# sinamalakouti/CDDMSL

Measured on AMD Instinct MI355X. Metric: images/sec (train step) VOC+Clipart RN50-C4, higher is better.
Workload: dtype bf16

## Files before the change

cddmsl_amd/csrc/bottleneck64.hip:

```cpp
#include "gemm_common.h"

namespace {

struct BottleneckArgs {
  const char* o1;
  const char* w2;
  const char* w3;
  const char* wd;
  const char* w1n;
  const char* x0;
  const char* residual;
  char* out;
  char* o1n;
  const float *s2, *b2, *s3, *b3, *sd, *bd, *s1n, *b1n;
  int H, W, M;
  FastDiv dW, dH;
};

template <bool DOWN, bool NEXT>
__global__ __launch_bounds__(512) void k_bottleneck64(BottleneckArgs p) {
  using T = __bf16;
  constexpr int KS2 = 36, WAVES = 8;
  const int lane = threadIdx.x & 63, r = lane & 31, hh = lane >> 5, wv = threadIdx.x >> 6;
  __shared__ __attribute__((aligned(16))) u32x4 wl2[2 * KS2 * 64];
  __shared__ __attribute__((aligned(16))) u32x4 wl3[8 * 4 * 64];
  __shared__ __attribute__((aligned(16))) u32x4 slots[WAVES * 256];
  __shared__ float sbl[4 * 256];
  for (int f = wv; f < 2 * KS2; f += WAVES) {
    const int nt = f / KS2, ks = f - nt * KS2;
    wl2[f * 64 + lane] = *(const u32x4*)(p.w2 + ((long)(nt * 32 + r) * (2 * KS2) + 2 * ks + hh) * 16);
  }
  for (int f = wv; f < 32; f += WAVES)
    wl3[f * 64 + lane] = *(const u32x4*)(p.w3 + ((long)((f >> 2) * 32 + r) * 8 + 2 * (f & 3) + hh) * 16);
  if (threadIdx.x < 256) {
    sbl[threadIdx.x] = p.s3[threadIdx.x]; sbl[256 + threadIdx.x] = p.b3[threadIdx.x];
    if (DOWN) { sbl[512 + threadIdx.x] = p.sd[threadIdx.x]; sbl[768 + threadIdx.x] = p.bd[threadIdx.x]; }
  }
  __syncthreads();
  float sc2[2], bi2[2], sc1[2], bi1[2];
#pragma unroll
  for (int nt = 0; nt < 2; ++nt) {
    sc2[nt] = p.s2[nt * 32 + r]; bi2[nt] = p.b2[nt * 32 + r];
    sc1[nt] = NEXT ? p.s1n[nt * 32 + r] : 1.f; bi1[nt] = NEXT ? p.b1n[nt * 32 + r] : 0.f;
  }
  const int wave = blockIdx.x * WAVES + wv, nwaves = gridDim.x * WAVES;
  const int ntiles = (p.M + 31) >> 5;
  const __amdgpu_buffer_rsrc_t rx = __builtin_amdgcn_make_buffer_rsrc((void*)(p.o1 - (long)(p.W + 1) * 128), 0, 0x7fffffff, 0x00020000);
  const __amdgpu_buffer_rsrc_t rx0 = __builtin_amdgcn_make_buffer_rsrc((void*)p.x0, 0, DOWN ? p.M * 128 : 0, 0x00020000);
  const __amdgpu_buffer_rsrc_t rres = __builtin_amdgcn_make_buffer_rsrc((void*)p.residual, 0, DOWN ? 0 : p.M * 512, 0x00020000);
  const __amdgpu_buffer_rsrc_t rout = __builtin_amdgcn_make_buffer_rsrc((void*)p.out, 0, p.M * 512, 0x00020000);
  const __amdgpu_buffer_rsrc_t ro1n = __builtin_amdgcn_make_buffer_rsrc((void*)p.o1n, 0, NEXT ? p.M * 128 : 0, 0x00020000);
  const float relu_floor = 0.f;
  char* const sb = (char*)slots + wv * 4096;
  char* wbase[8];
#pragma unroll
  for (int c = 0; c < 8; ++c) wbase[c] = sb + 4 * hh * 128 + ((((r >> 3) ^ (hh << 1)) ^ c) << 4) + (r & 7) * 2;
  const char* fbase = sb + r * 128;
  const int fsw = hh ^ ((r >> 1) & 7);
  const int mrow = lane >> 3;
  char* const mbase0 = sb + mrow * 128 + ((((lane & 7) ^ (lane >> 4))) << 4);
  char* const mbase1 = sb + mrow * 128 + ((((lane & 7) ^ (lane >> 4) ^ 4)) << 4);
  auto maddr = [&](int i) -> char* { return ((i & 1) ? mbase1 : mbase0) + i * 1024; };
  auto put = [&](const f32x16 (&acc)[2], const float (&sc)[2], const float (&bi)[2]) {
#pragma unroll
    for (int nt = 0; nt < 2; ++nt)
#pragma unroll
      for (int g = 0; g < 16; ++g) {
        float v = affine<T>(acc[nt][g], sc[nt], bi[nt]);
        asm("v_max_f32 %0, %1, %2" : "=v"(v) : "v"(v), "s"(relu_floor));
        *(unsigned short*)(wbase[(nt << 2) ^ ((g & 3) >> 1) ^ (((g >> 2) & 1) << 2)] + ((g & 3) + 8 * (g >> 2)) * 128) = f2bf(v);
      }
  };
  auto frags = [&](u32x4 (&fa)[4]) {
#pragma unroll
    for (int ks = 0; ks < 4; ++ks) fa[ks] = *(const u32x4*)(fbase + (((2 * ks) ^ fsw) << 4));
  };
  for (int tile = wave; tile < ntiles; tile += nwaves) {
    const int m = tile * 32 + r;
    const bool vm = m < p.M;
    const unsigned mm = vm ? m : 0;
    const unsigned tq = fdiv(mm, p.dW), ox = mm - tq * p.W;
    const unsigned img = fdiv(tq, p.dH), oy = tq - img * p.H;
    const int iy0 = (int)oy - 1, ix0 = (int)ox - 1;
    const unsigned lbase = (unsigned)((((int)img * p.H + iy0 + 1) * p.W + ix0 + 1) * 128) + hh * 16;
    unsigned bad = vm ? 0u : 0x1ffu;
#pragma unroll
    for (int ky = 0; ky < 3; ++ky)
#pragma unroll
      for (int kx = 0; kx < 3; ++kx)
        if ((unsigned)(iy0 + ky) >= (unsigned)p.H || (unsigned)(ix0 + kx) >= (unsigned)p.W) bad |= 1u << (3 * ky + kx);
    u32x4 a[KS2];
#pragma unroll
    for (int ks = 0; ks < KS2; ++ks) {
      const int t0 = (2 * ks) / 8, c0 = (2 * ks) % 8;
      const unsigned v = lbase | (__builtin_amdgcn_ubfe(bad, (unsigned)t0, 1u) << 31);
      a[ks] = __builtin_amdgcn_raw_buffer_load_b128(rx, v, ((t0 / 3) * p.W + (t0 % 3)) * 128 + c0 * 16, 0);
    }
    const unsigned rowbad[4] = {tile * 32 + mrow < p.M ? 0u : 0x80000000u, tile * 32 + 8 + mrow < p.M ? 0u : 0x80000000u,
                                tile * 32 + 16 + mrow < p.M ? 0u : 0x80000000u, tile * 32 + 24 + mrow < p.M ? 0u : 0x80000000u};
    const unsigned vq = (unsigned)(mrow * 512 + (lane & 7) * 16);
    u32x4 xa[4], rr[4];
    if (DOWN) {
#pragma unroll
      for (int ks = 0; ks < 4; ++ks)
        xa[ks] = __builtin_amdgcn_raw_buffer_load_b128(rx0, (unsigned)(r * 128 + hh * 16) | (vm ? 0u : 0x80000000u), tile * 4096 + ks * 32, 0);
    } else {
#pragma unroll
      for (int i = 0; i < 4; ++i) rr[i] = __builtin_amdgcn_raw_buffer_load_b128(rres, (vq + i * 4096) | rowbad[i], tile * 16384, 0);
    }
    f32x16 acc2[2];
#pragma unroll
    for (int nt = 0; nt < 2; ++nt)
#pragma unroll
      for (int g = 0; g < 16; ++g) acc2[nt][g] = 0.f;
    int wlane = lane;
    asm volatile("" : "+v"(wlane));
    const char* const wdp = p.wd + ((wlane & 31) * 8 + (wlane >> 5)) * 16;
    const char* const w1p = p.w1n + ((wlane & 31) * 32 + (wlane >> 5)) * 16;
#pragma unroll
    for (int ks = 0; ks < KS2; ++ks)
#pragma unroll
      for (int nt = 0; nt < 2; ++nt) Mma<T>::step(acc2[nt], a[ks], wl2[(nt * KS2 + ks) * 64 + wlane]);
    asm volatile("" ::: "memory");
    put(acc2, sc2, bi2);
    asm volatile("" ::: "memory");
    u32x4 fo2[4];
    frags(fo2);
    asm volatile("" ::: "memory");
    f32x16 acc1[2];
#pragma unroll
    for (int nt = 0; nt < 2; ++nt)
#pragma unroll
      for (int g = 0; g < 16; ++g) acc1[nt][g] = 0.f;
#pragma unroll
    for (int q = 0; q < 4; ++q) {
      f32x16 acc3[2], accd[2];
#pragma unroll
      for (int nt = 0; nt < 2; ++nt)
#pragma unroll
        for (int g = 0; g < 16; ++g) { acc3[nt][g] = 0.f; accd[nt][g] = 0.f; }
      u32x4 wdf[DOWN ? 2 : 1][DOWN ? 4 : 1], w1f[NEXT ? 2 : 1][NEXT ? 4 : 1];
      if (DOWN) {
#pragma unroll
        for (int nt = 0; nt < 2; ++nt)
#pragma unroll
          for (int ks = 0; ks < 4; ++ks)
            wdf[DOWN ? nt : 0][DOWN ? ks : 0] = *(const u32x4*)(wdp + ((q * 2 + nt) * 32 * 8 + 2 * ks) * 16);
      }
      if (!DOWN) {
#pragma unroll
        for (int i = 0; i < 4; ++i) *(u32x4*)maddr(i) = rr[i];
        if (q < 3) {
#pragma unroll
          for (int i = 0; i < 4; ++i) rr[i] = __builtin_amdgcn_raw_buffer_load_b128(rres, (vq + i * 4096) | rowbad[i], tile * 16384 + (q + 1) * 128, 0);
        }
      }
#pragma unroll
      for (int ks = 0; ks < 4; ++ks)
#pragma unroll
        for (int nt = 0; nt < 2; ++nt) Mma<T>::step(acc3[nt], fo2[ks], wl3[(((q * 2 + nt) << 2) + ks) * 64 + wlane]);
      if (DOWN) {
#pragma unroll
        for (int ks = 0; ks < 4; ++ks)
#pragma unroll
          for (int nt = 0; nt < 2; ++nt) Mma<T>::step(accd[nt], xa[ks], wdf[DOWN ? nt : 0][DOWN ? ks : 0]);
      }
      if (NEXT) {
#pragma unroll
        for (int nt = 0; nt < 2; ++nt)
#pragma unroll
          for (int ks = 0; ks < 4; ++ks)
            w1f[NEXT ? nt : 0][NEXT ? ks : 0] = *(const u32x4*)(w1p + (nt * 32 * 32 + 2 * (4 * q + ks)) * 16);
      }
      asm volatile("" ::: "memory");
#pragma unroll
      for (int nt = 0; nt < 2; ++nt) {
        const int ch = (q * 2 + nt) * 32 + r;
        const float s3 = sbl[ch], b3 = sbl[256 + ch];
        const float sd = DOWN ? sbl[512 + ch] : 1.f, bd = DOWN ? sbl[768 + ch] : 0.f;
#pragma unroll
        for (int g = 0; g < 16; ++g) {
          unsigned short* e = (unsigned short*)(wbase[(nt << 2) ^ ((g & 3) >> 1) ^ (((g >> 2) & 1) << 2)] + ((g & 3) + 8 * (g >> 2)) * 128);
          float v = affine<T>(acc3[nt][g], s3, b3);
          if (DOWN) v += bf2f(f2bf(affine<T>(accd[nt][g], sd, bd)));
          else v += bf2f(*e);
          asm("v_max_f32 %0, %1, %2" : "=v"(v) : "v"(v), "s"(relu_floor));
          *e = f2bf(v);
        }
      }
      asm volatile("" ::: "memory");
#pragma unroll
      for (int i = 0; i < 4; ++i) {
        const u32x4 o = *(const u32x4*)maddr(i);
        __builtin_amdgcn_raw_buffer_store_b128(o, rout, (vq + i * 4096) | rowbad[i], tile * 16384 + q * 128, CDDMSL_STORE_AUX);
        asm volatile("s_nop 4" ::: "memory");
        asm volatile("" :: "v"(o));
      }
      if (NEXT) {
        u32x4 fo[4];
        frags(fo);
#pragma unroll
        for (int ks = 0; ks < 4; ++ks)
#pragma unroll
          for (int nt = 0; nt < 2; ++nt) Mma<T>::step(acc1[nt], fo[ks], w1f[NEXT ? nt : 0][NEXT ? ks : 0]);
      }
      asm volatile("" ::: "memory");
    }
    if (NEXT) {
      put(acc1, sc1, bi1);
      asm volatile("" ::: "memory");
#pragma unroll
      for (int i = 0; i < 4; ++i) {
        const u32x4 o = *(const u32x4*)maddr(i);
        __builtin_amdgcn_raw_buffer_store_b128(o, ro1n, (unsigned)((i * 64 + lane) * 16) | rowbad[i], tile * 4096, 0);
        asm volatile("s_nop 4" ::: "memory");
        asm volatile("" :: "v"(o));
      }
      asm volatile("" ::: "memory");
    }
  }
}

}

extern "C" int cddmsl_bottleneck64_ok(int Nimg, int H, int W, int dtype) {
  if (dtype != 0 || Nimg <= 0 || H <= 0 || W <= 0) return 0;
  return (long)Nimg * H * W + W + 64 < (1L << 31) / 512 ? 1 : 0;
}

extern "C" int cddmsl_bottleneck64_fwd(const void* o1, const void* w2, const float* s2, const float* b2, const void* w3,
                                       const float* s3, const float* b3, const void* residual, const void* x0, const void* wd,
                                       const float* sd, const float* bd, const void* w1n, const float* s1n, const float* b1n,
                                       void* out, void* o1n, int Nimg, int H, int W, int dtype, void* stream) {
  if (!cddmsl_bottleneck64_ok(Nimg, H, W, dtype)) return CDDMSL_ERR_ARG;
  if (!o1 || !w2 || !s2 || !b2 || !w3 || !s3 || !b3 || !out) return CDDMSL_ERR_ARG;
  const bool down = wd != nullptr, next = w1n != nullptr;
  if (down ? (!x0 || !sd || !bd || residual) : (!residual || x0 || sd || bd)) return CDDMSL_ERR_ARG;
  if (next ? (!s1n || !b1n || !o1n) : (s1n || b1n || o1n)) return CDDMSL_ERR_ARG;
  BottleneckArgs a;
  a.o1 = (const char*)o1; a.w2 = (const char*)w2; a.w3 = (const char*)w3; a.wd = (const char*)wd; a.w1n = (const char*)w1n;
  a.x0 = (const char*)x0; a.residual = (const char*)residual; a.out = (char*)out; a.o1n = (char*)o1n;
  a.s2 = s2; a.b2 = b2; a.s3 = s3; a.b3 = b3; a.sd = sd; a.bd = bd; a.s1n = s1n; a.b1n = b1n;
  a.H = H; a.W = W; a.M = Nimg * H * W;
  a.dW = make_fastdiv((unsigned)W); a.dH = make_fastdiv((unsigned)H);
  if (record_kernel(13)) return CDDMSL_OK;
  const int ncu = persistent_blocks_raw(), ntiles = (a.M + 31) / 32;
  const int want = (ntiles + 7) / 8, cap = ncu > 0 ? ncu : 256;
  const unsigned nb = (unsigned)(want < cap ? want : cap);
  const hipStream_t st = (hipStream_t)stream;
  if (down && next) hipLaunchKernelGGL((k_bottleneck64<true, true>), dim3(nb), dim3(512), 0, st, a);
  else if (down) hipLaunchKernelGGL((k_bottleneck64<true, false>), dim3(nb), dim3(512), 0, st, a);
  else if (next) hipLaunchKernelGGL((k_bottleneck64<false, true>), dim3(nb), dim3(512), 0, st, a);
  else hipLaunchKernelGGL((k_bottleneck64<false, false>), dim3(nb), dim3(512), 0, st, a);
  return launch_status();
}
```

cddmsl_amd/csrc/conv_fwd.hip:

```cpp
#include "gemm_common.h"

namespace {

template <typename T> __device__ __forceinline__ void load8(const char* p, float* f);
template <> __device__ __forceinline__ void load8<__bf16>(const char* p, float* f) {
  const u32x4 v = *(const u32x4*)p;
#pragma unroll
  for (int j = 0; j < 4; ++j) { f[2 * j] = bf2f(v[j] & 0xffff); f[2 * j + 1] = bf2f(v[j] >> 16); }
}
template <> __device__ __forceinline__ void load8<float>(const char* p, float* f) {
  const f32x4 a = ((const f32x4*)p)[0], b = ((const f32x4*)p)[1];
  f[0] = a[0]; f[1] = a[1]; f[2] = a[2]; f[3] = a[3]; f[4] = b[0]; f[5] = b[1]; f[6] = b[2]; f[7] = b[3];
}

__device__ __forceinline__ int swz(int row, int chunk) { return row * KCH + (chunk ^ ((row >> 1) & 7)); }

template <typename T>
__global__ __launch_bounds__(256, 2) void k_conv_fwd_reg(ConvArgs p) {
  __shared__ __attribute__((aligned(16))) u32x4 lds[2][BM * KCH];
  const int t = threadIdx.x;
  const int ntn = (p.Cout + BN - 1) / BN;
  const int tile_n = blockIdx.x % ntn, tile_m = blockIdx.x / ntn;
  const int m0 = tile_m * BM, n0 = tile_n * BN;
  const int cc = t & 7, rb = t >> 3;
// ... 153 lines not shown
#pragma unroll
    for (int a = 0; a < 2; ++a) {
#pragma unroll
      for (int g = 0; g < 16; ++g) {
        int m = m0 + wm * 64 + a * 32 + (g & 3) + 8 * (g >> 2) + 4 * h;
        if (m >= p.M) continue;
        float v = affine<T>(acc[a][b][g], sc, bi);
        if (p.residual) v += Mma<T>::load(p.residual + ((long)m * p.ldr + n) * Mma<T>::ES);
        if (p.relu) v = fmaxf(v, 0.f);
        if (p.relu_mask && !(Mma<T>::load(p.relu_mask + ((long)m * p.ldm + n) * Mma<T>::ES) > 0.f)) v = 0.f;
        if (p.out_f32) *(float*)(p.y + ((long)m * p.ldy + n) * 4) = v;
        else Mma<T>::store(p.y + ((long)m * p.ldy + n) * Mma<T>::ES, v);
      }
    }
  }
}


__device__ __forceinline__ long pooled_row(const ConvArgs& p, int m) {
  const unsigned tq = fdiv((unsigned)m, p.dWo), ox = m - tq * p.Wo;
  const unsigned img = fdiv(tq, p.dHo), oy = tq - img * p.Ho;
  const unsigned hp = p.Ho >> 1, wp = p.Wo >> 1;
  return ((oy >> 1) < hp && (ox >> 1) < wp) ? ((long)img * hp + (oy >> 1)) * wp + (ox >> 1) : -1L;
}

template <typename T>
__global__ __launch_bounds__(256, 2) void k_conv_fwd(ConvArgs p) {
  __shared__ __attribute__((aligned(16))) u32x4 lds[2][2][BM * KCH];
  const int t = threadIdx.x;
  p.x += (long)blockIdx.y * p.bx; p.w += (long)blockIdx.y * p.bw; p.y += (long)blockIdx.y * p.by;
  const int wvu = __builtin_amdgcn_readfirstlane(t >> 6);
  const int ntn = (p.Cout + BN - 1) / BN;
  const int lbid = xcd_remap(blockIdx.x, gridDim.x);
  const int tile_n = lbid % ntn, tile_m = lbid / ntn;
  const int m0 = tile_m * BM, n0 = tile_n * BN;
  const int cc = t & 7, rb = t >> 3;
  const int cl = cc ^ ((rb >> 1) & 7);

  long rowoff[4], wrow[4];
  int iy0[4], ix0[4];
  bool vm[4], vn[4];
#pragma unroll
  for (int i = 0; i < 4; ++i) {
    int m = m0 + rb + 32 * i;
    vm[i] = m < p.M;
    unsigned mm = vm[i] ? m : 0;
    unsigned tq = fdiv(mm, p.dWo), ox = mm - tq * p.Wo;
    unsigned img = fdiv(tq, p.dHo), oy = tq - img * p.Ho;
    iy0[i] = (int)oy * p.stride - p.pad;
    ix0[i] = (int)ox * p.stride - p.pad;
    rowoff[i] = ((((long)img * p.Hi + iy0[i]) * p.Wi + ix0[i]) * p.xrs) * 16;
    int n = n0 + rb + 32 * i;
    vn[i] = n < p.Cout;
    wrow[i] = (long)(vn[i] ? n : 0) * p.wrs * 16;
  }
  const int nkt = (p.Kc + KCH - 1) / KCH;
  const char* zp = (const char*)g_zero_page;
  const bool taps = !(p.KH == 1 && p.KW == 1 && p.pad == 0);
  int kc = cl;
  int pp0 = (int)fdiv((unsigned)kc, p.dcpp);
  int coff = kc - pp0 * p.cpp;
  int ky = (int)fdiv((unsigned)pp0, p.dKW), kx = pp0 - ky * p.KW;

  const bool fast = (p.cpp & 7) == 0;
  const char* pa[4];
  const char* pb[4];
  int inca[4], incb[4];
  int tiles_left_in_tap = 0;
  auto retap = [&]() {
    const int delta = ((ky * p.Wi + kx) * p.xrs + coff) * 16;
#pragma unroll
    for (int i = 0; i < 4; ++i) {
      bool ok = vm[i];
      if (taps) {
        int iy = iy0[i] + ky, ix = ix0[i] + kx;
        ok = ok && iy >= 0 && iy < p.Hi && ix >= 0 && ix < p.Wi;
      }
      pa[i] = ok ? p.x + rowoff[i] + delta : zp;
      inca[i] = ok ? KCH * 16 : 0;
    }
  };
  if (fast) {
#pragma unroll
    for (int i = 0; i < 4; ++i) {
      pb[i] = vn[i] ? p.w + wrow[i] + (long)kc * 16 : zp;
      incb[i] = vn[i] ? KCH * 16 : 0;
    }
    retap();
    tiles_left_in_tap = p.cpp >> 3;
  }

  auto stage = [&](int buf) {
    if (fast) {
#pragma unroll
      for (int i = 0; i < 4; ++i) glds16(pa[i], &lds[buf][0][(8 * wvu + 32 * i) * KCH]);
#pragma unroll
      for (int i = 0; i < 4; ++i) glds16(pb[i], &lds[buf][1][(8 * wvu + 32 * i) * KCH]);
#pragma unroll
      for (int i = 0; i < 4; ++i) pb[i] += incb[i];
      if (--tiles_left_in_tap == 0) {
        tiles_left_in_tap = p.cpp >> 3;
        coff = cl;
        if (++kx == p.KW) { kx = 0; ++ky; }
        retap();
      } else {
#pragma unroll
        for (int i = 0; i < 4; ++i) pa[i] += inca[i];
      }
      return;
    }
    const bool vk = kc < p.Kc;
    const int delta = ((ky * p.Wi + kx) * p.xrs + coff) * 16;
#pragma unroll
    for (int i = 0; i < 4; ++i) {
      bool ok = vk && vm[i];
      if (taps) {
        int iy = iy0[i] + ky, ix = ix0[i] + kx;
        ok = ok && iy >= 0 && iy < p.Hi && ix >= 0 && ix < p.Wi;
      }
      const char* src = ok ? p.x + rowoff[i] + delta : zp;
      glds16(src, &lds[buf][0][(8 * wvu + 32 * i) * KCH]);
    }
#pragma unroll
    for (int i = 0; i < 4; ++i) {
      const char* src = (vk && vn[i]) ? p.w + wrow[i] + (long)kc * 16 : zp;
      glds16(src, &lds[buf][1][(8 * wvu + 32 * i) * KCH]);
    }
    kc += KCH;
    coff += KCH;
    while (coff >= p.cpp) {
      coff -= p.cpp;
      if (++kx == p.KW) { kx = 0; ++ky; }
    }
  };

  f32x16 acc[2][2];
#pragma unroll
  for (int a = 0; a < 2; ++a)
#pragma unroll
    for (int b = 0; b < 2; ++b)
#pragma unroll
      for (int r = 0; r < 16; ++r) acc[a][b][r] = 0.f;

  const int lane = t & 63, wv = t >> 6;
  const int wm = wv >> 1, wn = wv & 1;
  const int r = lane & 31, h = lane >> 5;

  const bool vec_ok = (p.Cout % 8 == 0) && (p.ldy % 8 == 0) && (!p.residual || p.ldr % 8 == 0) && (!p.relu_mask || p.ldm % 8 == 0);
  constexpr bool PRE = Mma<T>::ES == 2;
  u32x4 rres[2][4], rmsk[2][4];
  const bool rf32 = PRE && p.res_f32;
  if (PRE && vec_ok && ((p.residual && !rf32) || p.relu_mask)) {
    const int n = n0 + wn * 64 + (lane & 7) * 8;
#pragma unroll
    for (int a = 0; a < 2; ++a)
#pragma unroll
      for (int i = 0; i < 4; ++i) {
        int m = m0 + wm * 64 + a * 32 + (lane >> 3) + 8 * i;
        bool ok = m < p.M && n < p.Cout;
        const u32x4 z = {0u, 0u, 0u, 0u};
        if (p.res_pool) {
          const long po = pooled_row(p, m);
          rres[a][i] = (ok && po >= 0) ? *(const u32x4*)(p.residual + (po * p.ldr + n) * 2) : z;
        } else
        rres[a][i] = (ok && p.residual && !rf32) ? *(const u32x4*)(p.residual + ((long)m * p.ldr + n) * 2) : z;
        rmsk[a][i] = (ok && p.relu_mask) ? *(const u32x4*)(p.relu_mask + ((long)m * p.ldm + n) * 2) : z;
      }
  }

  stage(0);
  for (int kt = 0; kt < nkt; ++kt) {
    const int cur = kt & 1;
    if (kt + 1 < nkt) {
      stage(cur ^ 1);
      asm volatile("s_waitcnt vmcnt(8)" ::: "memory");
    } else {
      asm volatile("s_waitcnt vmcnt(0)" ::: "memory");
    }
    __builtin_amdgcn_s_barrier();
    u32x4 fa[2][2], fb[2][2];
#pragma unroll
    for (int i = 0; i < 2; ++i) {
      fa[0][i] = lds[cur][0][swz(wm * 64 + i * 32 + r, h)];
      fb[0][i] = lds[cur][1][swz(wn * 64 + i * 32 + r, h)];
    }
#pragma unroll
    for (int ks = 0; ks < KCH / 2; ++ks) {
      if (ks + 1 < KCH / 2) {
#pragma unroll
        for (int i = 0; i < 2; ++i) {
          fa[(ks + 1) & 1][i] = lds[cur][0][swz(wm * 64 + i * 32 + r, 2 * (ks + 1) + h)];
          fb[(ks + 1) & 1][i] = lds[cur][1][swz(wn * 64 + i * 32 + r, 2 * (ks + 1) + h)];
        }
      }
#pragma unroll
      for (int a = 0; a < 2; ++a)
#pragma unroll
        for (int b = 0; b < 2; ++b) Mma<T>::step(acc[a][b], fa[ks & 1][a], fb[ks & 1][b]);
    }
    asm volatile("s_waitcnt lgkmcnt(0)" ::: "memory");
    __builtin_amdgcn_s_barrier();
  }

  if (vec_ok) {
    float* ep = (float*)&lds[0][0][0] + wv * 2048;
    const int cg = lane & 7, rr = lane >> 3;
    const int n = n0 + wn * 64 + cg * 8;
    float sc[8], bi[8];
#pragma unroll
    for (int j = 0; j < 8; ++j) {
      sc[j] = (p.scale && n + j < p.Cout) ? p.scale[n + j] : 1.f;
      bi[j] = (p.bias && n + j < p.Cout) ? p.bias[n + j] : 0.f;
    }
#pragma unroll
    for (int a = 0; a < 2; ++a) {
      __syncthreads();
#pragma unroll
      for (int b = 0; b < 2; ++b)
#pragma unroll
        for (int g = 0; g < 16; ++g) {
          int row = (g & 3) + 8 * (g >> 2) + 4 * h, col = b * 32 + r;
          ep[row * 64 + ((((col >> 3) ^ (row & 7)) << 3) | (col & 7))] = acc[a][b][g];
        }
      __syncthreads();
      if (n < p.Cout) {
#pragma unroll
        for (int i = 0; i < 4; ++i) {
          int row = rr + 8 * i;
          int m = m0 + wm * 64 + a * 32 + row;
          if (m >= p.M) continue;
          const f32x4* src = (const f32x4*)(ep + row * 64 + ((cg ^ (row & 7)) << 3));
          f32x4 v0 = src[0], v1 = src[1];
          float v[8] = {v0[0], v0[1], v0[2], v0[3], v1[0], v1[1], v1[2], v1[3]};
#pragma unroll
          for (int j = 0; j < 8; ++j) v[j] = affine<T>(v[j], sc[j], bi[j]);
          if (p.residual) {
            float rv[8];
            if (rf32) load8<float>(p.residual + ((long)m * p.ldr + n) * 4, rv);
            else if (PRE) {
#pragma unroll
              for (int j = 0; j < 4; ++j) { rv[2 * j] = bf2f(rres[a][i][j] & 0xffff); rv[2 * j + 1] = bf2f(rres[a][i][j] >> 16); }
            } else if (p.res_pool) {
              const long po = pooled_row(p, m);
#pragma unroll
              for (int j = 0; j < 8; ++j) rv[j] = 0.f;
              if (po >= 0) load8<T>(p.residual + (po * p.ldr + n) * Mma<T>::ES, rv);
            } else load8<T>(p.residual + ((long)m * p.ldr + n) * Mma<T>::ES, rv);
            if (p.res_pool) {
#pragma unroll
              for (int j = 0; j < 8; ++j) rv[j] *= 0.25f;
            }
#pragma unroll
            for (int j = 0; j < 8; ++j) v[j] += rv[j];
          }
          if (p.relu) {
#pragma unroll
            for (int j = 0; j < 8; ++j) v[j] = fmaxf(v[j], 0.f);
          }
          if (p.relu_mask) {
            float mv[8];
            if (PRE) {
#pragma unroll
              for (int j = 0; j < 4; ++j) { mv[2 * j] = bf2f(rmsk[a][i][j] & 0xffff); mv[2 * j + 1] = bf2f(rmsk[a][i][j] >> 16); }
            } else load8<T>(p.relu_mask + ((long)m * p.ldm + n) * Mma<T>::ES, mv);
#pragma unroll
            for (int j = 0; j < 8; ++j) if (!(mv[j] > 0.f)) v[j] = 0.f;
          }
          if (p.out_f32 || Mma<T>::ES == 4) {
            f32x4* dst = (f32x4*)(p.y + ((long)m * p.ldy + n) * 4);
            f32x4 o0 = {v[0], v[1], v[2], v[3]}, o1 = {v[4], v[5], v[6], v[7]};
            dst[0] = o0; dst[1] = o1;
          } else {
            u32x4 o = {pack2bf(v[0], v[1]), pack2bf(v[2], v[3]), pack2bf(v[4], v[5]), pack2bf(v[6], v[7])};
            *(u32x4*)(p.y + ((long)m * p.ldy + n) * 2) = o;
          }
        }
      }
    }
    return;
  }
#pragma unroll
  for (int b = 0; b < 2; ++b) {
    int n = n0 + wn * 64 + b * 32 + r;
    if (n >= p.Cout) continue;
    float sc = p.scale ? p.scale[n] : 1.f;
    float bi = p.bias ? p.bias[n] : 0.f;
#pragma unroll
    for (int a = 0; a < 2; ++a) {
#pragma unroll
      for (int g = 0; g < 16; ++g) {
        int m = m0 + wm * 64 + a * 32 + (g & 3) + 8 * (g >> 2) + 4 * h;
        if (m >= p.M) continue;
        float v = affine<T>(acc[a][b][g], sc, bi);
        if (p.residual) v += Mma<T>::load(p.residual + ((long)m * p.ldr + n) * Mma<T>::ES);
        if (p.relu) v = fmaxf(v, 0.f);
        if (p.relu_mask && !(Mma<T>::load(p.relu_mask + ((long)m * p.ldm + n) * Mma<T>::ES) > 0.f)) v = 0.f;
        if (p.out_f32) *(float*)(p.y + ((long)m * p.ldy + n) * 4) = v;
        else Mma<T>::store(p.y + ((long)m * p.ldy + n) * Mma<T>::ES, v);
      }
    }
  }
}

template <typename T, int CPP, int NT, int NTAP = 9>
__global__ __launch_bounds__(256) void k_conv3x3_small(ConvArgs p) {
  constexpr int KC = NTAP * CPP, KS = (KC + 1) / 2;
  constexpr int PAD = NTAP == 9 ? 1 : 0;
  constexpr int ES = Mma<T>::ES;
  const int lane = threadIdx.x & 63, r = lane & 31, hh = lane >> 5;
  constexpr bool WLDS = CPP > 1;
  __shared__ __attribute__((aligned(16))) u32x4 wl[WLDS ? NT * KS * 64 : 1];
  u32x4 bw[WLDS ? 1 : NT][WLDS ? 1 : KS];
  {
    const int wv = threadIdx.x >> 6;
#pragma unroll
    for (int nt = 0; nt < NT; ++nt)
#pragma unroll
      for (int ks = 0; ks < KS; ++ks) {
        if (WLDS && ((nt * KS + ks) & 3) != wv) continue;
        const int q = 2 * ks + hh;
        u32x4 v = {0u, 0u, 0u, 0u};
        if (q < KC) v = *(const u32x4*)(p.w + ((long)(nt * 32 + r) * KC + q) * 16);
        if (WLDS) wl[(nt * KS + ks) * 64 + lane] = v;
        else bw[WLDS ? 0 : nt][WLDS ? 0 : ks] = v;
      }
    if (WLDS) __syncthreads();
  }
  float sc[NT], bi[NT];
#pragma unroll
  for (int nt = 0; nt < NT; ++nt) { sc[nt] = p.scale ? p.scale[nt * 32 + r] : 1.f; bi[nt] = p.bias ? p.bias[nt * 32 + r] : 0.f; }
  const int wave = (blockIdx.x * blockDim.x + threadIdx.x) >> 6, nwaves = (gridDim.x * blockDim.x) >> 6;
  const int ntiles = (p.M + 31) >> 5;
  const __amdgpu_buffer_rsrc_t rx = __builtin_amdgcn_make_buffer_rsrc((void*)(p.x - (long)(p.Wi + 1) * (CPP * 16)), 0, 0x7fffffff, 0x00020000);
  const long ybytes = (long)p.M * p.ldy * ES, mbytes = (long)p.M * p.ldm * ES;
  const __amdgpu_buffer_rsrc_t ry = __builtin_amdgcn_make_buffer_rsrc((void*)p.y, 0, (int)(ybytes > 0x7fffffffL ? 0x7fffffffL : ybytes), 0x00020000);
  const __amdgpu_buffer_rsrc_t rm = __builtin_amdgcn_make_buffer_rsrc((void*)p.relu_mask, 0, p.relu_mask ? (int)(mbytes > 0x7fffffffL ? 0x7fffffffL : mbytes) : 0, 0x00020000);
  const float relu_floor = p.relu ? 0.f : -__builtin_inff();
  __shared__ __attribute__((aligned(16))) u32x4 ost[ES == 2 ? 4 * 32 * NT * 4 : 1];
  const bool ost_ok = !p.relu_mask && p.ldy == NT * 32 && (long)p.M * NT * 64 < 0x7fffffffL;
  for (int tile = wave; tile < ntiles; tile += nwaves) {
    const int m = tile * 32 + r;
    const bool vm = m < p.M;
    const unsigned mm = vm ? m : 0;
    const unsigned tq = fdiv(mm, p.dWo), ox = mm - tq * p.Wo;
    const unsigned img = fdiv(tq, p.dHo), oy = tq - img * p.Ho;
    const int iy0 = (int)oy * p.stride - PAD, ix0 = (int)ox * p.stride - PAD;
    const unsigned lbase = (unsigned)((((int)img * p.Hi + iy0 + 1) * p.Wi + ix0 + 1) * (CPP * 16)) + (CPP > 1 ? hh * 16 : 0);
    unsigned bad = vm ? 0u : 0x1ffu;
    if (NTAP == 9) {
#pragma unroll
      for (int ky = 0; ky < 3; ++ky)
#pragma unroll
        for (int kx = 0; kx < 3; ++kx)
          if ((unsigned)(iy0 + ky) >= (unsigned)p.Hi || (unsigned)(ix0 + kx) >= (unsigned)p.Wi) bad |= 1u << (3 * ky + kx);
    }
    u32x4 a[KS];
#pragma unroll
    for (int ks = 0; ks < KS; ++ks) {
      const int q0 = 2 * ks, q1 = 2 * ks + 1;
      const int t0 = q0 / CPP, c0 = q0 % CPP, t1 = q1 / CPP, c1 = q1 % CPP;
      if (CPP > 1) {
        const unsigned v = lbase | (__builtin_amdgcn_ubfe(bad, (unsigned)t0, 1u) << 31);
        a[ks] = __builtin_amdgcn_raw_buffer_load_b128(rx, v, ((t0 / 3) * p.Wi + (t0 % 3)) * (CPP * 16) + c0 * 16, 0);
      } else {
        const int ky = hh ? t1 / 3 : t0 / 3, kx = hh ? t1 % 3 : t0 % 3, cc = hh ? c1 : c0;
        const bool inq = hh ? (q1 < KC) : (q0 < KC);
        const int iy = iy0 + ky, ix = ix0 + kx;
        const bool ok = vm && inq && (unsigned)iy < (unsigned)p.Hi && (unsigned)ix < (unsigned)p.Wi;
        u32x4 v = {0u, 0u, 0u, 0u};
        if (ok) v = *(const u32x4*)(p.x + ((((long)img * p.Hi + iy0) * p.Wi + ix0) + (long)ky * p.Wi + kx) * (CPP * 16) + cc * 16);
        a[ks] = v;
      }
    }
    f32x16 acc[NT];
#pragma unroll
    for (int nt = 0; nt < NT; ++nt)
#pragma unroll
      for (int g = 0; g < 16; ++g) acc[nt][g] = 0.f;
    int wlane = lane;
    asm volatile("" : "+v"(wlane));
#pragma unroll
    for (int ks = 0; ks < KS; ++ks)
#pragma unroll
      for (int nt = 0; nt < NT; ++nt) {
        if (WLDS) Mma<T>::step(acc[nt], a[ks], wl[(nt * KS + ks) * 64 + wlane]);
        else Mma<T>::step(acc[nt], a[ks], bw[WLDS ? 0 : nt][WLDS ? 0 : ks]);
      }
    if (ES == 2 && ost_ok) {
      char* ob = (char*)ost + (threadIdx.x >> 6) * (32 * NT * 64);
#pragma unroll
      for (int nt = 0; nt < NT; ++nt)
#pragma unroll
        for (int g = 0; g < 16; ++g) {
          const int row = (g & 3) + 8 * (g >> 2) + 4 * hh;
          float v = affine<T>(acc[nt][g], sc[nt], bi[nt]);
          asm("v_max_f32 %0, %1, %2" : "=v"(v) : "v"(v), "s"(relu_floor));
          *(unsigned short*)(ob + row * (NT * 64) + (nt * 32 + r) * 2) = f2bf(v);
        }
#pragma unroll
      for (int i = 0; i < 2 * NT; ++i) {
        const u32x4 o = *(const u32x4*)(ob + (i * 64 + lane) * 16);
        __builtin_amdgcn_raw_buffer_store_b128(o, ry, (unsigned)((i * 64 + lane) * 16), tile * (32 * NT * 64), 0);
      }
      continue;
    }
    const unsigned vy = (unsigned)(((tile * 32 + 4 * hh) * p.ldy + r) * ES), vmk = (unsigned)(((tile * 32 + 4 * hh) * p.ldm + r) * ES);
#pragma unroll
    for (int nt = 0; nt < NT; ++nt)
#pragma unroll
      for (int g = 0; g < 16; ++g) {
        const int row = (g & 3) + 8 * (g >> 2);
        float v = affine<T>(acc[nt][g], sc[nt], bi[nt]);
        asm("v_max_f32 %0, %1, %2" : "=v"(v) : "v"(v), "s"(relu_floor));
        if (p.relu_mask) {
          float mv;
          if (ES == 2) mv = bf2f((unsigned)__builtin_amdgcn_raw_buffer_load_b16(rm, vmk, (row * p.ldm + nt * 32) * ES, 0));
          else mv = __builtin_bit_cast(float, __builtin_amdgcn_raw_buffer_load_b32(rm, vmk, (row * p.ldm + nt * 32) * ES, 0));
          if (!(mv > 0.f)) v = 0.f;
        }
        if (ES == 2) __builtin_amdgcn_raw_buffer_store_b16((unsigned short)f2bf(v), ry, vy, (row * p.ldy + nt * 32) * ES, 0);
        else __builtin_amdgcn_raw_buffer_store_b32(__builtin_bit_cast(unsigned, v), ry, vy, (row * p.ldy + nt * 32) * ES, 0);
      }
  }
}

template <typename T> void launch_small(const ConvArgs& a, unsigned nb, hipStream_t st) {
  if (a.KH == 1 && a.cpp == 8) hipLaunchKernelGGL((k_conv3x3_small<T, 8, 2, 1>), dim3(nb), dim3(256), 0, st, a);
  else if (a.KH == 1) hipLaunchKernelGGL((k_conv3x3_small<T, 32, 2, 1>), dim3(nb), dim3(256), 0, st, a);
  else if (a.cpp == 1 && a.Cout == 32) hipLaunchKernelGGL((k_conv3x3_small<T, 1, 1>), dim3(nb), dim3(256), 0, st, a);
  else if (a.cpp == 1) hipLaunchKernelGGL((k_conv3x3_small<T, 1, 2>), dim3(nb), dim3(256), 0, st, a);
  else if (a.cpp == 8) hipLaunchKernelGGL((k_conv3x3_small<T, 8, 2>), dim3(nb), dim3(256), 0, st, a);
  else if (a.Cout == 32) hipLaunchKernelGGL((k_conv3x3_small<T, 4, 1>), dim3(nb), dim3(256), 0, st, a);
  else hipLaunchKernelGGL((k_conv3x3_small<T, 4, 2>), dim3(nb), dim3(256), 0, st, a);
}

template <typename T> void launch_tile128(const ConvArgs& a, const Plan& p, hipStream_t st) {
  const dim3 grid(p.gx, p.gy);
  switch (p.kernel) {
    case 8: launch_small<T>(a, p.gx, st); break;
    case 2: hipLaunchKernelGGL(k_conv_fwd_reg<T>, grid, dim3(256), 0, st, a); break;
    default: hipLaunchKernelGGL(k_conv_fwd<T>, grid, dim3(256), 0, st, a); break;
  }
}

}

void launch_fwd_tile128(const ConvArgs& a, const Plan& p, Operand op, hipStream_t st) {
  if (op == OP_BF16) launch_tile128<__bf16>(a, p, st);
  else launch_tile128<float>(a, p, st);
}
```

cddmsl_amd/csrc/gemm_common.h:

```cpp
#pragma once
#include "common.h"
#include <cstdlib>

namespace {

constexpr int BM = 128, BN = 128, KCH = 8;

struct FastDiv {
  unsigned mul, shr, d;
};
static inline FastDiv make_fastdiv(unsigned d) {
  FastDiv f;
  f.d = d;
  unsigned s = 0;
  while ((1ull << s) < d) ++s;
  f.shr = s;
  f.mul = (unsigned)(((1ull << 32) * ((1ull << s) - d)) / d + 1);
  return f;
}
__device__ __forceinline__ unsigned fdiv(unsigned n, const FastDiv& f) { return (__umulhi(n, f.mul) + n) >> f.shr; }

template <typename T> __device__ __forceinline__ float affine(float v, float sc, float bi) {
  return sizeof(T) <= 2 ? __builtin_fmaf(v, sc, bi) : v * sc + bi;
}

#ifndef CDDMSL_STORE_AUX
#define CDDMSL_STORE_AUX 2
#endif
#ifndef CDDMSL_LOAD_AUX
#define CDDMSL_LOAD_AUX 0
#endif

struct ConvArgs {
  const char* x;
  const char* w;
  char* y;
  const float* scale;
  const float* bias;
  const char* residual;
  const char* relu_mask;
  int Nimg, Hi, Wi, Cin, Ho, Wo, Cout, KH, KW, stride, pad;
  int ldy, ldr, ldm;
  int relu, out_f32, pool;
  int res_f32;
  int res_pool;
  int M, Kc, cpp;
  FastDiv dWo, dHo, dcpp, dKW;
  int xrs, wrs;
  long bx, bw, by;
  char* y8 = nullptr;
  const float* q8 = nullptr;
  unsigned* amax8 = nullptr;
  float* partial = nullptr;
  int tile0 = 0, ksplits = 1, kper = 0, tile_limit = 0;
  int nt_out = 1;
#ifdef CDDMSL_TILE_STAMPS
  unsigned long long* tstamps = nullptr;
#endif
};

template <typename T> struct Mma;
template <> struct Mma<__bf16> {
  static constexpr int ES = 2;
  __device__ static __forceinline__ void step(f32x16& acc, const u32x4& a, const u32x4& b) {
    acc = __builtin_amdgcn_mfma_f32_32x32x16_bf16(__builtin_bit_cast(bf16x8, a), __builtin_bit_cast(bf16x8, b), acc, 0, 0, 0);
  }
  __device__ static __forceinline__ float load(const char* p) { return bf2f(*(const unsigned short*)p); }
  __device__ static __forceinline__ void store(char* p, float v) { *(unsigned short*)p = f2bf(v); }
};
template <> struct Mma<float> {
  static constexpr int ES = 4;
  __device__ static __forceinline__ void step(f32x16& acc, const u32x4& a, const u32x4& b) {
    const f32x4 fa = __builtin_bit_cast(f32x4, a), fb = __builtin_bit_cast(f32x4, b);
    acc = __builtin_amdgcn_mfma_f32_32x32x2f32(fa[0], fb[0], acc, 0, 0, 0);
    acc = __builtin_amdgcn_mfma_f32_32x32x2f32(fa[1], fb[1], acc, 0, 0, 0);
    acc = __builtin_amdgcn_mfma_f32_32x32x2f32(fa[2], fb[2], acc, 0, 0, 0);
    acc = __builtin_amdgcn_mfma_f32_32x32x2f32(fa[3], fb[3], acc, 0, 0, 0);
  }
  __device__ static __forceinline__ float load(const char* p) { return *(const float*)p; }
  __device__ static __forceinline__ void store(char* p, float v) { *(float*)p = v; }
};
typedef __attribute__((ext_vector_type(8))) int i32x8;

__device__ __forceinline__ int xcd_remap(int bid, int nblk) {
  const int q = nblk >> 3, rem = nblk & 7, x = bid & 7, j = bid >> 3;
  return (x < rem ? x * (q + 1) : rem * (q + 1) + (x - rem) * q) + j;
}

template <typename T> __device__ __forceinline__ u32x4 avg4(const u32x4& a, const u32x4& b, const u32x4& c, const u32x4& d);
template <> __device__ __forceinline__ u32x4 avg4<float>(const u32x4& a, const u32x4& b, const u32x4& c, const u32x4& d) {
  const f32x4 fa = __builtin_bit_cast(f32x4, a), fb = __builtin_bit_cast(f32x4, b);
  const f32x4 fc = __builtin_bit_cast(f32x4, c), fd = __builtin_bit_cast(f32x4, d);
  f32x4 r = ((fa + fb) + (fc + fd)) * 0.25f;
  return __builtin_bit_cast(u32x4, r);
}
template <> __device__ __forceinline__ u32x4 avg4<__bf16>(const u32x4& a, const u32x4& b, const u32x4& c, const u32x4& d) {
  u32x4 r;
#pragma unroll
  for (int j = 0; j < 4; ++j) {
    float lo = (bf2f(a[j] & 0xffff) + bf2f(b[j] & 0xffff)) + (bf2f(c[j] & 0xffff) + bf2f(d[j] & 0xffff));
    float hi = (bf2f(a[j] >> 16) + bf2f(b[j] >> 16)) + (bf2f(c[j] >> 16) + bf2f(d[j] >> 16));
    r[j] = pack2bf(lo * 0.25f, hi * 0.25f);
  }
  return r;
}

__device__ __attribute__((aligned(16))) unsigned int g_zero_page[4] = {0u, 0u, 0u, 0u};

__device__ __forceinline__ void glds16(const void* g, void* l) {
  __builtin_amdgcn_global_load_lds((const __attribute__((address_space(1))) void*)g,
                                   (__attribute__((address_space(3))) void*)l, 16, 0, 0);
}

struct WgradArgs {
  const char* x;
  const char* dy;
  float* dw;
  const float* scale;
  int Nimg, Hi, Wi, Cin, Ho, Wo, Cout, KH, KW, stride, pad, ldd, pool;
  int M, Kc, cpp, K, ncc;
  int mtiles_per_split;
  FastDiv dWo, dHo;
  int xrs;
  int ldo;
  int direct;
  long bx, bd, bo;
  const float* g0 = nullptr;
  const unsigned long long* mbits = nullptr;
  float* gpos = nullptr;
  float* ws = nullptr;
#ifdef CDDMSL_TILE_STAMPS
  unsigned long long* tstamps = nullptr;
#endif
};

constexpr int WM = 64;
constexpr int WROW = 16 + 4;

__device__ __forceinline__ int fsw(int row) { return ((row & 3) << 2) | ((row >> 2) & 3); }

__device__ __forceinline__ void store_frags(f32x4* dst, const f32x16 (&acc)[4][2]) {
#pragma unroll
  for (int a = 0; a < 4; ++a)
#pragma unroll
    for (int b = 0; b < 2; ++b)
#pragma unroll
      for (int g4 = 0; g4 < 4; ++g4) {
        const f32x4 v = {acc[a][b][4 * g4], acc[a][b][4 * g4 + 1], acc[a][b][4 * g4 + 2], acc[a][b][4 * g4 + 3]};
        dst[((a * 2 + b) * 4 + g4) * 64] = v;
      }
}

static long env_int(const char* name, long dflt, bool* set = nullptr) {
  const char* e = getenv(name);
  if (set) *set = e != nullptr;
  return e ? atol(e) : dflt;
}

enum Operand { OP_BF16 = 0, OP_F32 = 1, OP_FP8 = 2 };
static int elem_size(Operand op) { return op == OP_BF16 ? 2 : op == OP_F32 ? 4 : 1; }

struct Plan {
  int kernel;
  unsigned gx, gy;
  int splits;
  int mtiles_per_split;
  int bpb;
};

static int persistent_blocks_raw() {
  static int ncu = -1;
  if (ncu < 0) {
    int dev = 0, n = 0;
    if (hipGetDevice(&dev) != hipSuccess || hipDeviceGetAttribute(&n, hipDeviceAttributeMultiprocessorCount, dev) != hipSuccess) n = 0;
    ncu = (n / 8) * 8;
  }
  return ncu;
}

}

extern "C" {
__attribute__((visibility("hidden"))) void launch_fwd_tile128(const ConvArgs& a, const Plan& p, Operand op, hipStream_t st);
__attribute__((visibility("hidden"))) void launch_fwd_tile256(const ConvArgs& a, const Plan& p, Operand op, hipStream_t st, void* ws, long ws_bytes);
__attribute__((visibility("hidden"))) void launch_wgrad(WgradArgs& a, const Plan& p, Operand op, hipStream_t st, void* ws, long ws_bytes);
__attribute__((visibility("hidden"))) void launch_gemm_tn(const WgradArgs& p, Operand op, const Plan& pl, int batch, int mode, hipStream_t st);
__attribute__((visibility("hidden"))) void launch_attnpool_dx(const WgradArgs& p, unsigned gx, unsigned gy, int nbatch, int bpb, hipStream_t st);
__attribute__((visibility("hidden"))) bool record_kernel(int id);
}
```

cddmsl_amd/csrc/gemm_conv.hip:

```cpp
#include "gemm_common.h"

namespace {

template <typename T>
__device__ __forceinline__ void weight_prep_body(const float* w, const float* scale, char* wf, char* wd, int Cout, int KH, int KW, int Cin,
                                                 long first, long stride) {
  __shared__ float tile[32][33];
  const int taps = KH * KW, nit = (Cin + 31) / 32, nct = (Cout + 31) / 32;
  const long ntiles = (long)nct * taps * nit;
  const int tx = threadIdx.x & 31, ty = threadIdx.x >> 5;
  constexpr int ES = Mma<T>::ES;
  for (long tl = first; tl < ntiles; tl += stride) {
    const int it = (int)(tl % nit); const long q = tl / nit;
    const int tap = (int)(q % taps), ct = (int)(q / taps);
    const int ky = tap / KW, kx = tap % KW;
    __syncthreads();
#pragma unroll
    for (int r = 0; r < 4; ++r) {
      const int co = ct * 32 + ty + 8 * r, ci = it * 32 + tx;
      float v = 0.f;
      if (co < Cout && ci < Cin) {
        const long i = ((long)co * taps + tap) * Cin + ci;
        v = w[i];
        if (wf) Mma<T>::store(wf + i * ES, v);
        if (scale) v *= scale[co];
      }
      tile[ty + 8 * r][tx] = v;
    }
    __syncthreads();
    if (wd) {
#pragma unroll
      for (int r = 0; r < 4; ++r) {
        const int ci = it * 32 + ty + 8 * r, co = ct * 32 + tx;
        if (ci < Cin && co < Cout) {
          const long j = (((long)ci * KH + (KH - 1 - ky)) * KW + (KW - 1 - kx)) * Cout + co;
          Mma<T>::store(wd + j * ES, tile[tx][ty + 8 * r]);
        }
      }
    }
  }
}
template <typename T>
__global__ __launch_bounds__(256) void k_weight_prep(const float* w, const float* scale, char* wf, char* wd, int Cout, int KH, int KW, int Cin) {
  weight_prep_body<T>(w, scale, wf, wd, Cout, KH, KW, Cin, (long)blockIdx.x, (long)gridDim.x);
}
template <typename T>
__global__ __launch_bounds__(256) void k_weight_prep_multi(const long long* table) {
  const long long* e = table + 8 * (long)blockIdx.y;
  weight_prep_body<T>((const float*)e[0], (const float*)e[1], (char*)e[2], (char*)e[3], (int)e[4], (int)e[5], (int)e[6], (int)e[7],
                      (long)blockIdx.x, (long)gridDim.x);
}

static thread_local int g_last_kernel = 0;
static thread_local int g_plan_only = 0;


static bool gemm256_legal(const ConvArgs& a) {
  const bool vec_ok = (a.ldy % 8 == 0) && (!a.residual || a.ldr % 8 == 0) && (!a.relu_mask || a.ldm % 8 == 0);
  if (a.pool || (a.cpp & 7) || (a.Cout & 255) || !vec_ok || a.KH * a.KW > 31) return false;
  if (2 * a.pad > a.KH - 1 || 2 * a.pad > a.KW - 1) return false;
  return true;
}

static bool use_gemm256(const ConvArgs& a, int batch) {
  const long mode = env_int("CDDMSL_GEMM256", 1);
  if (mode == 0) return false;
  if (!gemm256_legal(a)) return false;
  if (mode == 2) return true;
  const long tiles = (long)((a.M + 255) / 256) * (a.Cout / 256) * batch;
  return tiles >= 160;
}

static bool fwd2_legal(const ConvArgs& a) {
  const bool vec_ok = (a.ldy % 8 == 0) && (!a.residual || a.ldr % 8 == 0) && (!a.relu_mask || a.ldm % 8 == 0);
  if (a.pool || a.res_pool || (a.cpp & 3) || (a.Cout & 127) || !vec_ok || a.KH * a.KW > 31) return false;
  if (2 * a.pad > a.KH - 1 || 2 * a.pad > a.KW - 1) return false;
  return true;
}
static bool use_fwd2(const ConvArgs& a, int batch) {
  const long mode = env_int("CDDMSL_FWD2", 1);
  if (mode == 0 || !fwd2_legal(a)) return false;
  if (mode == 2) return true;
  if (use_gemm256(a, batch) || batch != 1) return false;
  return (long)(a.Cout / 128) * ((a.M + 255) / 256) >= env_int("CDDMSL_FWD2_MIN", 256);
}

static Plan plan_fwd(const ConvArgs& a, Operand op, int batch) {
  const long tiles256 = (long)(a.Cout / 256) * ((a.M + 255) / 256);
  if (op == OP_FP8) {
    if (!gemm256_legal(a) || tiles256 > 0x7fffffffL) return {};
    return {10, (unsigned)tiles256, 1};
  }
  if (a.y8 && !use_gemm256(a, batch)) return {};
  const long tiles128 = (long)((a.Cout + BN - 1) / BN) * ((a.M + BM - 1) / BM);
  if (tiles128 > 0x7fffffffL) return {};
  const bool packed = batch == 1 && a.xrs == a.cpp && a.wrs == a.Kc;
  if (!a.pool && a.KH == 3 && a.KW == 3 && a.pad == 1 && (a.cpp == 1 || a.cpp == 4 || (a.cpp == 8 && a.Cout == 64)) &&
      (a.Cout == 32 || a.Cout == 64) && !a.residual && !a.out_f32 && packed) {
    return {8, a.cpp > 1 ? 256u * 2 : 256u * 8, 1};
  }
  if (op == OP_BF16 && !a.pool && a.KH == 1 && a.KW == 1 && a.pad == 0 && a.stride == 1 && a.Cout == 64 && (a.cpp == 8 || a.cpp == 32) &&
      !a.residual && !a.out_f32 && !a.y8 && packed && a.ldy == 64 && env_int("CDDMSL_SMALL_1X1", 1) != 0) return {8, 512, 1};
  if (use_fwd2(a, batch)) return {11, (unsigned)((long)(a.Cout / 128) * ((a.M + 255) / 256)), (unsigned)batch};
  if (use_gemm256(a, batch)) return {3, (unsigned)tiles256, (unsigned)batch};
  if (a.pool) return {2, (unsigned)tiles128, 1};
  return {1, (unsigned)tiles128, (unsigned)batch};
}

static void* g_ws = nullptr;
static long g_ws_bytes = 0;

static int run_fwd(const ConvArgs& a, Operand op, const Plan& p, void* stream) {
  if (p.kernel == 0) return CDDMSL_ERR_ARG;
  g_last_kernel = p.kernel;
  if (g_plan_only) return CDDMSL_OK;
  if (p.kernel == 3 || p.kernel == 10 || p.kernel == 11) launch_fwd_tile256(a, p, op, (hipStream_t)stream, g_ws, g_ws_bytes);
  else launch_fwd_tile128(a, p, op, (hipStream_t)stream);
  return launch_status();
}

}

#ifdef CDDMSL_TILE_STAMPS
static unsigned long long* g_tile_stamps = nullptr;
extern "C" void cddmsl_debug_tile_stamps(unsigned long long* p) { g_tile_stamps = p; }
#endif
extern "C" int cddmsl_last_kernel(void) { return g_last_kernel; }
extern "C" int cddmsl_plan_only(int on) { const int was = g_plan_only; g_plan_only = on; return was; }
bool record_kernel(int id) { g_last_kernel = id; return g_plan_only != 0; }

static int nt_out_for(long out_bytes) {
  static const long nt_min_mb = env_int("CDDMSL_NT_MIN_MB", 128);
  return out_bytes > (nt_min_mb << 20) ? 1 : 0;
}

static int fill_conv(ConvArgs& a, Operand op, const void* x, const void* w, void* y, const float* scale, const float* bias,
                     const void* residual, const void* relu_mask, int Nimg, int Hi, int Wi, int Cin, int Cout, int KH, int KW,
                     int stride, int pad, int pool, int ldy, int ldr, int ldm, int relu, int out_f32, void* y8, const float* q8,
                     float* amax8) {
  const int es = elem_size(op);
  if (Nimg < 0 || Hi <= 0 || Wi <= 0 || Cin <= 0 || Cout <= 0 || KH <= 0 || KW <= 0 || stride <= 0) return CDDMSL_ERR_ARG;
  if ((Cin * es) % 16 != 0) return CDDMSL_ERR_ARG;
  if (pool && (KH != 1 || KW != 1 || pad != 0 || stride != 1)) return CDDMSL_ERR_ARG;
  a.x = (const char*)x; a.w = (const char*)w; a.y = (char*)y; a.scale = scale; a.bias = bias;
  a.residual = (const char*)residual; a.relu_mask = (const char*)relu_mask;
  a.Nimg = Nimg; a.Hi = Hi; a.Wi = Wi; a.Cin = Cin; a.Cout = Cout; a.KH = KH; a.KW = KW; a.stride = stride; a.pad = pad;
  if (pool) { a.Ho = Hi / 2; a.Wo = Wi / 2; }
  else { a.Ho = (Hi + 2 * pad - KH) / stride + 1; a.Wo = (Wi + 2 * pad - KW) / stride + 1; }
  if (a.Ho <= 0 || a.Wo <= 0) return CDDMSL_ERR_ARG;
  if ((out_f32 & 2) && (!(out_f32 & 1) || !residual || relu_mask || pool)) return CDDMSL_ERR_ARG;
  a.ldy = ldy; a.ldr = ldr; a.ldm = ldm; a.relu = relu; a.out_f32 = out_f32 & 1; a.pool = pool;
  a.res_f32 = (op == OP_BF16 && (out_f32 & 2)) ? 1 : 0;
  a.res_pool = (out_f32 & 4) ? 1 : 0;
  if (a.res_pool && (!residual || (out_f32 & 2) || pool || KH != 1 || KW != 1 || pad != 0 || (long)Nimg * (a.Ho / 2) * (a.Wo / 2) * ldr * es >= (1L << 31) ||
                     (Cout & 7) || (ldy & 7) || (ldr & 7) || (relu_mask && (ldm & 7)))) return CDDMSL_ERR_ARG;
  if (a.res_f32 && ((Cout & 7) || (ldy & 7) || (ldr & 7))) return CDDMSL_ERR_ARG;
  long M = (long)Nimg * a.Ho * a.Wo;
  if (M > 0x7fffff00L) return CDDMSL_ERR_ARG;
  a.M = (int)M; a.cpp = Cin * es / 16; a.Kc = KH * KW * a.cpp;
  a.dWo = make_fastdiv((unsigned)a.Wo); a.dHo = make_fastdiv((unsigned)a.Ho);
  a.dcpp = make_fastdiv((unsigned)a.cpp); a.dKW = make_fastdiv((unsigned)KW);
  a.xrs = a.cpp; a.wrs = a.Kc; a.bx = a.bw = a.by = 0;
#ifdef CDDMSL_TILE_STAMPS
  a.tstamps = g_tile_stamps;
#endif
  if (a.M == 0) return CDDMSL_OK;
  a.nt_out = nt_out_for((long)a.M * Cout * 2);
  if (y8) {
    if (op == OP_F32 || (out_f32 & 1) || ldy != Cout) return CDDMSL_ERR_ARG;
    a.y8 = (char*)y8; a.q8 = q8; a.amax8 = (unsigned*)amax8;
  }
  return CDDMSL_OK;
}

static int conv_fwd_any(Operand op, const void* x, const void* w, void* y, const float* scale, const float* bias,
                        const void* residual, const void* relu_mask, int Nimg, int Hi, int Wi, int Cin,
                        int Cout, int KH, int KW, int stride, int pad, int pool, int ldy, int ldr, int ldm,
                        int relu, int out_f32, void* y8, const float* q8, float* amax8, void* stream) {
  ConvArgs a;
  const int st = fill_conv(a, op, x, w, y, scale, bias, residual, relu_mask, Nimg, Hi, Wi, Cin, Cout, KH, KW, stride, pad, pool, ldy, ldr, ldm,
                           relu, out_f32, y8, q8, amax8);
  if (st != CDDMSL_OK || a.M == 0) return st;
  return run_fwd(a, op, plan_fwd(a, op, 1), stream);
}

extern "C" int cddmsl_conv_fwd(const void* x, const void* w, void* y, const float* scale, const float* bias,
                               const void* residual, const void* relu_mask, int Nimg, int Hi, int Wi, int Cin,
                               int Cout, int KH, int KW, int stride, int pad, int pool, int ldy, int ldr, int ldm,
                               int relu, int out_f32, int dtype, void* stream) {
  if (dtype != 0 && dtype != 1) return CDDMSL_ERR_ARG;
  return conv_fwd_any((Operand)dtype, x, w, y, scale, bias, residual, relu_mask, Nimg, Hi, Wi, Cin, Cout, KH, KW, stride, pad, pool, ldy, ldr, ldm,
                      relu, out_f32, nullptr, nullptr, nullptr, stream);
}

extern "C" int cddmsl_conv_fwd_q8(const void* x, const void* w, void* y, const float* scale, const float* bias,
                                  const void* residual, const void* relu_mask, int Nimg, int Hi, int Wi, int Cin,
                                  int Cout, int KH, int KW, int stride, int pad, int relu, void* y8, const float* q8, float* amax8,
                                  void* stream) {
  if (!y8) return CDDMSL_ERR_ARG;
  return conv_fwd_any(OP_BF16, x, w, y, scale, bias, residual, relu_mask, Nimg, Hi, Wi, Cin, Cout, KH, KW, stride, pad, 0, Cout, Cout, Cout,
                      relu, 0, y8, q8, amax8, stream);
}

extern "C" int cddmsl_conv_fwd_fp8(const void* x, const void* w, void* y, const float* scale, const float* bias,
                                   const void* residual, const void* relu_mask, int Nimg, int Hi, int Wi, int Cin, int Cout, int KH,
                                   int KW, int pad, int relu, int out_f32, void* y8, const float* q8, float* amax8, void* stream) {
  if (Cin % 128 != 0 || (out_f32 & ~1)) return CDDMSL_ERR_ARG;
  return conv_fwd_any(OP_FP8, x, w, y, scale, bias, residual, relu_mask, Nimg, Hi, Wi, Cin, Cout, KH, KW, 1, pad, 0, Cout, Cout, Cout,
                      relu, out_f32, y8, q8, amax8, stream);
}

static bool wgrad256_ok(const WgradArgs& a, int batch) {
  const long mode = env_int("CDDMSL_GEMM256", 1);
  if (mode == 0) return false;
  if ((a.Cout & 255) || (a.K & 255) || (a.cpp & 7) || (a.ldd & 7)) return false;
  if (mode == 2) return true;
  return (long)(a.Cout / 256) * (a.K / 256) * batch * ((a.M + WM - 1) / WM) >= env_int("CDDMSL_WGRAD256_MIN", 4000);
}
static bool wgrad256_span_ok(int mtiles_per_split, int Wi, long row_bytes) {
  return ((long)mtiles_per_split * WM + WM + 2L * Wi + 2) * row_bytes + (1L << 20) < (1L << 31);
}

static int even_split(int total_mt, long* splits) {
  const int mps = (int)((total_mt + *splits - 1) / *splits);
  *splits = (total_mt + mps - 1) / mps;
  return mps;
}

static long split_512_rounds(long tiles, int total_mt, bool taps) {
  bool forced;
  const long target = env_int("CDDMSL_WGRAD_BLOCKS", taps ? 1024 : 512, &forced);
  const long maxs = (total_mt + 7) / 8;
  long splits = 1;
  const long r0 = (target + 511) / 512;
  double best = -1.0;
  for (long r = r0; r <= r0 + 1; ++r) {
    long c = (512 * r) / tiles;
    if (c < 1) c = 1;
    if (c > maxs) c = maxs;
    long real = c;
    even_split(total_mt, &real);
    const long blocks = tiles * real, rounds = (blocks + 511) / 512;
    const double eff = (double)blocks / (512.0 * rounds);
    if (eff > best + 0.03) { best = eff; splits = c; }
    if (c == maxs) break;
  }
  if (forced) { splits = (target + tiles - 1) / tiles; if (splits > maxs) splits = maxs; }
  return splits < 1 ? 1 : splits;
}

static long split_256_rounds(long tiles, int total_mt) {
  const long maxs = (total_mt + 15) / 16;
  long sp = 1;
  double best = -1.0;
  for (int r = 1; r <= 6; ++r) {
    long c = (256L * r) / tiles;
    if (c < 1) continue;
    if (c > maxs) c = maxs;
    const long blocks = tiles * c, rounds = (blocks + 255) / 256;
    const double eff = (double)blocks / (256.0 * rounds);
    if (eff > best + 0.02) { best = eff; sp = c; }
    if (c == maxs) break;
  }
  return sp;
}

static Plan plan_wgrad(const WgradArgs& a, Operand op, int batch) {
  const int es = elem_size(op), total_mt = (a.M + WM - 1) / WM;
  const long tiles256 = (long)(a.Cout / 256) * (a.K / 256);
  const long row_bytes = (long)a.ldd * es > a.xrs * 16L ? (long)a.ldd * es : a.xrs * 16L;
  if (op == OP_FP8) {
    long sp = split_256_rounds(tiles256, total_mt);
    const int mps = even_split(total_mt, &sp);
    if (!wgrad256_span_ok(mps, a.Wi, row_bytes)) return {};
    return {12, (unsigned)(tiles256 * sp), 1, (int)sp, mps};
  }
  const int cols = 256 / es;
  const long tiles = (long)((a.Cout + cols - 1) / cols) * ((a.K + cols - 1) / cols);
  long splits = split_512_rounds(tiles, total_mt, !(a.KH == 1 && a.KW == 1));
  const int mps = even_split(total_mt, &splits);
  if (tiles * splits > 0x7fffffffL) return {};
  const bool same = !a.pool && a.stride == 1 && a.Ho == a.Hi && a.Wo == a.Wi;
  if (same && op == OP_BF16 && wgrad256_ok(a, batch)) {
    bool forced;
    const long want = env_int("CDDMSL_WGRAD256_BLOCKS", 0, &forced);
    const long maxs = (total_mt + 15) / 16;
    long sp = forced ? (want + tiles256 - 1) / tiles256 : split_256_rounds(tiles256, total_mt);
    if (sp > maxs) sp = maxs;
    if (sp < 1) sp = 1;
    const int mps256 = even_split(total_mt, &sp);
    if (wgrad256_span_ok(mps256, a.Wi, row_bytes)) return {6, (unsigned)(tiles256 * sp), 1, (int)sp, mps256};
  }
  return {same ? 5 : 4, (unsigned)(tiles * splits), 1, (int)splits, mps};
}

extern "C" int cddmsl_set_workspace(void* ptr, long bytes) {
  if (bytes < 0 || (ptr == nullptr && bytes != 0) || ((size_t)ptr & 15)) return CDDMSL_ERR_ARG;
  g_ws = ptr; g_ws_bytes = bytes;
  return CDDMSL_OK;
}

static int run_wgrad(WgradArgs& a, Operand op, const Plan& p, void* stream) {
  if (p.kernel == 0) return CDDMSL_ERR_ARG;
  g_last_kernel = p.kernel;
  if (g_plan_only) return CDDMSL_OK;
  a.mtiles_per_split = p.mtiles_per_split;
  launch_wgrad(a, p, op, (hipStream_t)stream, g_ws, g_ws_bytes);
  return launch_status();
}

static int fill_wgrad(WgradArgs& a, Operand op, const void* x, const void* dy, float* dw, const float* scale, int Nimg, int Hi,
                      int Wi, int Cin, int Cout, int KH, int KW, int stride, int pad, int pool, int ldd) {
  const int es = elem_size(op);
  if (Nimg < 0 || Hi <= 0 || Wi <= 0 || Cin <= 0 || Cout <= 0 || KH <= 0 || KW <= 0 || stride <= 0) return CDDMSL_ERR_ARG;
  if ((Cin * es) % 16 != 0 || (Cout * es) % 16 != 0 || (ldd * es) % 16 != 0) return CDDMSL_ERR_ARG;
  if (pool && (KH != 1 || KW != 1 || pad != 0 || stride != 1)) return CDDMSL_ERR_ARG;
  a.x = (const char*)x; a.dy = (const char*)dy; a.dw = dw; a.scale = scale;
  a.Nimg = Nimg; a.Hi = Hi; a.Wi = Wi; a.Cin = Cin; a.Cout = Cout; a.KH = KH; a.KW = KW; a.stride = stride; a.pad = pad;
  a.ldd = ldd; a.pool = pool;
  if (pool) { a.Ho = Hi / 2; a.Wo = Wi / 2; }
  else { a.Ho = (Hi + 2 * pad - KH) / stride + 1; a.Wo = (Wi + 2 * pad - KW) / stride + 1; }
  if (a.Ho <= 0 || a.Wo <= 0) return CDDMSL_ERR_ARG;
  long M = (long)Nimg * a.Ho * a.Wo;
  if (M > 0x7fffff00L) return CDDMSL_ERR_ARG;
  a.M = (int)M; a.cpp = Cin * es / 16; a.Kc = KH * KW * a.cpp; a.K = KH * KW * Cin; a.ncc = Cout * es / 16;
  a.mtiles_per_split = 0;
  a.dWo = make_fastdiv((unsigned)a.Wo); a.dHo = make_fastdiv((unsigned)a.Ho);
  a.xrs = a.cpp; a.ldo = a.K; a.direct = 0; a.bx = a.bd = a.bo = 0;
#ifdef CDDMSL_TILE_STAMPS
  a.tstamps = g_tile_stamps;
#endif
  return CDDMSL_OK;
}

extern "C" int cddmsl_conv_wgrad(const void* x, const void* dy, float* dw, const float* scale, int Nimg, int Hi,
                                 int Wi, int Cin, int Cout, int KH, int KW, int stride, int pad, int pool, int ldd,
                                 int dtype, void* stream) {
  if (dtype != 0 && dtype != 1) return CDDMSL_ERR_ARG;
  WgradArgs a;
  const int st = fill_wgrad(a, (Operand)dtype, x, dy, dw, scale, Nimg, Hi, Wi, Cin, Cout, KH, KW, stride, pad, pool, ldd);
  if (st != CDDMSL_OK || a.M == 0) return st;
  return run_wgrad(a, (Operand)dtype, plan_wgrad(a, (Operand)dtype, 1), stream);
}

extern "C" int cddmsl_conv_wgrad_fp8_ok(int Cin, int Cout, int KH, int KW, int pad, int ldd) {
  return (Cin % 256 == 0 && Cout % 256 == 0 && KH == KW && (KH & 1) && 2 * pad == KH - 1 && ldd % 16 == 0) ? 1 : 0;
}
extern "C" int cddmsl_conv_wgrad_fp8(const void* x8, const void* dy8, float* dw, const float* scale, int Nimg, int Hi, int Wi, int Cin,
                                     int Cout, int KH, int KW, int pad, int ldd, void* stream) {
  if (!cddmsl_conv_wgrad_fp8_ok(Cin, Cout, KH, KW, pad, ldd) || ldd < Cout) return CDDMSL_ERR_ARG;
  WgradArgs a;
  const int st = fill_wgrad(a, OP_FP8, x8, dy8, dw, scale, Nimg, Hi, Wi, Cin, Cout, KH, KW, 1, pad, 0, ldd);
  if (st != CDDMSL_OK || a.M == 0) return st;
  return run_wgrad(a, OP_FP8, plan_wgrad(a, OP_FP8, 1), stream);
}

extern "C" int cddmsl_gemm_nt_batched(const void* a, const void* w, void* c, const float* bias, int M, int N, int K, int lda,
                                      int ldb, int ldc, int batch, long sa, long sw, long sc, int out_f32, int dtype, void* stream) {
  int es = dtype == 0 ? 2 : 4;
  if (dtype != 0 && dtype != 1) return CDDMSL_ERR_ARG;
  if (M < 0 || N <= 0 || K <= 0 || batch < 0 || batch > 65535) return CDDMSL_ERR_ARG;
  if ((K * es) % 16 || (lda * es) % 16 || (ldb * es) % 16 || (sa * es) % 16 || (sw * es) % 16) return CDDMSL_ERR_ARG;
  if (M == 0 || batch == 0) return CDDMSL_OK;
  const Operand op = (Operand)dtype;
  ConvArgs p;
  const int st = fill_conv(p, op, a, w, c, nullptr, bias, nullptr, nullptr, 1, 1, M, K, N, 1, 1, 1, 0, 0, ldc, 0, 0, 0, out_f32 ? 1 : 0,
                           nullptr, nullptr, nullptr);
  if (st != CDDMSL_OK) return st;
  p.xrs = lda * es / 16; p.wrs = ldb * es / 16;
  p.bx = sa * es; p.bw = sw * es; p.by = sc * (out_f32 ? 4 : es);
  p.nt_out = 1;
  return run_fwd(p, op, plan_fwd(p, op, batch), stream);
}

static unsigned tn_small_grid(long kt, long batch, int* bpb) {
  long b = (kt * batch + 4095) / 4096;
  if (b < 8) b = 8;
  if (b > batch) b = batch;
  *bpb = (int)b;
  return (unsigned)((batch + b - 1) / b);
}

static Plan plan_gemm_tn(const WgradArgs& p, Operand op, int batch, int mode) {
  const int cols = 256 / elem_size(op), M = p.M, N = p.Cout, K = p.K;
  const long tiles = (long)((N + cols - 1) / cols) * ((K + cols - 1) / cols);
  const int total_mt = (M + WM - 1) / WM;
  if (op == OP_BF16 && total_mt == 1 && N <= 64 && batch >= 64 && K % 128 == 0 && N % 8 == 0) {
    Plan p = {9, (unsigned)(K / 128), 0};
    p.gy = tn_small_grid(K / 128, batch, &p.bpb);
    return p;
  }
  if (total_mt <= 4 && batch >= 64) {
    long bpb = (tiles * batch + 4095) / 4096, minb = (8 + total_mt - 1) / total_mt;
    if (bpb < minb) bpb = minb;
    if (bpb > batch) bpb = batch;
    return {7, (unsigned)tiles, (unsigned)((batch + bpb - 1) / bpb), 0, 0, (int)bpb};
  }
  long splits = 1;
  if (mode == 0) {
    const long want = (2048 + tiles * batch - 1) / (tiles * batch), maxs = (total_mt + 7) / 8;
    splits = want < 1 ? 1 : (want > maxs ? maxs : want);
    if (splits < 1) splits = 1;
  }
  const int mps = even_split(total_mt, &splits);
  if (tiles * splits > 0x7fffffffL) return {};
  return {5, (unsigned)(tiles * splits), (unsigned)batch, (int)splits, mps};
}

extern "C" int cddmsl_gemm_tn_batched(const void* a, const void* b, void* out, int M, int N, int K, int lda, int ldb, int ldo,
                                      int batch, long sa, long sb, long so, int mode, int dtype, void* stream) {
  int es = dtype == 0 ? 2 : 4;
  if (dtype != 0 && dtype != 1) return CDDMSL_ERR_ARG;
  if (M <= 0 || N <= 0 || K <= 0 || batch <= 0 || batch > 65535 || mode < 0 || mode > 2) return CDDMSL_ERR_ARG;
  if ((K * es) % 16 || (N * es) % 16 || (lda * es) % 16 || (ldb * es) % 16 || (sa * es) % 16 || (sb * es) % 16) return CDDMSL_ERR_ARG;
  const Operand op = (Operand)dtype;
  WgradArgs p;
  const int fs = fill_wgrad(p, op, b, a, (float*)out, nullptr, 1, 1, M, K, N, 1, 1, 1, 0, 0, lda);
  if (fs != CDDMSL_OK) return fs;
  p.xrs = ldb * es / 16; p.ldo = ldo; p.direct = mode;
  p.bx = sb * es; p.bd = sa * es; p.bo = so * (mode == 2 ? es : 4);
  const Plan pl = plan_gemm_tn(p, op, batch, mode);
  if (pl.kernel == 0) return CDDMSL_ERR_ARG;
  g_last_kernel = pl.kernel;
  if (g_plan_only) return CDDMSL_OK;
  p.mtiles_per_split = pl.mtiles_per_split;
  launch_gemm_tn(p, op, pl, batch, mode, (hipStream_t)stream);
  return launch_status();
}

extern "C" int cddmsl_attnpool_dx(const void* pds, const void* zu, const float* g0, const unsigned long long* mbits, void* dx, float* gpos,
                                  int K, int H2, int P, int TP, int C, int dtype, void* stream) {
  if (dtype != 0 || K < 0 || P != 49 || TP != 56 || H2 <= 0 || H2 > 64 || (H2 & 7) || C <= 0 || (C & 127) || !g0 || !mbits || !dx) return CDDMSL_ERR_ARG;
  if (K == 0) return CDDMSL_OK;
  if (K > 65535 * 8) return CDDMSL_ERR_ARG;
  WgradArgs p;
  const int fs = fill_wgrad(p, OP_BF16, zu, pds, (float*)dx, nullptr, 1, 1, H2, C, TP, 1, 1, 1, 0, 0, TP);
  if (fs != CDDMSL_OK) return fs;
  p.direct = 3;
  p.bx = (long)H2 * C * 2; p.bd = (long)H2 * TP * 2; p.bo = (long)P * C * 2;
  p.g0 = g0; p.mbits = mbits; p.gpos = gpos;
  int bpb;
  const unsigned gy = tn_small_grid(C / 128, K, &bpb);
  launch_attnpool_dx(p, (unsigned)(C / 128), gy, K, bpb, (hipStream_t)stream);
  return launch_status();
}

extern "C" int cddmsl_weight_prep_multi(const long long* table, int count, int dtype, void* stream) {
  if ((dtype != 0 && dtype != 1) || count < 0 || count > 65535) return CDDMSL_ERR_ARG;
  if (count == 0) return CDDMSL_OK;
  if (dtype == 0) hipLaunchKernelGGL(k_weight_prep_multi<__bf16>, dim3(256, (unsigned)count), dim3(256), 0, (hipStream_t)stream, table);
  else hipLaunchKernelGGL(k_weight_prep_multi<float>, dim3(256, (unsigned)count), dim3(256), 0, (hipStream_t)stream, table);
  return launch_status();
}

extern "C" int cddmsl_weight_prep(const float* w, const float* scale, void* w_fwd, void* w_dgrad, int Cout, int KH,
                                  int KW, int Cin, int dtype, void* stream) {
  if (dtype != 0 && dtype != 1) return CDDMSL_ERR_ARG;
  long n = (long)Cout * KH * KW * Cin;
  if (n <= 0) return n == 0 ? CDDMSL_OK : CDDMSL_ERR_ARG;
  const long tiles = (long)((Cout + 31) / 32) * KH * KW * ((Cin + 31) / 32);
  unsigned grid = (unsigned)(tiles > 4096 ? 4096 : tiles);
  if (dtype == 0) hipLaunchKernelGGL(k_weight_prep<__bf16>, dim3(grid), dim3(256), 0, (hipStream_t)stream, w, scale, (char*)w_fwd, (char*)w_dgrad, Cout, KH, KW, Cin);
  else hipLaunchKernelGGL(k_weight_prep<float>, dim3(grid), dim3(256), 0, (hipStream_t)stream, w, scale, (char*)w_fwd, (char*)w_dgrad, Cout, KH, KW, Cin);
  return launch_status();
}
```

cddmsl_amd/hip.py:

```python
import ctypes
import os
from ctypes import c_float, c_int, c_long, c_void_p

import torch

from ._lib import check, lib, ptr, require_cuda, stream_ptr

DT = {torch.bfloat16: 0, torch.float32: 1}

_sigs_done = False


def _L():
    global _sigs_done
    L = lib()
    if not _sigs_done:
        vp, ci, cf = c_void_p, c_int, c_float
        L.cddmsl_last_kernel.argtypes = []
        L.cddmsl_plan_only.argtypes = [ci]
        L.cddmsl_conv_fwd.argtypes = [vp] * 7 + [ci] * 16 + [vp]
        L.cddmsl_bottleneck64_ok.argtypes = [ci] * 4
        L.cddmsl_bottleneck64_fwd.argtypes = [vp] * 17 + [ci] * 4 + [vp]
        L.cddmsl_conv_wgrad.argtypes = [vp] * 4 + [ci] * 12 + [vp]
        L.cddmsl_set_workspace.argtypes = [vp, c_long]
        L.cddmsl_weight_prep.argtypes = [vp] * 4 + [ci] * 5 + [vp]
        L.cddmsl_weight_prep_multi.argtypes = [vp, ci, ci, vp]
        L.cddmsl_preprocess.argtypes = [vp, vp] + [ci] * 6 + [vp, vp, ci, ci, vp]
        L.cddmsl_maxpool3s2_fwd.argtypes = [vp, vp] + [ci] * 5 + [vp]
        L.cddmsl_upsample_zero2.argtypes = [vp] * 4 + [ci] * 5 + [vp]
        L.cddmsl_meanpool_fwd.argtypes = [vp, vp, c_long, ci, ci, ci, vp]
        L.cddmsl_meanpool_bwd.argtypes = [vp, vp, c_long, ci, ci, ci, vp]
        L.cddmsl_preprocess224.argtypes = [vp, vp] + [ci] * 11 + [vp, vp, ci, vp]
        L.cddmsl_preprocess_batch.argtypes = [vp, vp, vp, ci, vp, ci, ci, ci, vp, vp, ci, ci, vp]
        L.cddmsl_preprocess224_batch.argtypes = [vp, vp, vp, ci, vp] + [ci] * 8 + [vp, vp, ci, vp]
        L.cddmsl_avgpool2_fwd.argtypes = [vp, vp] + [ci] * 5 + [vp]
        L.cddmsl_avgpool2_bwd.argtypes = [vp] * 4 + [ci] * 5 + [vp]
        L.cddmsl_avgpool2_bwd_q8.argtypes = [vp] * 4 + [ci] * 4 + [vp] * 4
        L.cddmsl_attn_tokens_fwd.argtypes = [vp] * 3 + [ci] * 5 + [vp]
        L.cddmsl_attn_tokens_bwd.argtypes = [vp] * 4 + [ci] * 5 + [vp]
        L.cddmsl_attnpool_softmax_fwd.argtypes = [vp] * 3 + [c_long, ci, ci, ci, cf, ci, vp]
        L.cddmsl_attnpool_softmax_bwd.argtypes = [vp] * 4 + [c_long, ci, ci, ci, cf, ci, vp]
        L.cddmsl_gemm_nt_batched.argtypes = [vp] * 4 + [ci] * 7 + [c_long] * 3 + [ci, ci, vp]
        L.cddmsl_gemm_tn_batched.argtypes = [vp] * 3 + [ci] * 7 + [c_long] * 3 + [ci, ci, vp]
        L.cddmsl_relu_bwd.argtypes = [vp, vp, vp, c_long, ci, ci, vp]
        L.cddmsl_colsum.argtypes = [vp, vp, c_long, ci, ci, ci, vp]
        L.cddmsl_sgd_clip_step.argtypes = [vp] * 4 + [ci, vp] + [cf] * 4 + [ci, vp]
        L.cddmsl_roi_align_forward.argtypes = [vp] * 5 + [ci] * 7 + [cf, ci, ci, ci, vp]
        L.cddmsl_roi_align_backward.argtypes = [vp] * 7 + [ci] * 7 + [cf, ci, ci, ci, vp]
        L.cddmsl_nms_anyorder.argtypes = [vp] * 4 + [ci, cf, vp, vp, vp]
        L.cddmsl_roi_align_nchw_anyorder.argtypes = [vp] * 3 + [ci] * 7 + [cf, ci, ci, ci, vp, vp, vp]
        L.cddmsl_roi_align_backward_nchw_anyorder.argtypes = [vp] * 3 + [ci] * 7 + [cf, ci, ci, ci, vp, vp, vp]
        L.cddmsl_quantize_fp8.argtypes = [vp] * 4 + [c_long, ci, vp]
        L.cddmsl_conv_fwd_fp8.argtypes = [vp] * 7 + [ci] * 10 + [vp] * 4
        L.cddmsl_conv_wgrad_fp8_ok.argtypes = [ci] * 6
        L.cddmsl_conv_wgrad_fp8.argtypes = [vp] * 4 + [ci] * 9 + [vp]
        L.cddmsl_conv_fwd_q8.argtypes = [vp] * 7 + [ci] * 10 + [vp] * 4
        L.cddmsl_fp8_dot_nt.argtypes = [vp] * 4 + [ci] * 4 + [vp]
        L.cddmsl_roi_align_forward_affine.argtypes = [vp] * 6 + [ci] * 8 + [cf, ci, ci, ci] + [vp] * 4
        L.cddmsl_roi_align_backward_pooled.argtypes = [vp] * 7 + [ci] * 7 + [cf, ci, ci, ci, vp]
        L.cddmsl_anchors.argtypes = [vp, vp, ci, ci, ci, cf, cf, vp]
        L.cddmsl_sort_desc.argtypes = [vp] * 5 + [ci, ci, vp, vp, vp]
        L.cddmsl_rpn_decode.argtypes = [vp] * 6 + [ci] * 5 + [cf] * 8 + [vp]
        L.cddmsl_nms.argtypes = [vp] * 5 + [ci, ci, cf, ci, vp]
        L.cddmsl_iou_match.argtypes = [vp, ci, vp, ci, vp, vp, vp, ci, cf, cf, ci, ci, ci, ci, vp]
        L.cddmsl_iou_match_batched.argtypes = [vp] * 7 + [ci] * 5 + [cf, cf] + [ci] * 4 + [vp]
        L.cddmsl_l2norm_fwd.argtypes = [vp, vp, vp, c_long, ci, cf, vp]
        L.cddmsl_l2norm_bwd.argtypes = [vp, vp, vp, vp, c_long, ci, vp]
        L.cddmsl_cosine_logits_fwd.argtypes = [vp] * 4 + [c_long, ci, ci, cf, cf, vp]
        L.cddmsl_cosine_logits_bwd.argtypes = [vp] * 5 + [c_long, ci, ci, cf, ci, vp]
        L.cddmsl_layernorm_fwd.argtypes = [vp] * 6 + [c_long, ci, cf, ci, vp]
        L.cddmsl_layernorm_bwd.argtypes = [vp] * 6 + [c_long, ci, ci, ci, vp]
        L.cddmsl_focal_ce_fwd.argtypes = [vp] * 4 + [c_long, ci, cf, ci, cf, vp]
        L.cddmsl_focal_ce_bwd.argtypes = [vp] * 5 + [c_long, ci, cf, ci, cf, vp]
        L.cddmsl_attn_small_fwd.argtypes = [vp] * 4 + [ci] * 8 + [cf, ci, vp]
        L.cddmsl_attn_small_bwd.argtypes = [vp] * 7 + [ci] * 8 + [cf, ci, vp]
        L.cddmsl_attn_tokens_fwd_mask.argtypes = [vp] * 4 + [ci] * 5 + [vp]
        L.cddmsl_attnpool_dx.argtypes = [vp] * 6 + [ci] * 6 + [vp]
        L.cddmsl_rpn_losses.argtypes = [vp, vp, vp, ci, vp, ci, vp, vp, vp, vp, c_long, cf, cf, cf, cf, cf, vp, vp, vp, vp, vp]
        L.cddmsl_box_l1.argtypes = [vp, ci, vp, ci, vp, vp, vp, cf, cf, cf, cf, cf, vp, vp, vp, vp]
        L.cddmsl_attn_last_fwd.argtypes = [vp] * 4 + [ci] * 8 + [cf, ci, vp]
        L.cddmsl_attn_last_bwd.argtypes = [vp] * 6 + [ci] * 8 + [cf, ci, vp]
        L.cddmsl_contrastive_fwd.argtypes = [vp] * 4 + [ci, ci, vp]
        L.cddmsl_contrastive_bwd.argtypes = [vp] * 5 + [ci, ci, vp]
        L.cddmsl_instance_boxes.argtypes = [vp] + [ci] * 4 + [vp, ci, vp, vp, vp, vp]
        L.cddmsl_text_embed.argtypes = [vp] * 4 + [c_long, ci, ci, ci, ci, vp]
        L.cddmsl_attn_causal_fwd.argtypes = [vp, vp] + [ci] * 6 + [cf, ci, vp]
        L.cddmsl_quick_gelu.argtypes = [vp, c_long, ci, vp]
        L.cddmsl_text_pool.argtypes = [vp] * 5 + [c_long, ci, ci, ci, cf, ci, vp]
        L.cddmsl_skinny_gemm_workspace.argtypes = [ci] * 3
        L.cddmsl_skinny_gemm.argtypes = [vp] * 6 + [c_long] + [ci] * 4 + [vp]
        L.cddmsl_lm_head_workspace.argtypes = [ci, ci]
        L.cddmsl_lm_head_argmax.argtypes = [vp, vp, vp, ci, vp, vp, c_long, ci, ci, ci, vp]
        L.cddmsl_decode_attn.argtypes = [vp] * 4 + [ci] * 6 + [cf, ci, vp]
        L.cddmsl_pos_embed.argtypes = [vp, ci] + [vp] * 4 + [c_long] + [ci] * 6 + [vp]
        L.cddmsl_gelu_new.argtypes = [vp, c_long, ci, vp]
        L.cddmsl_lm_head_topk_workspace.argtypes = [ci, ci]
        L.cddmsl_lm_head_topk.argtypes = [vp] * 7 + [c_long] + [ci] * 4 + [vp]
        L.cddmsl_beam_step.argtypes = [vp] * 15 + [ci] * 5 + [vp]
        L.cddmsl_decode_attn_beam.argtypes = [vp] * 7 + [ci] * 9 + [cf, ci, vp]
        _sigs_done = True
    return L


class _Profiler:

    def __init__(self):
        self.on = False
        self.only = None
        self.events = []
        self.shapes = []

    def enable(self, only=None):
        self.on, self.only, self.events, self.shapes = True, (set(only) if only else None), [], []

    def begin(self, name=None, plan=None):
        if not self.on:
            return None
        if self.only is not None:
            if name is None and plan is not None:
                L = _L()
                L.cddmsl_plan_only(1)
                try:
                    plan()
                finally:
                    L.cddmsl_plan_only(0)
                name = _CONV_KERNEL.get(L.cddmsl_last_kernel())
            if name not in self.only:
                return None
        e = torch.cuda.Event(enable_timing=True)
        e.record()
        return e

    def end(self, e0, name, flops=0.0, shape=None, nbytes=0.0):
        if e0 is None:
            return
        e1 = torch.cuda.Event(enable_timing=True)
        e1.record()
        self.events.append((name, flops, e0, e1, nbytes))
        if shape is not None:
            self.shapes.append((name, shape, flops, e0, e1, nbytes))

    def by_shape(self):
        torch.cuda.synchronize()
        out = {}
        for name, shape, flops, e0, e1, nbytes in self.shapes:
            d = out.setdefault((name, shape), [0, 0.0, 0.0, 0.0])
            d[0] += 1
            d[1] += e0.elapsed_time(e1)
            d[2] += flops
            d[3] += nbytes
        return out

    def collect(self):
        torch.cuda.synchronize()
        out = {}
        for name, flops, e0, e1, nbytes in self.events:
            d = out.setdefault(name, {"flops": 0.0, "ms": 0.0, "launches": 0, "bytes": 0.0})
            d["flops"] += flops
            d["bytes"] += nbytes
            d["ms"] += e0.elapsed_time(e1)
            d["launches"] += 1
        self.on, self.only, self.events = False, None, []
        return out


PROFILE = _Profiler()
_CONV_KERNEL = {10: "k_conv_fwd256_fp8", 11: "k_conv_fwd2", 1: "k_conv_fwd", 2: "k_conv_fwd_reg", 3: "k_conv_fwd256", 4: "k_conv_wgrad", 5: "k_conv_wgrad_dma", 6: "k_wgrad256", 7: "k_gemm_tn_stream", 8: "k_conv3x3_small", 9: "k_gemm_tn_small", 12: "k_wgrad256_fp8",
                13: "k_bottleneck64"}


def _timed(name):
    def deco(fn):
        def wrapper(*a, **k):
            e0 = PROFILE.begin(name)
            r = fn(*a, **k)
            PROFILE.end(e0, name)
            return r
        wrapper.__name__, wrapper.__doc__ = fn.__name__, fn.__doc__
        return wrapper
    return deco


def _dt(t):
    if t.dtype not in DT:
        raise TypeError(f"unsupported dtype {t.dtype}: the kernels compute in bf16 or f32")
    return DT[t.dtype]


def _conv_input_pixels(N, H, W, Ho, Wo, KH, KW, stride, pool):
    if pool:
        return N * min(H, 2 * Ho) * min(W, 2 * Wo)
    rows = min(H, Ho * min(KH, stride) if stride > KH else (Ho - 1) * stride + KH)
    cols = min(W, Wo * min(KW, stride) if stride > KW else (Wo - 1) * stride + KW)
    return N * rows * cols


class OutSpec:

    def __init__(self):
        self.full, self.used = None, 0


def conv_fwd(x, w, scale=None, bias=None, residual=None, relu=False, relu_mask=None, stride=1, pad=0,
             pool=False, out_f32=False, residual_pooled=False, emit8=None, out_spec=None):
    require_cuda(x, w, scale, bias, residual, relu_mask)
    ensure_workspace(x.device)
    assert x.dim() == 4 and w.dim() == 4 and x.is_contiguous() and w.is_contiguous()
    assert x.dtype == w.dtype
    N, H, W, Cin = x.shape
    Cout, KH, KW, Cin2 = w.shape
    assert Cin == Cin2, (x.shape, w.shape)
    if pool:
        Ho, Wo = H // 2, W // 2
    else:
        Ho, Wo = (H + 2 * pad - KH) // stride + 1, (W + 2 * pad - KW) // stride + 1
    ydt = torch.float32 if out_f32 else x.dtype
    if out_spec is not None and out_spec.full is None:
        out_spec.full = torch.empty((2 * N, Ho, Wo, Cout), device=x.device, dtype=ydt)
        y, out_spec.used = out_spec.full[:N], 1
    elif out_spec is not None and out_spec.used == 1 and tuple(out_spec.full.shape) == (2 * N, Ho, Wo, Cout) and out_spec.full.dtype == ydt:
        y, out_spec.used = out_spec.full[N:], 2
    else:
        y = torch.empty((N, Ho, Wo, Cout), device=x.device, dtype=ydt)
    for v in (scale, bias):
        assert v is None or (v.dtype == torch.float32 and v.numel() == Cout and v.is_contiguous())
    res_f32 = residual is not None and residual.dtype == torch.float32 and x.dtype != torch.float32
    if res_f32:
        assert out_f32 and relu_mask is None and not pool and Cout % 8 == 0
    if residual_pooled:
        assert residual is not None and not res_f32 and residual.dtype == x.dtype and residual.is_contiguous()
        assert tuple(residual.shape) == (N, Ho // 2, Wo // 2, Cout) and pooled_residual_ok(residual), residual.shape
    for v in (residual, relu_mask):
        assert v is None or (v is residual and residual_pooled) or (
            (v.dtype == x.dtype or (v is residual and res_f32)) and v.is_contiguous() and v.numel() == y.numel())
    y8 = None
    if emit8 is not None:
        assert x.dtype == torch.bfloat16 and not out_f32 and not pool and not residual_pooled and not res_f32
        y8 = torch.empty(y.shape, device=x.device, dtype=torch.uint8)

    def launch():
        if y8 is not None:
            return _L().cddmsl_conv_fwd_q8(ptr(x), ptr(w), ptr(y), ptr(scale), ptr(bias), ptr(residual), ptr(relu_mask),
                                           N, H, W, Cin, Cout, KH, KW, stride, pad, int(relu), ptr(y8), ptr(emit8[0]), ptr(emit8[1]), stream_ptr())
        return _L().cddmsl_conv_fwd(ptr(x), ptr(w), ptr(y), ptr(scale), ptr(bias), ptr(residual), ptr(relu_mask),
                                    N, H, W, Cin, Cout, KH, KW, stride, pad, int(pool), Cout, Cout, Cout,
                                    int(relu), int(out_f32) | (2 if res_f32 else 0) | (4 if residual_pooled else 0), _dt(x), stream_ptr())
    e0 = PROFILE.begin(plan=launch) if PROFILE.on else None
    st = launch()
    check(st, "cddmsl_conv_fwd")
    PROFILE.end(e0, _CONV_KERNEL.get(_L().cddmsl_last_kernel(), "conv_fwd") if e0 is not None else "conv_fwd",
                2.0 * N * Ho * Wo * Cout * KH * KW * Cin,
                (N * Ho * Wo, Cout, KH * KW * Cin, KH, int(pool), stride),
                nbytes=float(_conv_input_pixels(N, H, W, Ho, Wo, KH, KW, stride, bool(pool)) * Cin * x.element_size()
                             + w.numel() * w.element_size() + y.numel() * y.element_size()
                             + (residual.numel() * residual.element_size() if residual is not None else 0)
                             + (relu_mask.numel() * relu_mask.element_size() if relu_mask is not None else 0)))
    if y8 is not None:
        y._fp8 = (y8, emit8[0].data_ptr())
    return y


def bottleneck64_ok(o1, w2, w3, wd=None, w1n=None):
    if not (o1.is_cuda and o1.dtype == torch.bfloat16 and o1.dim() == 4 and o1.is_contiguous() and o1.shape[3] == 64):
        return False
    want = ((w2, (64, 3, 3, 64)), (w3, (256, 1, 1, 64)), (wd, (256, 1, 1, 64)), (w1n, (64, 1, 1, 256)))
    if any(w is not None and (tuple(w.shape) != s or w.dtype != torch.bfloat16 or not w.is_contiguous()) for w, s in want):
        return False
    N, H, W, _ = o1.shape
    return N > 0 and bool(_L().cddmsl_bottleneck64_ok(N, H, W, 0))


def bottleneck64_fwd(o1, w2, bn2, w3, bn3, residual=None, x0=None, wd=None, bnd=None, w1n=None, bn1n=None):
    require_cuda(o1, w2, w3, residual, x0, wd, w1n)
    assert bottleneck64_ok(o1, w2, w3, wd, w1n) and (residual is None) != (wd is None)
    N, H, W, _ = o1.shape
    for t, c in ((residual, 256), (x0 if wd is not None else None, 64)):
        assert t is None or (t.dtype == torch.bfloat16 and t.is_contiguous() and tuple(t.shape) == (N, H, W, c))
    for bn, c in ((bn2, 64), (bn3, 256), (bnd, 256), (bn1n, 64)):
        assert bn is None or all(v.dtype == torch.float32 and v.numel() == c and v.is_contiguous() and v.is_cuda for v in bn)
    assert (wd is None) == (bnd is None) and (w1n is None) == (bn1n is None) and (wd is None or x0 is not None)
    out = torch.empty((N, H, W, 256), device=o1.device, dtype=o1.dtype)
    o1n = torch.empty((N, H, W, 64), device=o1.device, dtype=o1.dtype) if w1n is not None else None
    sd, bd = bnd if bnd is not None else (None, None)
    s1n, b1n = bn1n if bn1n is not None else (None, None)
    e0 = PROFILE.begin(name="k_bottleneck64") if PROFILE.on else None
    check(_L().cddmsl_bottleneck64_fwd(ptr(o1), ptr(w2), ptr(bn2[0]), ptr(bn2[1]), ptr(w3), ptr(bn3[0]), ptr(bn3[1]), ptr(residual),
                                       ptr(x0 if wd is not None else None), ptr(wd), ptr(sd), ptr(bd), ptr(w1n), ptr(s1n), ptr(b1n),
                                       ptr(out), ptr(o1n), N, H, W, 0, stream_ptr()), "cddmsl_bottleneck64_fwd")
    M = N * H * W
    kn = 576 * 64 + 64 * 256 + (64 * 256 if wd is not None else 0) + (256 * 64 if w1n is not None else 0)
    PROFILE.end(e0, "k_bottleneck64", 2.0 * M * kn, (M, 256, 576, 3, int(wd is not None), int(w1n is not None)),
                nbytes=float(2 * M * (64 + (64 if wd is not None else 256) + 256 + (64 if w1n is not None else 0)) + 2 * kn))
    return out, o1n


def conv_emit8_ok(M, Cout, KH, KW, Cin_chunks_ok=True):
    return Cout % 256 == 0 and KH * KW <= 31 and ((M + 255) // 256) * (Cout // 256) >= 160 and Cin_chunks_ok and os.environ.get("CDDMSL_GEMM256", "1") != "0"


FP8_MAX = 448.0


@_timed("quantize_fp8")
def quantize_fp8(x, scale=None, amax=None):
    require_cuda(x, scale, amax)
    assert x.is_contiguous() and x.dtype in (torch.bfloat16, torch.float32) and x.numel() % 8 == 0
    y = torch.empty(x.shape, device=x.device, dtype=torch.uint8)
    check(_L().cddmsl_quantize_fp8(ptr(x), ptr(y), ptr(scale), ptr(amax), x.numel(), 0 if x.dtype == torch.bfloat16 else 1, stream_ptr()),
          "cddmsl_quantize_fp8")
    return y


def conv_fwd_fp8_ok(M, Cin, Cout, KH, KW, pad):
    min_tiles = int(os.environ.get("CDDMSL_FP8_MIN_TILES", "160"))
    min_k = int(os.environ.get("CDDMSL_FP8_MIN_K", "2048"))
    return Cin % 128 == 0 and Cout % 256 == 0 and KH * KW <= 31 and 2 * pad <= KH - 1 and ((M + 255) // 256) * (Cout // 256) >= min_tiles \
        and KH * KW * Cin >= min_k


def conv_fwd_fp8(x8, w8, scale=None, bias=None, residual=None, relu=False, relu_mask=None, pad=0, out_f32=False, emit8=None):
    require_cuda(x8, w8, scale, bias, residual, relu_mask)
    assert x8.dtype == torch.uint8 and w8.dtype == torch.uint8 and x8.is_contiguous() and w8.is_contiguous()
    N, H, W, Cin = x8.shape
    Cout, KH, KW, Cin2 = w8.shape
    assert Cin == Cin2
    Ho, Wo = H + 2 * pad - KH + 1, W + 2 * pad - KW + 1
    y = torch.empty((N, Ho, Wo, Cout), device=x8.device, dtype=torch.float32 if out_f32 else torch.bfloat16)
    for v in (scale, bias):
        assert v is None or (v.dtype == torch.float32 and v.numel() == Cout and v.is_contiguous())
    for v in (residual, relu_mask):
        assert v is None or (v.dtype == torch.bfloat16 and v.is_contiguous() and v.numel() == y.numel())

    y8 = torch.empty(y.shape, device=x8.device, dtype=torch.uint8) if emit8 is not None else None
    assert emit8 is None or not out_f32

    def launch():
        return _L().cddmsl_conv_fwd_fp8(ptr(x8), ptr(w8), ptr(y), ptr(scale), ptr(bias), ptr(residual), ptr(relu_mask),
                                        N, H, W, Cin, Cout, KH, KW, pad, int(relu), int(out_f32), ptr(y8),
                                        ptr(emit8[0]) if emit8 else c_void_p(0), ptr(emit8[1]) if emit8 else c_void_p(0), stream_ptr())
    e0 = PROFILE.begin(name="k_conv_fwd256_fp8") if PROFILE.on else None
    check(launch(), "cddmsl_conv_fwd_fp8")
    PROFILE.end(e0, "k_conv_fwd256_fp8", 2.0 * N * Ho * Wo * Cout * KH * KW * Cin, (N * Ho * Wo, Cout, KH * KW * Cin, KH, 0, 1),
                nbytes=float(x8.numel() + w8.numel() + y.numel() * y.element_size() + (residual.numel() * 2 if residual is not None else 0)
                             + (relu_mask.numel() * 2 if relu_mask is not None else 0)))
    if y8 is not None:
        y._fp8 = (y8, emit8[0].data_ptr())
    return y


@_timed("fp8_dot_nt")
def fp8_dot_nt(a8, b8, alpha=None):
    require_cuda(a8, b8, alpha)
    R, K = a8.shape
    N = b8.shape[0]
    assert a8.dtype == torch.uint8 and b8.dtype == torch.uint8 and a8.is_contiguous() and b8.is_contiguous() and b8.shape[1] == K
    c = torch.empty((R, N), device=a8.device, dtype=torch.float32)
    check(_L().cddmsl_fp8_dot_nt(ptr(a8), ptr(b8), ptr(c), ptr(alpha), R, N, K, N, stream_ptr()), "cddmsl_fp8_dot_nt")
    return c


def pooled_residual_ok(t):
    return t.numel() * t.element_size() < 2 ** 31 and t.shape[-1] % 8 == 0


def linear_fwd(x, w, scale=None, bias=None, residual=None, relu=False, relu_mask=None, out_f32=False):
    M, K = x.shape
    y = conv_fwd(x.view(1, 1, M, K), w.view(w.shape[0], 1, 1, K), scale, bias,
                 None if residual is None else residual.view(1, 1, M, -1), relu,
                 None if relu_mask is None else relu_mask.view(1, 1, M, -1), out_f32=out_f32)
    return y.view(M, w.shape[0])


_WORKSPACE = {}
WORKSPACE_BYTES = 288 << 20


def ensure_workspace(device):
    key = torch.device(device).index or 0
    if key not in _WORKSPACE:
        ws = torch.empty(WORKSPACE_BYTES, dtype=torch.uint8, device=device)
        check(_L().cddmsl_set_workspace(ptr(ws), ctypes.c_long(ws.numel())), "cddmsl_set_workspace")
        _WORKSPACE[key] = ws
    return _WORKSPACE[key]


def conv_wgrad(x, dy, w_shape, scale=None, stride=1, pad=0, pool=False, out=None):
    require_cuda(x, dy, scale, out)
    Cout, KH, KW, Cin = w_shape
    N, H, W, Cin2 = x.shape
    assert Cin == Cin2 and x.dtype == dy.dtype and x.is_contiguous() and dy.is_contiguous()
    assert dy.shape[-1] == Cout and dy.numel() // Cout == (N * (H // 2) * (W // 2) if pool else
                                                          N * ((H + 2 * pad - KH) // stride + 1) * ((W + 2 * pad - KW) // stride + 1))
    if out is None:
        out = torch.zeros(w_shape, device=x.device, dtype=torch.float32)
    assert out.dtype == torch.float32 and out.is_contiguous() and tuple(out.shape) == tuple(w_shape)
    ensure_workspace(x.device)
    def launch():
        return _L().cddmsl_conv_wgrad(ptr(x), ptr(dy), ptr(out), ptr(scale), N, H, W, Cin, Cout, KH, KW, stride, pad,
                                      int(pool), Cout, _dt(x), stream_ptr())
    e0 = PROFILE.begin(plan=launch) if PROFILE.on else None
    st = launch()
    check(st, "cddmsl_conv_wgrad")
    PROFILE.end(e0, _CONV_KERNEL.get(_L().cddmsl_last_kernel(), "conv_wgrad") if e0 is not None else "conv_wgrad",
                2.0 * (dy.numel() // Cout) * Cout * KH * KW * Cin,
                (dy.numel() // Cout, Cout, KH * KW * Cin, KH, int(pool), stride),
                nbytes=float(_conv_input_pixels(N, H, W, (H // 2) if pool else (H + 2 * pad - KH) // stride + 1,
                                                 (W // 2) if pool else (W + 2 * pad - KW) // stride + 1, KH, KW, stride, bool(pool)) * Cin * x.element_size()
                             + dy.numel() * dy.element_size() + out.numel() * 4))
    return out


def conv_wgrad_fp8_ok(M, Cin, Cout, KH, KW, pad, min_m=None, taps_only=True):
    min_m = int(os.environ.get("CDDMSL_FP8_WGRAD_MIN_M", "300000" if min_m is None else str(min_m)))
    return os.environ.get("CDDMSL_FP8_WGRAD", "1") != "0" and (KH * KW > 1 or not taps_only) and M >= min_m \
        and bool(_L().cddmsl_conv_wgrad_fp8_ok(Cin, Cout, KH, KW, pad, Cout))


def conv_wgrad_fp8(x8, dy8, w_shape, scale, pad=0, out=None):
    require_cuda(x8, dy8, scale, out)
    Cout, KH, KW, Cin = w_shape
    N, H, W, Cin2 = x8.shape
    assert Cin == Cin2 and x8.dtype == torch.uint8 and dy8.dtype == torch.uint8 and x8.is_contiguous() and dy8.is_contiguous()
    assert dy8.shape[-1] == Cout and dy8.numel() // Cout == N * H * W and 2 * pad == KH - 1
    assert scale is not None and scale.dtype == torch.float32 and scale.numel() == Cout and scale.is_contiguous()
    if out is None:
        out = torch.zeros(w_shape, device=x8.device, dtype=torch.float32)
    assert out.dtype == torch.float32 and out.is_contiguous() and tuple(out.shape) == tuple(w_shape)
    ensure_workspace(x8.device)
    def launch():
        return _L().cddmsl_conv_wgrad_fp8(ptr(x8), ptr(dy8), ptr(out), ptr(scale), N, H, W, Cin, Cout, KH, KW, pad, Cout, stream_ptr())
    e0 = PROFILE.begin(name="k_wgrad256_fp8") if PROFILE.on else None
    check(launch(), "cddmsl_conv_wgrad_fp8")
    PROFILE.end(e0, "k_wgrad256_fp8", 2.0 * (N * H * W) * Cout * KH * KW * Cin, (N * H * W, Cout, KH * KW * Cin, KH, 0, 1),
                nbytes=float(x8.numel() + dy8.numel() + out.numel() * 4))
    return out


@_timed("weight_prep")
def weight_prep(w_master, scale, dtype, want_fwd=True, want_dgrad=True):
    require_cuda(w_master, scale)
    assert w_master.dtype == torch.float32 and w_master.is_contiguous() and w_master.dim() == 4
    Cout, KH, KW, Cin = w_master.shape
    wf = torch.empty((Cout, KH, KW, Cin), device=w_master.device, dtype=dtype) if want_fwd else None
    wd = torch.empty((Cin, KH, KW, Cout), device=w_master.device, dtype=dtype) if want_dgrad else None
    st = _L().cddmsl_weight_prep(ptr(w_master), ptr(scale), ptr(wf), ptr(wd), Cout, KH, KW, Cin, DT[dtype], stream_ptr())
    check(st, "cddmsl_weight_prep")
    return wf, wd


@_timed("weight_prep")
def weight_prep_multi(table, count, dtype):
    require_cuda(table)
    assert table.dtype == torch.int64 and table.is_contiguous() and table.shape == (count, 8)
    check(_L().cddmsl_weight_prep_multi(ptr(table), count, DT[dtype], stream_ptr()), "cddmsl_weight_prep_multi")


def _f3(v):
    return (c_float * 3)(*[float(x) for x in v])


def _image_table(images_u8):
    import ctypes
    n = len(images_u8)
    ptrs = (ctypes.c_void_p * n)(*[im.data_ptr() for im in images_u8])
    hs = (ctypes.c_int * n)(*[int(im.shape[1]) for im in images_u8])
    ws = (ctypes.c_int * n)(*[int(im.shape[2]) for im in images_u8])
    return ptrs, hs, ws


@_timed("preprocess")
def preprocess(images_u8, Hp, Wp, mean, std, dtype, Cp=None, div255=True):
    require_cuda(*images_u8)
    Cp = Cp or (8 if dtype == torch.bfloat16 else 4)
    out = torch.empty((len(images_u8), Hp, Wp, Cp), device=images_u8[0].device, dtype=dtype)
    m, s = _f3(mean), _f3(std)
    for im in images_u8:
        assert im.dtype == torch.uint8 and im.dim() == 3 and im.shape[0] == 3 and im.is_contiguous()
    ptrs, hs, ws = _image_table(images_u8)
    check(_L().cddmsl_preprocess_batch(ptrs, hs, ws, len(images_u8), ptr(out), Hp, Wp, Cp, m, s, int(div255), DT[dtype], stream_ptr()),
          "cddmsl_preprocess_batch")
    return out


@_timed("preprocess224")
def preprocess224(images_u8, Hp, Wp, mean, std, dtype, size=224, Cp=None):
    require_cuda(*images_u8)
    Cp = Cp or (8 if dtype == torch.bfloat16 else 4)
    if Wp <= Hp:
        RW, RH = size, int(size * Hp / Wp)
    else:
        RH, RW = size, int(size * Wp / Hp)
    top, left = int(round((RH - size) / 2.0)), int(round((RW - size) / 2.0))
    out = torch.empty((len(images_u8), size, size, Cp), device=images_u8[0].device, dtype=dtype)
    m, s = _f3(mean), _f3(std)
    for im in images_u8:
        assert im.dtype == torch.uint8 and im.dim() == 3 and im.is_contiguous()
    ptrs, hs, ws = _image_table(images_u8)
    check(_L().cddmsl_preprocess224_batch(ptrs, hs, ws, len(images_u8), ptr(out), Hp, Wp, RH, RW, top, left, size, Cp,
                                           m, s, DT[dtype], stream_ptr()), "cddmsl_preprocess224_batch")
    return out


@_timed("avgpool2_fwd")
def avgpool2_fwd(x):
    require_cuda(x)
    N, H, W, C = x.shape
    y = torch.empty((N, H // 2, W // 2, C), device=x.device, dtype=x.dtype)
    check(_L().cddmsl_avgpool2_fwd(ptr(x), ptr(y), N, H, W, C, _dt(x), stream_ptr()), "cddmsl_avgpool2_fwd")
    return y


@_timed("avgpool2_bwd")
def avgpool2_bwd(dy, in_shape, mask=None, add=None, emit8=None):
    require_cuda(dy, mask, add)
    N, H, W, C = in_shape
    assert dy.is_contiguous() and tuple(dy.shape) == (N, H // 2, W // 2, C)
    dx = torch.empty(in_shape, device=dy.device, dtype=dy.dtype)
    if emit8 is not None and dy.dtype == torch.bfloat16:
        y8 = torch.empty(in_shape, device=dy.device, dtype=torch.uint8)
        check(_L().cddmsl_avgpool2_bwd_q8(ptr(dy), ptr(mask), ptr(add), ptr(dx), N, H, W, C, ptr(y8), ptr(emit8[0]), ptr(emit8[1]), stream_ptr()),
              "cddmsl_avgpool2_bwd_q8")
        dx._fp8 = (y8, emit8[0].data_ptr())
        return dx
    check(_L().cddmsl_avgpool2_bwd(ptr(dy), ptr(mask), ptr(add), ptr(dx), N, H, W, C, _dt(dy), stream_ptr()), "cddmsl_avgpool2_bwd")
    return dx


@_timed("attn_tokens_fwd")
def attn_tokens_fwd(x, pos, tp=None):
    require_cuda(x, pos)
    K, P, C = x.shape
    tp = tp or P + 1
    assert pos.dtype == torch.float32 and tuple(pos.shape) == (P + 1, C) and x.is_contiguous() and pos.is_contiguous()
    tok = torch.empty((K, tp, C), device=x.device, dtype=x.dtype)
    check(_L().cddmsl_attn_tokens_fwd(ptr(x), ptr(pos), ptr(tok), K, P, tp, C, _dt(x), stream_ptr()), "cddmsl_attn_tokens_fwd")
    return tok


@_timed("attn_tokens_fwd")
def attn_tokens_fwd_mask(x, pos, tp=None):
    require_cuda(x, pos)
    K, P, C = x.shape
    tp = tp or P + 1
    assert pos.dtype == torch.float32 and tuple(pos.shape) == (P + 1, C) and x.is_contiguous() and pos.is_contiguous() and P <= 64
    tok = torch.empty((K, tp, C), device=x.device, dtype=x.dtype)
    mbits = torch.empty((K, C), device=x.device, dtype=torch.int64)
    check(_L().cddmsl_attn_tokens_fwd_mask(ptr(x), ptr(pos), ptr(tok), ptr(mbits), K, P, tp, C, _dt(x), stream_ptr()), "cddmsl_attn_tokens_fwd_mask")
    return tok, mbits


def rpn_losses(logits, deltas, pos, neg, midx, gt, gt_off, anchors, weights, inv_norm, gout=None):
    require_cuda(logits, deltas, pos, neg, midx, gt, gt_off, anchors)
    for t in (logits, deltas, gt, anchors):
        assert t.dtype == torch.float32 and t.is_contiguous()
    for t in (pos, neg, midx, gt_off):
        assert t.dtype == torch.int64 and t.is_contiguous()
    A = anchors.shape[0]
    assert deltas.numel() == 4 * logits.numel() and midx.numel() == logits.numel()
    args = (ptr(logits), ptr(deltas), ptr(pos), pos.numel(), ptr(neg), neg.numel(), ptr(midx), ptr(gt), ptr(gt_off), ptr(anchors), A,
            *[float(w) for w in weights], float(inv_norm))
    if gout is None:
        out = torch.empty(2, device=logits.device, dtype=torch.float32)
        check(_L().cddmsl_rpn_losses(*args, ptr(out), None, None, None, stream_ptr()), "cddmsl_rpn_losses")
        return out
    dl, dd = torch.zeros_like(logits), torch.zeros_like(deltas)
    g = gout.contiguous().float()
    check(_L().cddmsl_rpn_losses(*args, None, ptr(g), ptr(dl), ptr(dd), stream_ptr()), "cddmsl_rpn_losses(backward)")
    return dl, dd


def box_l1(deltas, fg, cls, src, tgt, weights, inv_norm, gout=None):
    require_cuda(deltas, fg, src, tgt)
    assert deltas.dtype == torch.float32 and deltas.dim() == 2 and deltas.is_contiguous() and fg.dtype == torch.int64 and fg.is_contiguous()
    assert src.dtype == tgt.dtype == torch.float32 and src.is_contiguous() and tgt.is_contiguous() and (cls is None or (cls.dtype == torch.int64 and cls.is_contiguous()))
    args = (ptr(deltas), deltas.shape[1], ptr(fg), fg.numel(), ptr(cls), ptr(src), ptr(tgt), *[float(w) for w in weights], float(inv_norm))
    if gout is None:
        out = torch.empty(1, device=deltas.device, dtype=torch.float32)
        check(_L().cddmsl_box_l1(*args, ptr(out), None, None, stream_ptr()), "cddmsl_box_l1")
        return out
    dd = torch.zeros_like(deltas)
    g = gout.contiguous().float().view(1)
    check(_L().cddmsl_box_l1(*args, None, ptr(g), ptr(dd), stream_ptr()), "cddmsl_box_l1(backward)")
    return dd


def attnpool_dx_ok(K, H, P, TP, C, dtype):
    return dtype == torch.bfloat16 and P == 49 and TP == 56 and 2 * H <= 64 and (2 * H) % 8 == 0 and C % 128 == 0 and 0 < K <= 65535 * 8


@_timed("attnpool_dx")
def attnpool_dx(pds, zu, g0, mbits, P, gpos=None):
    require_cuda(pds, zu, g0, mbits)
    K, H2, TP = pds.shape
    C = zu.shape[2]
    assert pds.dtype == zu.dtype == torch.bfloat16 and g0.dtype == torch.float32 and mbits.dtype == torch.int64
    assert pds.is_contiguous() and zu.is_contiguous() and g0.is_contiguous() and mbits.is_contiguous() and tuple(zu.shape) == (K, H2, C)
# ... 794 lines not shown
```

cddmsl_amd/layers.py:

```python
import os
import weakref

import torch

from . import hip

_STEP = [0]


def bump_weight_version():
    _STEP[0] += 1


_LOAD_GEN = [0]


def note_weights_loaded(*_):
    _LOAD_GEN[0] += 1
    _STEP[0] += 1


def load_generation():
    return _LOAD_GEN[0]

# ... 259 lines not shown
                                    pad, emit8=emit8)
    if emit8 is not None:
        Cout_d, KH, KW, Cin_d = wd.shape
        N, H, W, _ = g.shape
        pad = kw.get("pad", 0)
        M = N * (H + 2 * pad - KH + 1) * (W + 2 * pad - KW + 1)
        if not (T == torch.bfloat16 and hip.conv_emit8_ok(M, Cout_d, KH, KW, (Cin_d * 2 // 16) % 8 == 0) and not kw.get("residual_pooled", False)):
            emit8 = None
    return hip.conv_fwd(g, wd, emit8=emit8, **kw)


def _fp8_dgrad_wanted(pw, g_shape, pad, fp8):
    if not fp8:
        return False
    Cout, KH, KW, Cin = _ohwi(pw.param).shape
    N, H, W, _ = g_shape
    M = N * (H + 2 * pad - KH + 1) * (W + 2 * pad - KW + 1)
    return hip.conv_fwd_fp8_ok(M, Cout, Cin, KH, KW, pad)


def cat_prepared(weights, dtype):
    return torch.cat([hip.weight_prep(_ohwi(w.detach()), None, dtype, True, False)[0] for w in weights], dim=0)


class ConvFn(torch.autograd.Function):

    @staticmethod
    def forward(ctx, x, anchor, pw, bias, stride, pad, relu, out_f32, train_w, residual=None, fp8=False):
        y = conv_fwd_auto(x, pw, None, None if bias is None else bias.detach(), fp8, residual=None if residual is None else residual.detach(),
                          relu=relu, stride=stride, pad=pad, out_f32=out_f32)
        ctx.pw, ctx.bias, ctx.cfg = pw, bias, (stride, pad, relu, out_f32, train_w)
        ctx.fp8 = bool(fp8)
        ctx.save_for_backward(x, y if relu else None, _fp8_made_for(x, pw) if fp8 else None)
        return y

    @staticmethod
    def backward(ctx, dy):
        x, y, x8 = ctx.saved_tensors
        stride, pad, relu, out_f32, train_w = ctx.cfg
        f8 = ctx.fp8 and x8 is not None and stride == 1
        g_slot = fp8_slot_of(ctx.pw, "_fp8_g") if f8 else None
        T = x.dtype
        dy_in = dy
        dy = dy.contiguous()
        if relu:
            dy = hip.relu_bwd(dy, y if y.dtype == T else y.to(T))
        elif dy.dtype != T:
            dy = dy.to(T)
        w = ctx.pw.param
        if train_w:
            if f8:
                wgrad_auto(x, dy, ctx.pw, None, pad, _ohwi(_grad_buf(w)), True, x8, g_slot, min_m=65536)
            else:
                hip.conv_wgrad(x, dy, _ohwi(w).shape, None, stride=stride, pad=pad, out=_ohwi(_grad_buf(w)))
            if ctx.bias is not None:
                hip.colsum(dy.view(-1, dy.shape[-1]), out=_grad_buf(ctx.bias))
        dx = None
        if ctx.needs_input_grad[0]:
            assert stride == 1, "input gradient of a strided conv is not on the hot path"
            _, wd = ctx.pw.get(T, need_dgrad=True)
            KH = _ohwi(w).shape[1]
            Kd, rows = dy.shape[-1], dy.numel() // dy.shape[-1]
            if KH == 1 and _ohwi(w).shape[2] == 1 and pad == 0 and rows <= 1024 and Kd >= 8192 and Kd % (16 * 64) == 0:
                S, N = 16, x.shape[-1]
                part = torch.empty(S, rows, N, device=dy.device, dtype=torch.float32)
                hip.gemm_nt_batched(dy, wd, part, rows, N, Kd // S, Kd, Kd, N, S, Kd // S, Kd // S, rows * N)
                dx = part.sum(0).to(T).view(x.shape)
            elif f8:
                dx = dgrad_auto(dy, ctx.pw, True, g_slot, pad=KH - 1 - pad)
            else:
                dx = hip.conv_fwd(dy, wd, stride=1, pad=KH - 1 - pad)
        return dx, None, None, None, None, None, None, None, None, (dy_in if ctx.needs_input_grad[9] else None), None


class FrozenMlpFn(torch.autograd.Function):

    @staticmethod
    def forward(ctx, x, pw1, b1, pw2, b2, residual):
        T = x.dtype
        w1, _ = pw1.get(T, need_dgrad=False)
        w2, _ = pw2.get(T, need_dgrad=False)
        M, K = x.shape
        h = hip.conv_fwd(x.view(1, 1, M, K), w1, None, b1.detach(), relu=True)
        y = hip.conv_fwd(h, w2, None, b2.detach(), residual.detach().view(1, 1, M, -1), out_f32=True)
        ctx.pw = (pw1, pw2)
        ctx.save_for_backward(h)
        return y.view(M, -1)

    @staticmethod
    def backward(ctx, dy):
        (h,) = ctx.saved_tensors
        T = h.dtype
        M = h.shape[2]
        g = dy.contiguous()
        if g.dtype != T:
            g = g.to(T)
        _, w2d = ctx.pw[1].get(T, need_dgrad=True)
        _, w1d = ctx.pw[0].get(T, need_dgrad=True)
        dh = hip.conv_fwd(g.view(1, 1, M, -1), w2d, relu_mask=h)
        dx = hip.conv_fwd(dh, w1d).view(M, -1) if ctx.needs_input_grad[0] else None
        return dx, None, None, None, None, (dy if ctx.needs_input_grad[5] else None)


def frozen_mlp(x2d, pw1, b1, pw2, b2, residual):
    return FrozenMlpFn.apply(x2d.contiguous(), pw1, b1, pw2, b2, residual.contiguous())


def conv(x, pw, bias=None, stride=1, pad=0, relu=False, out_f32=False, train_w=True, residual=None, fp8=False):
    anchor = pw.param if train_w else None
    assert residual is None or not relu
    return ConvFn.apply(x, anchor, pw, bias, stride, pad, relu, out_f32, train_w, residual, fp8)


def linear(x2d, pw, bias=None, relu=False, out_f32=False, train_w=True, residual=None):
    M, K = x2d.shape
    y = conv(x2d.contiguous().view(1, 1, M, K), pw, bias, 1, 0, relu, out_f32, train_w,
             None if residual is None else residual.contiguous().view(1, 1, M, -1))
    return y.view(M, -1)


class FusedHeadsFn(torch.autograd.Function):

    @staticmethod
    def forward(ctx, x, anchor, heads, out_f32):
        T = x.dtype
        K = heads[0][0].shape[1] if heads[0][0].dim() == 2 else heads[0][0].shape[1]
        ws = [w.detach().reshape(w.shape[0], -1) for w, _ in heads]
        n = sum(w.shape[0] for w in ws)
        npad = (n + 7) // 8 * 8
        wcat = torch.zeros(npad, 1, 1, ws[0].shape[1], device=x.device, dtype=torch.float32)
        wcat[:n, 0, 0] = torch.cat(ws, dim=0)
        bcat = torch.zeros(npad, device=x.device, dtype=torch.float32)
        bcat[:n] = torch.cat([b.detach() for _, b in heads])
        wf, wd = hip.weight_prep(wcat, None, T, True, True)
        y = hip.conv_fwd(x, wf, None, bcat, out_f32=out_f32)
        ctx.heads, ctx.wd, ctx.npad = heads, wd, npad
        ctx.save_for_backward(x)
        return y

    @staticmethod
    def backward(ctx, dy):
        (x,) = ctx.saved_tensors
        T = x.dtype
        dy = dy.contiguous()
        if dy.dtype != T:
            dy = dy.to(T)
        K = x.shape[-1]
        dw = hip.conv_wgrad(x, dy, (ctx.npad, 1, 1, K))
        db = hip.colsum(dy.view(-1, ctx.npad))
        off = 0
        for w, b in ctx.heads:
            n = w.shape[0]
            _grad_buf(w).view(n, -1).add_(dw[off:off + n].view(n, -1)) if w.dim() == 2 else \
                _ohwi(_grad_buf(w)).add_(dw[off:off + n])
            _grad_buf(b).add_(db[off:off + n])
            off += n
        dx = hip.conv_fwd(dy, ctx.wd) if ctx.needs_input_grad[0] else None
        return dx, None, None, None


def fused_heads(x, heads, out_f32=True):
    return FusedHeadsFn.apply(x, heads[0][0], heads, out_f32)


class BlockParams:

    def __init__(self, w1, w2, w3, wd, bn1, bn2, bn3, bnd, stride, frozen, fp8=False):
        self.stride, self.frozen, self.fp8 = stride, frozen, fp8
        self.bn = (bn1, bn2, bn3, bnd)
        self.w = (w1, w2, w3, wd)
        self.pw = tuple(None if w is None else PreparedWeight(w, b[0], frozen) for w, b in zip(self.w, self.bn))


def _block_forward(x, bp, save, px_given=None, next_pw=None, out_spec=None):
    (s1, b1), (s2, b2), (s3, b3), bnd = bp.bn
    pool = bp.stride > 1
    f8 = bp.fp8
    o1_shape = (x.shape[0], x.shape[1], x.shape[2], _ohwi(bp.w[0]).shape[0])
    o1 = conv_fwd_auto(x, bp.pw[0], s1, b1, f8, emit8=fp8_emit_for(bp.pw[1], o1_shape, 1, f8), relu=True)
    x8 = _fp8_made_for(x, bp.pw[0]) if f8 and save else None
    M2 = x.shape[0] * x.shape[1] * x.shape[2]
    e8o2 = fp8_act_slot(bp.pw[2]).emit() if save and not pool and _fp8_wgrad1x1_wanted(bp.pw[2], M2, f8) else None
    o2 = conv_fwd_auto(o1, bp.pw[1], s2, b2, f8, emit8=e8o2, relu=True, pad=1)
    o2_8 = _fp8_made_for(o2, bp.pw[2]) if e8o2 is not None else None
    p2 = hip.avgpool2_fwd(o2) if pool else o2
    if pool and px_given is not None and tuple(px_given.shape) == (x.shape[0], x.shape[1] // 2, x.shape[2] // 2, x.shape[3]):
        px = px_given
    else:
        px = hip.avgpool2_fwd(x) if pool else x
    if bp.pw[3] is not None:
        idn = conv_fwd_auto(px, bp.pw[3], bnd[0], bnd[1], f8)
    else:
        idn = x
    out_shape = (p2.shape[0], p2.shape[1], p2.shape[2], _ohwi(bp.w[2]).shape[0])
    out = conv_fwd_auto(p2, bp.pw[2], s3, b3, f8, emit8=fp8_emit_for(next_pw, out_shape, 0, f8), residual=idn, relu=True, out_spec=out_spec)
    return out, ((o1, o2, p2 if pool else None, px if pool else None, (x8, _fp8_made_for(o1, bp.pw[1]) if f8 else None, o2_8)) if save else None)


def _block_backward(gs, x, o1, o2, p2, px, bp, need_dx, mask_x, prev_bp=None, c8=(None, None, None)):
    T = x.dtype
    (s1, _), (s2, _), (s3, _), bnd = bp.bn
    pool = bp.stride > 1
    f8 = bp.fp8 and T == torch.bfloat16
    w1p, w2p, w3p, wdp = bp.w
    shp = lambda w: _ohwi(w).shape
    gs_slot = fp8_slot_of(bp, "_fp8_gs") if f8 else None
    d2_slot = fp8_slot_of(bp.pw[1], "_fp8_g") if f8 else None
    x8, o1_8, o2_8 = c8
    M2 = o2.shape[0] * o2.shape[1] * o2.shape[2]
    if o2_8 is not None and not pool:
        wgrad_auto(o2, gs, bp.pw[2], s3, 0, _ohwi(_grad_buf(w3p)), f8, o2_8, gs_slot, taps_only=False)
    else:
        hip.conv_wgrad(p2 if pool else o2, gs, shp(w3p), s3, out=_ohwi(_grad_buf(w3p)))
    d1_slot = fp8_slot_of(bp.pw[0], "_fp8_g") if f8 and x8 is not None and _fp8_wgrad1x1_wanted(bp.pw[0], M2, f8) else None
    if pool:
        dp2 = dgrad_auto(gs, bp.pw[2], f8, gs_slot)
        dpre2 = hip.avgpool2_bwd(dp2, tuple(o2.shape), mask=o2, emit8=d2_slot.emit() if f8 and _fp8_dgrad_wanted(bp.pw[1], o2.shape, 1, f8) else None)
    else:
        e8 = d2_slot.emit() if f8 and _fp8_dgrad_wanted(bp.pw[1], o2.shape, 1, f8) else None
        dpre2 = dgrad_auto(gs, bp.pw[2], f8, gs_slot, emit8=e8, relu_mask=o2)
    dpre1 = dgrad_auto(dpre2, bp.pw[1], f8, d2_slot, pad=1, relu_mask=o1, emit8=d1_slot.emit() if d1_slot is not None else None)
    wgrad_auto(o1, dpre2, bp.pw[1], s2, 1, _ohwi(_grad_buf(w2p)), f8, o1_8, d2_slot)
    if d1_slot is not None:
        wgrad_auto(x, dpre1, bp.pw[0], s1, 0, _ohwi(_grad_buf(w1p)), f8, x8, d1_slot, taps_only=False)
    else:
        hip.conv_wgrad(x, dpre1, shp(w1p), s1, out=_ohwi(_grad_buf(w1p)))
    if wdp is not None:
        hip.conv_wgrad(px if pool else x, gs, shp(wdp), bnd[0], out=_ohwi(_grad_buf(wdp)))
    if not need_dx:
        return None
    pooled = False
    if wdp is not None:
        dxb = dgrad_auto(gs, bp.pw[3], f8, gs_slot)
        if pool:
            pooled = x.shape[1] % 2 == 0 and x.shape[2] % 2 == 0 and hip.pooled_residual_ok(dxb)
            if not pooled:
                dxb = hip.avgpool2_bwd(dxb, tuple(x.shape))
    else:
        dxb = gs
    e8 = None
    if f8 and prev_bp is not None and prev_bp.fp8 and not pooled and _fp8_dgrad_wanted(prev_bp.pw[2], x.shape, 0, True):
        e8 = fp8_slot_of(prev_bp, "_fp8_gs").emit()
    return dgrad_auto(dpre1, bp.pw[0], False, None, emit8=e8, residual=dxb, relu_mask=x if mask_x else None, residual_pooled=pooled)


class ResStageFn(torch.autograd.Function):
    @staticmethod
    def forward(ctx, x, anchor, blocks, out_grad_premasked=False, px0=None, out_spec=None):
        ctx.out_grad_premasked = out_grad_premasked
        saved, o1_8s = [x], []
        cur = x
        for bi, bp in enumerate(blocks):
            cur, mids = _block_forward(cur, bp, True, px0 if bi == 0 else None, blocks[bi + 1].pw[0] if bi + 1 < len(blocks) else None,
                                       out_spec if bi + 1 == len(blocks) else None)
            saved += [mids[0], mids[1], mids[2], mids[3], cur]
            o1_8s += list(mids[4])
        ctx.blocks = blocks
        ctx.save_for_backward(*saved, *o1_8s)
        return cur

    @staticmethod
    def backward(ctx, g):
        blocks = ctx.blocks
        saved, o1_8s = ctx.saved_tensors[:-3 * len(blocks)], ctx.saved_tensors[-3 * len(blocks):]
        need_dx = ctx.needs_input_grad[0]
        gs = g.contiguous() if ctx.out_grad_premasked else hip.relu_bwd(g.contiguous(), saved[-1])
        for i in range(len(blocks) - 1, -1, -1):
            x, o1, o2, p2, px = saved[5 * i: 5 * i + 5]
            gs = _block_backward(gs, x, o1, o2, p2, px, blocks[i], need_dx or i > 0, mask_x=i > 0, prev_bp=blocks[i - 1] if i > 0 else None,
                                 c8=tuple(o1_8s[3 * i: 3 * i + 3]))
        return gs, None, None, None, None, None


def _fused_stage_ok(x, blocks, out_spec):
    if os.environ.get("CDDMSL_FUSED_BOTTLENECK", "1") == "0" or out_spec is not None:
        return False
    if not (x.is_cuda and x.dtype == torch.bfloat16 and x.dim() == 4 and x.is_contiguous()):
        return False
    cin = x.shape[3]
    for bi, bp in enumerate(blocks):
        if bp.fp8 or bp.stride != 1 or any(v is None for b in bp.bn[:3] for v in b):
            return False
        if tuple(_ohwi(bp.w[0]).shape) != (64, 1, 1, cin) or tuple(_ohwi(bp.w[1]).shape) != (64, 3, 3, 64) or tuple(_ohwi(bp.w[2]).shape) != (256, 1, 1, 64):
            return False
        if bp.w[3] is not None:
            if bi > 0 or cin != 64 or tuple(_ohwi(bp.w[3]).shape) != (256, 1, 1, 64) or any(v is None for v in bp.bn[3]):
                return False
        elif cin != 256:
            return False
        cin = 256
    return bool(blocks) and bool(hip._L().cddmsl_bottleneck64_ok(x.shape[0], x.shape[1], x.shape[2], 0))


def _fused_stage_forward(x, blocks):
    T = x.dtype
    wf = lambda pw: pw.get(T, need_dgrad=False)[0]
    o1 = conv_fwd_auto(x, blocks[0].pw[0], blocks[0].bn[0][0], blocks[0].bn[0][1], False, relu=True)
    cur = x
    for bi, bp in enumerate(blocks):
        nxt = blocks[bi + 1] if bi + 1 < len(blocks) else None
        kw = dict(x0=cur, wd=wf(bp.pw[3]), bnd=bp.bn[3]) if bp.pw[3] is not None else dict(residual=cur)
        if nxt is not None:
            kw.update(w1n=wf(nxt.pw[0]), bn1n=nxt.bn[0])
        cur, o1 = hip.bottleneck64_fwd(o1, wf(bp.pw[1]), bp.bn[1], wf(bp.pw[2]), bp.bn[2], **kw)
    return cur


def res_stage(x, blocks, frozen, out_grad_premasked=False, out_spec=None):
    px0 = getattr(x, "_pooled2", None)
    if frozen or not torch.is_grad_enabled():
        if _fused_stage_ok(x, blocks, out_spec):
            return _fused_stage_forward(x, blocks)
        cur = x
        for bi, bp in enumerate(blocks):
            cur, _ = _block_forward(cur, bp, False, px0 if bi == 0 else None, blocks[bi + 1].pw[0] if bi + 1 < len(blocks) else None,
                                    out_spec if bi + 1 == len(blocks) else None)
        return cur
    return ResStageFn.apply(x, blocks[0].w[0], blocks, out_grad_premasked, px0, out_spec)


class StackHalvesFn(torch.autograd.Function):

    @staticmethod
    def forward(ctx, a, b, full):
        n = a.shape[0]
        assert a.data_ptr() == full.data_ptr() and b.data_ptr() == full[n:].data_ptr() and full.shape[0] == 2 * n and a.shape == b.shape
        ctx.n = n
        return full.view(full.shape)

    @staticmethod
    def backward(ctx, g):
        return g[:ctx.n], g[ctx.n:], None


def stack_halves(a, b, full):
    return StackHalvesFn.apply(a, b, full)


def res_stage_attnpool(x, blocks, frozen, ap):
    fuse = not frozen and torch.is_grad_enabled()
    y = res_stage(x, blocks, frozen, out_grad_premasked=fuse)
    return AttnPoolFn.apply(y, None if ap.frozen else ap.q_w, ap, fuse)


def roi_downsample_on_map(K, out_size, N, H, W):
    if os.environ.get("CDDMSL_ROI_COMMUTE", "1") == "0":
        return False
    v = os.environ.get("CDDMSL_ROI_COMMUTE_DOWN", "")
    if v in ("0", "1"):
        return v == "1"
    return K * (out_size // 2) ** 2 > N * H * W


def _roi_block0_forward(feat, rois, bp, out_size, scale, sr, extra, next_pw=None, on_map=None):
    T = feat.dtype
    (s1, b1), (s2, b2), (s3, b3), bnd = bp.bn
    w1, _ = bp.pw[0].get(T, False)
    f8 = bp.fp8
    K, E = rois.shape[0], (0 if extra is None else extra.shape[0])
    N, H, W, _ = feat.shape
    z = hip.conv_fwd(feat, w1)
    o1_shape = (K + E, out_size, out_size, z.shape[-1])
    e8 = fp8_emit_for(bp.pw[1], o1_shape, 1, f8) if E == 0 else None
    o1 = hip.roi_align_forward_affine(z, rois, out_size, out_size, scale, sr, True, s1, b1, relu=True, extra_rows=E, emit8=e8)
    del z
    if on_map is None:
        on_map = roi_downsample_on_map(K, out_size, N, H, W)
    if on_map:
        wd, _ = bp.pw[3].get(T, False)
        zd = hip.conv_fwd(feat, wd)
        idn = hip.roi_align_forward_affine(zd, rois, out_size, out_size, scale, sr, True, bnd[0], bnd[1], pooled_only=True, extra_rows=E)
        del zd
        px = None
        if E:
            px = hip.avgpool2_fwd(extra)
            idn[K:].copy_(hip.conv_fwd(px, wd, bnd[0], bnd[1]))
    else:
        px = hip.roi_align_forward_affine(feat, rois, out_size, out_size, scale, sr, True, pooled_only=True, extra_rows=E)
        idn = None
    if E:
        o1[K:].copy_(hip.conv_fwd(extra, w1, s1, b1, relu=True))
        if idn is None:
            px[K:].copy_(hip.avgpool2_fwd(extra))
    o2 = conv_fwd_auto(o1, bp.pw[1], s2, b2, f8, relu=True, pad=1)
    p2 = hip.avgpool2_fwd(o2)
    if idn is None:
        idn = conv_fwd_auto(px, bp.pw[3], bnd[0], bnd[1], f8)
    out_shape = (p2.shape[0], p2.shape[1], p2.shape[2], _ohwi(bp.w[2]).shape[0])
    out = conv_fwd_auto(p2, bp.pw[2], s3, b3, f8, emit8=fp8_emit_for(next_pw, out_shape, 0, f8), residual=idn, relu=True)
    return o1, o2, p2, px, out, (_fp8_made_for(o1, bp.pw[1]) if f8 else None)


class RoIStageFn(torch.autograd.Function):

    @staticmethod
    def forward(ctx, feat, anchor, rois, roi_start, blocks, out_size, scale, sr, out_grad_premasked, extra):
        feat = feat.contiguous()
        nxt = lambda i: blocks[i + 1].pw[0] if i + 1 < len(blocks) else None
        on_map = roi_downsample_on_map(rois.shape[0], out_size, feat.shape[0], feat.shape[1], feat.shape[2])
        o1, o2, p2, px, cur, o1_8 = _roi_block0_forward(feat, rois, blocks[0], out_size, scale, sr, extra, nxt(0), on_map)
        saved, o1_8s = [feat, rois, roi_start, extra, o1, o2, p2, px, cur], [None, o1_8, None]
        for bi, bp in enumerate(blocks[1:], start=1):
            cur, mids = _block_forward(cur, bp, True, None, nxt(bi))
            saved += [mids[0], mids[1], mids[2], mids[3], cur]
            o1_8s += list(mids[4])
        ctx.blocks, ctx.meta = blocks, (out_size, scale, sr, out_grad_premasked, on_map)
        ctx.save_for_backward(*saved, *o1_8s)
        return cur

    @staticmethod
    def backward(ctx, g):
        blocks = ctx.blocks
        saved, o1_8s = ctx.saved_tensors[:-3 * len(blocks)], ctx.saved_tensors[-3 * len(blocks):]
        out_size, scale, sr, premasked, on_map = ctx.meta
        feat, rois, roi_start, extra = saved[:4]
        st = saved[4:]
        gs = g.contiguous() if premasked else hip.relu_bwd(g.contiguous(), st[-1])
        for i in range(len(blocks) - 1, 0, -1):
            o1, o2, p2, px = st[5 * i: 5 * i + 4]
            gs = _block_backward(gs, st[5 * i - 1], o1, o2, p2, px, blocks[i], True, mask_x=True, prev_bp=blocks[i - 1], c8=tuple(o1_8s[3 * i: 3 * i + 3]))
        bp = blocks[0]
        o1, o2, p2, px = st[0:4]
        T = o1.dtype
        (s1, _), (s2, _), (s3, _), bnd = bp.bn
        w1p, w2p, w3p, wdp = bp.w
        shp = lambda w: _ohwi(w).shape
        K, E = rois.shape[0], (0 if extra is None else extra.shape[0])
        f8 = bp.fp8 and T == torch.bfloat16
        gs_slot = fp8_slot_of(bp, "_fp8_gs") if f8 else None
        d2_slot = fp8_slot_of(bp.pw[1], "_fp8_g") if f8 else None
        hip.conv_wgrad(p2, gs, shp(w3p), s3, out=_ohwi(_grad_buf(w3p)))
        e8 = d2_slot.emit() if f8 and _fp8_dgrad_wanted(bp.pw[1], o2.shape, 1, f8) else None
        dpre2 = hip.avgpool2_bwd(dgrad_auto(gs, bp.pw[2], f8, gs_slot), tuple(o2.shape), mask=o2, emit8=e8)
        dpre1 = dgrad_auto(dpre2, bp.pw[1], f8, d2_slot, pad=1, relu_mask=o1)
        wgrad_auto(o1, dpre2, bp.pw[1], s2, 1, _ohwi(_grad_buf(w2p)), f8, o1_8s[1], d2_slot)
        N, H, W, C = feat.shape
        _, w1d = bp.pw[0].get(T, True)
        dfeat = dextra = dzd = wdd = None
        if on_map:
            _, wdd = bp.pw[3].get(T, True)
            dzd = hip.roi_align_backward(gs[:K], rois, roi_start, (N, H, W, gs.shape[-1]), scale, sr, True, pooled=True)
            hip.conv_wgrad(feat, dzd, shp(wdp), bnd[0], out=_ohwi(_grad_buf(wdp)))
            if E:
                hip.conv_wgrad(px, gs[K:], shp(wdp), bnd[0], out=_ohwi(_grad_buf(wdp)))
        else:
            hip.conv_wgrad(px, gs, shp(wdp), bnd[0], out=_ohwi(_grad_buf(wdp)))
            dxb = dgrad_auto(gs, bp.pw[3], f8, gs_slot)
        dz = hip.roi_align_backward(dpre1[:K], rois, roi_start, (N, H, W, dpre1.shape[-1]), scale, sr, True)
        hip.conv_wgrad(feat, dz, shp(w1p), s1, out=_ohwi(_grad_buf(w1p)))
        if E:
            hip.conv_wgrad(extra, dpre1[K:], shp(w1p), s1, out=_ohwi(_grad_buf(w1p)))
            if ctx.needs_input_grad[9]:
                dxe = hip.conv_fwd(gs[K:], wdd) if on_map else dxb[K:].contiguous()
                dextra = hip.conv_fwd(dpre1[K:], w1d, residual=hip.avgpool2_bwd(dxe, tuple(extra.shape)))
        if ctx.needs_input_grad[0]:
            r = hip.conv_fwd(dzd, wdd) if on_map else hip.roi_align_backward(dxb[:K], rois, roi_start, (N, H, W, C), scale, sr, True, pooled=True)
            dfeat = hip.conv_fwd(dz, w1d, residual=r)
        return dfeat, None, None, None, None, None, None, None, None, dextra


def roi_stage_supported(blocks):
    bp = blocks[0]
    return bp.stride == 2 and bp.w[3] is not None and tuple(bp.w[0].shape[2:]) == (1, 1) and tuple(bp.w[3].shape[2:]) == (1, 1)


def roi_stage(feat, rois, roi_start, blocks, frozen, out_size, scale, sr, extra=None, out_grad_premasked=False):
    assert rois.dim() == 2 and rois.size(1) == 5 and out_size % 2 == 0
    assert extra is None or tuple(extra.shape[1:]) == (out_size, out_size, feat.shape[3])
    if frozen or not torch.is_grad_enabled():
        nxt = lambda i: blocks[i + 1].pw[0] if i + 1 < len(blocks) else None
        cur = _roi_block0_forward(feat.contiguous(), rois, blocks[0], out_size, scale, sr, extra, nxt(0))[4]
        for bi, bp in enumerate(blocks[1:], start=1):
            cur, _ = _block_forward(cur, bp, False, None, nxt(bi))
        return cur
    return RoIStageFn.apply(feat, blocks[0].w[0], rois, roi_start, blocks, out_size, scale, sr, out_grad_premasked, extra)


def roi_stage_attnpool(feat, rois, roi_start, blocks, frozen, ap, out_size, scale, sr, extra=None):
    fuse = not frozen and torch.is_grad_enabled()
    y = roi_stage(feat, rois, roi_start, blocks, frozen, out_size, scale, sr, extra, out_grad_premasked=fuse)
    return AttnPoolFn.apply(y, None if ap.frozen else ap.q_w, ap, fuse)


class RoIAlignFn(torch.autograd.Function):
    @staticmethod
    def forward(ctx, x, rois, roi_start, out_size, scale, sampling_ratio, aligned, with_pooled=False, extra=None):
        K, E = rois.shape[0], (0 if extra is None else extra.shape[0])
        out = hip.roi_align_forward(x, rois, out_size, out_size, scale, sampling_ratio, aligned, with_pooled=with_pooled, extra_rows=E)
        ctx.save_for_backward(rois, roi_start)
        ctx.meta = (tuple(x.shape), scale, sampling_ratio, aligned, K)
        y = out[0] if with_pooled else out
        if E:
            y[K:].copy_(extra)
            if with_pooled:
                out[1][K:].copy_(hip.avgpool2_fwd(extra.contiguous()))
        if with_pooled:
            ctx.mark_non_differentiable(out[1])
        return out

    @staticmethod
    def backward(ctx, dy, *unused):
        rois, roi_start = ctx.saved_tensors
        shape, scale, sr, aligned, K = ctx.meta
        dy = dy.contiguous()
        dx = hip.roi_align_backward(dy[:K], rois, roi_start, shape, scale, sr, aligned)
        dextra = dy[K:] if (dy.shape[0] > K and ctx.needs_input_grad[8]) else None
        return dx, None, None, None, None, None, None, None, dextra


def roi_align(x, rois, roi_start, out_size, scale, sampling_ratio, aligned=True, with_pooled=False, extra=None):
    assert rois.dim() == 2 and rois.size(1) == 5
    assert extra is None or tuple(extra.shape[1:]) == (out_size, out_size, x.shape[3])
    if with_pooled and out_size % 2 == 0:
        y, yp = RoIAlignFn.apply(x, rois, roi_start, out_size, scale, sampling_ratio, aligned, True, extra)
        y._pooled2 = yp
        return y
    return RoIAlignFn.apply(x, rois, roi_start, out_size, scale, sampling_ratio, aligned, False, extra)


class AttnPoolParams:
    def __init__(self, pos, q_w, q_b, k_w, k_b, v_w, v_b, c_w, c_b, heads, frozen=False):
        self.pos, self.heads, self.frozen = pos, heads, frozen
        self.q_w, self.q_b, self.k_w, self.k_b, self.v_w, self.v_b, self.c_w, self.c_b = q_w, q_b, k_w, k_b, v_w, v_b, c_w, c_b
        self.pq = PreparedWeight(q_w, None, frozen)
        self.pk = PreparedWeight(k_w, None, frozen)
        self.pv = PreparedWeight(v_w, None, frozen)
        self.pc = PreparedWeight(c_w, None, frozen)


class AttnPoolFn(torch.autograd.Function):

    TP = 56

    @staticmethod
    def forward(ctx, x, anchor, ap, premask_input_grad=False):
        ctx.relu_src = x if premask_input_grad else None
        T = x.dtype
        K, h, w, C = x.shape
        P, TP, H = h * w, AttnPoolFn.TP, ap.heads
        D = C // H
        assert ap.pos.shape[0] == P + 1 <= TP, "attention pool needs a 7x7 map (clip_backbone.py:86)"
        dev = x.device
        fused_dx = hip.attnpool_dx_ok(K, H, P, TP, C, T) and bool(ctx.needs_input_grad[0]) and os.environ.get("CDDMSL_ATTNPOOL_DX", "1") != "0"
        mbits = None
        if fused_dx and premask_input_grad:
            tok, mbits = hip.attn_tokens_fwd_mask(x.view(K, P, C), ap.pos.detach(), TP)
        else:
            tok = hip.attn_tokens_fwd(x.view(K, P, C), ap.pos.detach(), TP)
        wq, _ = ap.pq.get(T, False)
        wk, wkT = ap.pk.get(T, True)
        wv, wvT = ap.pv.get(T, True)
        wc, _ = ap.pc.get(T, False)
        q0 = hip.conv_fwd(tok.view(K, 1, TP, C), wq, None, ap.q_b.detach(), stride=TP).view(K, C)
        zu = torch.empty((K, 2 * H, C), device=dev, dtype=T)
        hip.gemm_nt_batched(q0, wkT, zu, K, C, D, C, C, 2 * H * C, H, D, D, C, c_off=H * C)
        S = torch.empty((K, H, TP), device=dev, dtype=torch.float32)
        hip.gemm_nt_batched(zu, tok, S, H, TP, C, C, C, TP, K, 2 * H * C, TP * C, H * TP, a_off=H * C)
        p, pT = hip.attnpool_softmax_fwd(S, P + 1, D ** -0.5, T)
        z = torch.empty((K, H, C), device=dev, dtype=T)
        hip.gemm_tn_batched(pT, tok, z, TP, H, C, H, C, C, K, TP * H, TP * C, H * C)
        o = torch.empty((K, C), device=dev, dtype=T)
        hip.gemm_nt_batched(z, wv, o, K, D, C, H * C, C, C, H, C, D * C, D)
        o = o + ap.v_b.detach().to(T)
        out = hip.conv_fwd(o.view(1, 1, K, C), wc, None, ap.c_b.detach(), out_f32=True).view(K, -1)
        ctx.ap = ap
        ctx.fused_dx = fused_dx
        ctx.save_for_backward(tok, q0, zu, p, z, o, mbits)
        ctx.shape = (K, h, w, C)
        return out

    @staticmethod
    def backward(ctx, dout):
        ap = ctx.ap
        tok, q0, zu, p, z, o, mbits = ctx.saved_tensors
        K, h, w, C = ctx.shape
        P, TP, H = h * w, AttnPoolFn.TP, ap.heads
        D = C // H
        T = tok.dtype
        dev = tok.device
        train = not ap.frozen
        dout_t = dout.contiguous().to(T)
        if train:
            hip.conv_wgrad(o.view(1, 1, K, C), dout_t.view(1, 1, K, -1), _ohwi(ap.c_w).shape, out=_ohwi(_grad_buf(ap.c_w)))
            hip.colsum(dout_t, out=_grad_buf(ap.c_b))
        _, wcd = ap.pc.get(T, True)
        wk, wkT = ap.pk.get(T, True)
        wv, wvT = ap.pv.get(T, True)
        do = hip.conv_fwd(dout_t.view(1, 1, K, -1), wcd).view(K, C)
        if train:
            hip.colsum(do, out=_grad_buf(ap.v_b))
            hip.gemm_tn_batched(do, z, _grad_buf(ap.v_w), K, D, C, C, H * C, C, H, D, C, D * C, accumulate=True)
        hip.gemm_nt_batched(do, wvT, zu, K, C, D, C, C, 2 * H * C, H, D, D, C)
        dP = torch.empty((K, H, TP), device=dev, dtype=torch.float32)
        hip.gemm_nt_batched(zu, tok, dP, H, TP, C, C, C, TP, K, 2 * H * C, TP * C, H * TP)
        dsT, pds = hip.attnpool_softmax_bwd(p, dP, D ** -0.5, T)
        du = torch.empty((K, H, C), device=dev, dtype=T)
        hip.gemm_tn_batched(dsT, tok, du, TP, H, C, H, C, C, K, TP * H, TP * C, H * C)
        dq0 = torch.empty((K, C), device=dev, dtype=T)
        hip.gemm_nt_batched(du, wk, dq0, K, D, C, H * C, C, C, H, C, D * C, D)
        if train:
            hip.gemm_tn_batched(q0, du, _grad_buf(ap.k_w), K, D, C, C, H * C, C, H, D, C, D * C, accumulate=True)
            _grad_buf(ap.k_b)
            hip.conv_wgrad(tok.view(K, 1, TP, C), dq0.view(K, 1, 1, C), _ohwi(ap.q_w).shape, stride=TP, out=_ohwi(_grad_buf(ap.q_w)))
            hip.colsum(dq0, out=_grad_buf(ap.q_b))
        _, wqd = ap.pq.get(T, True)
        gpos = _grad_buf(ap.pos) if train else None
# ... 300 lines not shown
```

cddmsl_amd/modeling/backbone.py:

```python
from collections import OrderedDict

import torch
from torch import nn

from .. import hip, layers
from ..registry import BACKBONE_REGISTRY
from ..structures import ShapeSpec


def to_nhwc(x):
    v = x.permute(0, 2, 3, 1)
    return v if v.is_contiguous() else v.contiguous()


def to_nchw(x):
    return x.permute(0, 3, 1, 2)


class Conv2dW(nn.Module):

    def __init__(self, cin, cout, k):
        super().__init__()
        w = torch.empty(cout, cin, k, k).contiguous(memory_format=torch.channels_last)
        self.weight = nn.Parameter(w)


class FrozenBatchNorm2d(nn.Module):

    def __init__(self, num_features, eps=1e-5):
        super().__init__()
        self.num_features, self.eps = num_features, eps
        self.register_buffer("weight", torch.ones(num_features))
        self.register_buffer("bias", torch.zeros(num_features))
        self.register_buffer("running_mean", torch.zeros(num_features))
        self.register_buffer("running_var", torch.ones(num_features) - eps)
        self._aff = None

    def affine(self):
        if self._aff is None or self._aff[0].device != self.weight.device:
            scale = self.weight * (self.running_var + self.eps).rsqrt()
            bias = self.bias - self.running_mean * scale
            self._aff = (scale.float().contiguous(), bias.float().contiguous())
        return self._aff

    def _load_from_state_dict(self, *a, **k):
        self._aff = None
        layers.note_weights_loaded()
        return super()._load_from_state_dict(*a, **k)


class Bottleneck(nn.Module):
    expansion = 4

    def __init__(self, inplanes, planes, stride=1):
        super().__init__()
        self.conv1, self.bn1 = Conv2dW(inplanes, planes, 1), FrozenBatchNorm2d(planes)
        self.conv2, self.bn2 = Conv2dW(planes, planes, 3), FrozenBatchNorm2d(planes)
        self.conv3, self.bn3 = Conv2dW(planes, planes * 4, 1), FrozenBatchNorm2d(planes * 4)
        self.stride = stride
        self.downsample = None
        if stride > 1 or inplanes != planes * 4:
            self.downsample = nn.Sequential(OrderedDict([("0", Conv2dW(inplanes, planes * 4, 1)),
                                                         ("1", FrozenBatchNorm2d(planes * 4))]))
        self.frozen = False

    def params(self):
        ds = self.downsample
        return layers.BlockParams(self.conv1.weight, self.conv2.weight, self.conv3.weight,
                                  None if ds is None else ds[0].weight,
                                  self.bn1.affine(), self.bn2.affine(), self.bn3.affine(),
                                  None if ds is None else ds[1].affine(), self.stride, self.frozen, getattr(self, "fp8", False))


class ResStage(nn.Sequential):

    def __init__(self, *blocks):
        super().__init__(*blocks)
        self._bp = None

    def block_params(self):
        dev = (self[0].conv1.weight.device, layers.load_generation())
        if self._bp is None or self._bp[0] != dev:
            self._bp = (dev, [b.params() for b in self])
        return self._bp[1]

    def forward_nhwc(self, x, then_attnpool=None, out_spec=None):
        frozen = self[0].frozen
        if then_attnpool is not None:
            return layers.res_stage_attnpool(x, self.block_params(), frozen, then_attnpool._params())
        return layers.res_stage(x, self.block_params(), frozen, out_spec=out_spec)

    def forward(self, x):
        return to_nchw(self.forward_nhwc(to_nhwc(x)))


class AttentionPool2d(nn.Module):
    def __init__(self, spacial_dim, embed_dim, num_heads, output_dim=None):
        super().__init__()
        self.positional_embedding = nn.Parameter(torch.randn(spacial_dim ** 2 + 1, embed_dim) / embed_dim ** 0.5)
        self.k_proj = nn.Linear(embed_dim, embed_dim)
        self.q_proj = nn.Linear(embed_dim, embed_dim)
        self.v_proj = nn.Linear(embed_dim, embed_dim)
        self.c_proj = nn.Linear(embed_dim, output_dim or embed_dim)
        self.num_heads = num_heads
        self._ap = None

    def _params(self):
        frozen = not self.q_proj.weight.requires_grad
        if self._ap is None or self._ap.pos.device != self.positional_embedding.device or self._ap.frozen != frozen:
            self._ap = layers.AttnPoolParams(self.positional_embedding, self.q_proj.weight, self.q_proj.bias,
                                             self.k_proj.weight, self.k_proj.bias, self.v_proj.weight, self.v_proj.bias,
                                             self.c_proj.weight, self.c_proj.bias, self.num_heads, frozen)
        return self._ap

    def forward(self, x):
        return layers.attnpool(to_nhwc(x), self._params())


class ModifiedResNet(nn.Module):
    def __init__(self, layers_, output_dim, heads, input_resolution=224, width=64, out_features=None, freeze_at=0,
                 depth=None, pool_vec=False, create_att_pool=True, compute_dtype=torch.bfloat16):
        super().__init__()
        self.output_dim, self.input_resolution, self.compute_dtype = output_dim, input_resolution, compute_dtype
        self.conv1, self.bn1 = Conv2dW(3, width // 2, 3), FrozenBatchNorm2d(width // 2)
        self.conv2, self.bn2 = Conv2dW(width // 2, width // 2, 3), FrozenBatchNorm2d(width // 2)
        self.conv3, self.bn3 = Conv2dW(width // 2, width, 3), FrozenBatchNorm2d(width)
        self._inplanes = width
        self.layer1 = self._make_layer(width, layers_[0])
        self.layer2 = self._make_layer(width * 2, layers_[1], stride=2)
        self.layer3 = self._make_layer(width * 4, layers_[2], stride=2)
        self.layer4 = self._make_layer(width * 8, layers_[3], stride=2)
        self.attnpool = AttentionPool2d(input_resolution // 32, width * 32, heads, output_dim)
        self._out_features = list(out_features) if out_features else []
        ch = {"stem": width, "res2": width * 4, "res3": width * 8, "res4": width * 16, "res5": width * 32}
        st = {"stem": 4, "res2": 4, "res3": 8, "res4": 16, "res5": 32}
        self._out_feature_channels = {k: ch[k] for k in ch if k != "res5" or "res5" in self._out_features}
        self._out_feature_strides = {k: st[k] for k in self._out_feature_channels}
        self._stem_w = None
        self.freeze(freeze_at)

    def _make_layer(self, planes, blocks, stride=1):
        ls = [Bottleneck(self._inplanes, planes, stride)]
        self._inplanes = planes * 4
        for _ in range(1, blocks):
            ls.append(Bottleneck(self._inplanes, planes))
        return ResStage(*ls)

    @property
    def size_divisibility(self):
        return 0

    def output_shape(self):
        return {n: ShapeSpec(channels=self._out_feature_channels[n], stride=self._out_feature_strides[n])
                for n in self._out_features}

    def freeze(self, freeze_at=0):
        assert freeze_at >= 1, "the HIP stem path has no backward: MODEL.BACKBONE.FREEZE_AT must be >= 1"
        self.freeze_at = freeze_at
        for m in (self.conv1, self.conv2, self.conv3):
            m.weight.requires_grad = False
        for idx, stage in enumerate([self.layer1, self.layer2, self.layer3, self.layer4], start=2):
            if freeze_at >= idx:
                for blk in stage:
                    blk.frozen = True
                    for p in blk.parameters():
                        p.requires_grad = False
        return self

    def _stem_weights(self, T, cp):
        dev = self.conv1.weight.device
        key = (T, cp, dev, layers.load_generation(), self.conv1.weight._version, self.conv2.weight._version, self.conv3.weight._version)
        if self._stem_w is None or self._stem_w[0] != key:
            w1 = torch.zeros(self.conv1.weight.shape[0], 3, 3, cp, device=dev)
            w1[..., :3] = self.conv1.weight.detach().permute(0, 2, 3, 1)
            ws = [hip.weight_prep(w1, None, T, True, False)[0],
                  hip.weight_prep(layers._ohwi(self.conv2.weight.detach()), None, T, True, False)[0],
                  hip.weight_prep(layers._ohwi(self.conv3.weight.detach()), None, T, True, False)[0]]
            self._stem_w = (key, ws)
        return self._stem_w[1]

    def stem_nhwc(self, x):
        w1, w2, w3 = self._stem_weights(x.dtype, x.shape[-1])
        (s1, b1), (s2, b2), (s3, b3) = self.bn1.affine(), self.bn2.affine(), self.bn3.affine()
        x = hip.conv_fwd(x, w1, s1, b1, relu=True, stride=2, pad=1)
        x = hip.conv_fwd(x, w2, s2, b2, relu=True, pad=1)
        x = hip.conv_fwd(x, w3, s3, b3, relu=True, pad=1)
        return hip.avgpool2_fwd(x)

    def forward_nhwc(self, x, want_res5=None, res4_spec=None):
        with torch.no_grad():
            x = self.stem_nhwc(x)
        x = self.layer1.forward_nhwc(x)
        x = self.layer2.forward_nhwc(x)
        res4 = self.layer3.forward_nhwc(x, out_spec=res4_spec)
        out = {"res4": res4}
        if "res5" in self._out_features and want_res5 is not False:
            out["res5"] = self.layer4.forward_nhwc(res4)
        return out

    def forward(self, x, want_res5=None):
        assert x.dim() == 4, f"ResNet takes an input of shape (N, C, H, W). Got {x.shape} instead!"
        T = self.compute_dtype
        cp = 8 if T == torch.bfloat16 else 4
        xin = torch.zeros(x.shape[0], x.shape[2], x.shape[3], cp, device=x.device, dtype=T)
        xin[..., :3] = x.permute(0, 2, 3, 1)
        return {k: to_nchw(v) for k, v in self.forward_nhwc(xin, want_res5).items()}


@BACKBONE_REGISTRY.register()
def build_clip_resnet_backbone(cfg, input_shape=None):
    depth = cfg.MODEL.RESNETS.DEPTH
    blocks = {50: [3, 4, 6, 3], 101: [3, 4, 23, 3], 200: [4, 6, 10, 6]}[depth]
    width = {50: 64, 101: 64, 200: 80}[depth]
    embed_dim = {50: 1024, 101: 512, 200: 640}[depth]
    res = {50: 224, 101: 224, 200: 288}[depth]
    mode = cfg.MODEL.get("COMPUTE_DTYPE", "bf16")
    dt = {"bf16": torch.bfloat16, "f32": torch.float32, "fp8": torch.bfloat16}[mode]
    net = ModifiedResNet(blocks, embed_dim, width * 32 // 64, res, width, cfg.MODEL.RESNETS.OUT_FEATURES,
                         cfg.MODEL.BACKBONE.FREEZE_AT, depth, False, True, dt)
    if mode == "fp8":
        for m in net.modules():
            if isinstance(m, Bottleneck):
                m.fp8 = True
    return net


def build_backbone(cfg, input_shape=None):
    if input_shape is None:
        input_shape = ShapeSpec(channels=len(cfg.MODEL.PIXEL_MEAN))
    return BACKBONE_REGISTRY.get(cfg.MODEL.BACKBONE.NAME)(cfg, input_shape)
```

include/cddmsl_hip.h:

```cpp
#ifndef CDDMSL_HIP_H
#define CDDMSL_HIP_H
#include <stddef.h>

#ifdef __cplusplus
extern "C" {
#endif

int cddmsl_abi_version(void);

int cddmsl_conv_fwd(const void* x, const void* w, void* y, const float* scale, const float* bias, const void* residual,
                    const void* relu_mask, int Nimg, int Hi, int Wi, int Cin, int Cout, int KH, int KW, int stride, int pad,
                    int pool, int ldy, int ldr, int ldm, int relu, int out_f32, int dtype, void* stream);
int cddmsl_bottleneck64_ok(int Nimg, int H, int W, int dtype);
int cddmsl_bottleneck64_fwd(const void* o1, const void* w2, const float* s2, const float* b2, const void* w3, const float* s3,
                            const float* b3, const void* residual, const void* x0, const void* wd, const float* sd,
                            const float* bd, const void* w1n, const float* s1n, const float* b1n, void* out, void* o1n,
                            int Nimg, int H, int W, int dtype, void* stream);
int cddmsl_set_workspace(void* ptr, long bytes);
int cddmsl_conv_wgrad(const void* x, const void* dy, float* dw, const float* scale, int Nimg, int Hi, int Wi, int Cin,
                      int Cout, int KH, int KW, int stride, int pad, int pool, int ldd, int dtype, void* stream);
int cddmsl_gemm_nt_batched(const void* a, const void* w, void* c, const float* bias, int M, int N, int K, int lda, int ldb, int ldc,
                           int batch, long sa, long sw, long sc, int out_f32, int dtype, void* stream);
int cddmsl_gemm_tn_batched(const void* a, const void* b, void* out, int M, int N, int K, int lda, int ldb, int ldo, int batch, long sa,
                           long sb, long so, int mode, int dtype, void* stream);
int cddmsl_last_kernel(void);
int cddmsl_plan_only(int on);
int cddmsl_weight_prep(const float* w, const float* scale, void* w_fwd, void* w_dgrad, int Cout, int KH, int KW, int Cin,
                       int dtype, void* stream);
int cddmsl_weight_prep_multi(const long long* table, int count, int dtype, void* stream);

int cddmsl_quantize_fp8(const void* x, void* y, const float* scale, float* amax, long numel, int src_dtype, void* stream);
int cddmsl_conv_fwd_fp8(const void* x, const void* w, void* y, const float* scale, const float* bias, const void* residual,
                        const void* relu_mask, int Nimg, int Hi, int Wi, int Cin, int Cout, int KH, int KW, int pad, int relu,
                        int out_f32, void* y8, const float* q8, float* amax8, void* stream);
int cddmsl_conv_fwd_q8(const void* x, const void* w, void* y, const float* scale, const float* bias, const void* residual,
                       const void* relu_mask, int Nimg, int Hi, int Wi, int Cin, int Cout, int KH, int KW, int stride, int pad,
                       int relu, void* y8, const float* q8, float* amax8, void* stream);
int cddmsl_fp8_dot_nt(const void* a, const void* b, float* c, const float* alpha, int R, int N, int K, int ldc, void* stream);
int cddmsl_conv_wgrad_fp8_ok(int Cin, int Cout, int KH, int KW, int pad, int ldd);
int cddmsl_conv_wgrad_fp8(const void* x8, const void* dy8, float* dw, const float* scale, int Nimg, int Hi, int Wi, int Cin, int Cout,
                          int KH, int KW, int pad, int ldd, void* stream);

int cddmsl_roi_align_forward(const void* x, const float* rois, void* y, void* y_pooled, int* dbg_grid, int N, int C, int H, int W,
                             int K, int ph, int pw, float spatial_scale, int sampling_ratio, int aligned, int dtype, void* stream);
int cddmsl_roi_align_backward(const void* dy, const float* rois, const int* roi_start, void* dx, float* ws_ay, float* ws_ax,
                              int* ws_fp, int N, int C, int H, int W, int K, int ph, int pw, float spatial_scale,
                              int sampling_ratio, int aligned, int dtype, void* stream);
int cddmsl_roi_align_forward_affine(const void* x, const float* rois, void* y, void* y_pooled, const float* scale,
                                    const float* bias, int relu, int N, int C, int H, int W, int K, int ph, int pw,
                                    float spatial_scale, int sampling_ratio, int aligned, int dtype, void* y8, const float* q8,
                                    float* amax8, void* stream);
int cddmsl_roi_align_backward_pooled(const void* dy, const float* rois, const int* roi_start, void* dx, float* ws_ay,
                                     float* ws_ax, int* ws_fp, int N, int C, int H, int W, int K, int ph, int pw,
                                     float spatial_scale, int sampling_ratio, int aligned, int dtype, void* stream);
int cddmsl_roi_align_nchw_anyorder(const void* input, const float* rois, void* output, int N, int C, int H, int W, int K, int ph, int pw,
                                   float spatial_scale, int sampling_ratio, int aligned, int dtype, void* temp, size_t* temp_bytes,
                                   void* stream);
int cddmsl_roi_align_backward_nchw_anyorder(const void* grad, const float* rois, void* grad_input, int N, int C, int H, int W, int K,
                                            int ph, int pw, float spatial_scale, int sampling_ratio, int aligned, int dtype, void* temp,
                                            size_t* temp_bytes, void* stream);

int cddmsl_anchors(const float* cell, float* out, int Hf, int Wf, int A, float stride, float offset, void* stream);
int cddmsl_sort_desc(const float* keys_in, float* keys_out, int* idx_scratch, int* order_out, const int* offsets, int N,
                     int total, void* temp, size_t* temp_bytes, void* stream);
int cddmsl_rpn_decode(const int* order, const float* deltas, const float* cell, const int* img_hw, float* boxes,
                      unsigned char* valid, int N, int Hf, int Wf, int A, int topk, float stride, float offset, float wx,
                      float wy, float ww, float wh, float scale_clamp, float min_size, void* stream);
int cddmsl_nms(const float* boxes, const unsigned char* valid, unsigned long long* mask_ws, int* keep, int* nkeep, int N,
               int n, float thr, int max_keep, void* stream);
int cddmsl_nms_anyorder(const float* boxes, const float* scores, long* keep, int* nkeep, int K, float iou_threshold, void* temp,
                        size_t* temp_bytes, void* stream);
int cddmsl_iou_match(const float* gt, int G, const float* preds, int P, long* matches, signed char* labels,
                     unsigned int* best_ws, int nthr, float t0, float t1, int l0, int l1, int l2, int allow_low_quality,
                     void* stream);

int cddmsl_iou_match_batched(const float* gt, const int* gt_off, const float* preds, const int* pred_off, long* matches,
                             signed char* labels, unsigned int* best_ws, int N, int P, int maxG, int totalG, int nthr, float t0,
                             float t1, int l0, int l1, int l2, int allow_low_quality, void* stream);

int cddmsl_attn_tokens_fwd(const void* x, const float* pos, void* tok, int K, int P, int TP, int C, int dtype, void* stream);
int cddmsl_attn_tokens_fwd_mask(const void* x, const float* pos, void* tok, unsigned long long* mbits, int K, int P, int TP, int C,
                                int dtype, void* stream);
int cddmsl_attnpool_dx(const void* pds, const void* zu, const float* g0, const unsigned long long* mbits, void* dx, float* gpos, int K,
                       int H2, int P, int TP, int C, int dtype, void* stream);
int cddmsl_attn_tokens_bwd(const void* dtok, const void* relu_mask, void* dx, float* gpos, int K, int P, int TP, int C, int dtype,
                           void* stream);
int cddmsl_attnpool_softmax_fwd(const float* S, float* p, void* pT, long K, int H, int P1, int TP, float scale, int dtype, void* stream);
int cddmsl_attnpool_softmax_bwd(const float* p, const float* dP, void* dsT, void* pds, long K, int H, int P1, int TP, float scale,
                                int dtype, void* stream);

int cddmsl_attn_small_fwd(const void* q, const void* k, const void* v, void* o, int nseq, int t, int heads, int dh, int ldq,
                          int ldk, int ldv, int ldo, float scale, int dtype, void* stream);
int cddmsl_attn_small_bwd(const void* q, const void* k, const void* v, const void* dout, void* dq, void* dk, void* dv, int nseq,
                          int t, int heads, int dh, int ldq, int ldk, int ldv, int ldo, float scale, int dtype, void* stream);
int cddmsl_attn_last_fwd(const void* q, const void* kv, void* o, float* p, int n, int t, int heads, int dh, int ldq, int ldkv, int voff,
                         int ldo, float scale, int dtype, void* stream);
int cddmsl_attn_last_bwd(const void* q, const void* kv, const void* dout, const float* p, void* dq, void* dkv, int n, int t, int heads,
                         int dh, int ldq, int ldkv, int voff, int ldo, float scale, int dtype, void* stream);

int cddmsl_text_embed(const long* ids, const void* tok, const float* pos, float* x, long rows, int t, int W, int vocab, int dtype,
                      void* stream);
int cddmsl_attn_causal_fwd(const void* qkv, void* o, int nseq, int t, int heads, int dh, int ldqkv, int ldo, float scale, int dtype,
                           void* stream);
int cddmsl_quick_gelu(void* x, long numel, int dtype, void* stream);
int cddmsl_text_pool(const float* x, const long* rows, const float* gamma, const float* beta, void* y, long R, int nout, int group,
                     int W, float eps, int dtype, void* stream);

int cddmsl_skinny_gemm_workspace(int M, int N, int K);
int cddmsl_skinny_gemm(const void* x, const void* w, const float* bias, const float* residual, void* y, float* ws, long ws_bytes, int M,
                       int N, int K, int epi, void* stream);
int cddmsl_lm_head_workspace(int M, int V);
int cddmsl_lm_head_argmax(const void* h, const void* wte, long* ids, int ld_ids, float* logits, void* ws, long ws_bytes, int M, int V,
                          int K, void* stream);
int cddmsl_decode_attn(const void* qkv, void* kc, void* vc, void* o, int nseq, int heads, int dh, int L, int Lmax, int ldqkv, float scale,
                       int dtype, void* stream);
int cddmsl_pos_embed(const long* ids, int ld_ids, const void* tab, const float* src, const float* wpe, float* x, long rows, int t, int pos0,
                     int W, int vocab, int npos, int dtype, void* stream);
int cddmsl_gelu_new(void* x, long numel, int dtype, void* stream);
int cddmsl_lm_head_topk_workspace(int M, int V);
int cddmsl_lm_head_topk(const void* h, const void* wte, float* vals, int* idx, float* logZ, float* logits, void* ws, long ws_bytes, int M,
                        int V, int K, int B, void* stream);
int cddmsl_beam_step(const float* vals, const int* idx, const float* logZ, const float* sum_in, const int* len_in,
                     const unsigned char* stop_in, const int* hist_in, const unsigned char* anc_in, float* sum_out, int* len_out,
                     unsigned char* stop_out, int* hist_out, unsigned char* anc_out, int* src, long* next_tok, int n, int B, int T, int step,
                     int stop_id, void* stream);
int cddmsl_decode_attn_beam(const void* qkv, const void* pk, const void* pv, void* gk, void* gv, const unsigned char* anc, void* o, int rows,
                            int B, int heads, int dh, int P, int L, int Tg, int ldanc, int ldqkv, float scale, int dtype, void* stream);

int cddmsl_l2norm_fwd(const float* x, float* y, float* inv, long R, int D, float eps, void* stream);
int cddmsl_l2norm_bwd(const float* dy, const float* y, const float* inv, float* dx, long R, int D, void* stream);
int cddmsl_cosine_logits_fwd(const float* x, const float* wn, float* scores, float* inv, long R, int D, int Kc,
                             float temperature, float eps, void* stream);
int cddmsl_cosine_logits_bwd(const float* ds, const float* x, const float* wn, const float* inv, float* dx, long R, int D,
                             int Kc, float temperature, int accumulate, void* stream);
int cddmsl_layernorm_fwd(const float* x, const float* gamma, const float* beta, void* y, float* mean, float* rstd, long R, int D,
                         float eps, int dtype, void* stream);
int cddmsl_layernorm_bwd(const void* dy, const float* x, const float* gamma, const float* mean, const float* rstd, float* dx,
                         long R, int D, int accumulate, int dtype, void* stream);
int cddmsl_focal_ce_fwd(const float* logits, const long* target, float* row_loss, float* probs, long R, int C, float gamma,
                        int bg_class, float bg_weight, void* stream);
int cddmsl_focal_ce_bwd(const float* logits, const long* target, const float* probs, const float* gscale, float* dlogits, long R,
                        int C, float gamma, int bg_class, float bg_weight, void* stream);
int cddmsl_contrastive_fwd(const float* S, float* rlse, float* clse, float* loss, int n, int ld, void* stream);
int cddmsl_contrastive_bwd(const float* S, const float* rlse, const float* clse, const float* gloss, float* dS, int n, int ld,
                           void* stream);
int cddmsl_rpn_losses(const float* logits, const float* deltas, const long* pos, int npos, const long* neg, int nneg, const long* midx,
                      const float* gt, const long* gt_off, const float* anchors, long A, float wx, float wy, float ww, float wh, float inv_norm,
                      float* out2, const float* gout2, float* dlogits, float* ddeltas, void* stream);
int cddmsl_box_l1(const float* deltas, int ld, const long* fg, int nfg, const long* cls, const float* src, const float* tgt, float wx, float wy,
                  float ww, float wh, float inv_norm, float* out1, const float* gout1, float* ddeltas, void* stream);

int cddmsl_preprocess(const unsigned char* img, void* out, int n, int h, int w, int Hp, int Wp, int Cp, const float* mean3,
                      const float* std3, int div255, int dtype, void* stream);
int cddmsl_preprocess224(const unsigned char* img, void* out, int n, int h, int w, int Hp, int Wp, int RH, int RW, int top,
                         int left, int S, int Cp, const float* mean3, const float* std3, int dtype, void* stream);
int cddmsl_preprocess_batch(const unsigned char* const* imgs, const int* hs, const int* ws, int N, void* out, int Hp, int Wp, int Cp,
                            const float* mean3, const float* std3, int div255, int dtype, void* stream);
int cddmsl_preprocess224_batch(const unsigned char* const* imgs, const int* hs, const int* ws, int N, void* out, int Hp, int Wp, int RH,
                               int RW, int top, int left, int S, int Cp, const float* mean3, const float* std3, int dtype, void* stream);
int cddmsl_avgpool2_fwd(const void* x, void* y, int N, int H, int W, int C, int dtype, void* stream);
int cddmsl_avgpool2_bwd(const void* dy, const void* mask, const void* add, void* dx, int N, int H, int W, int C, int dtype,
                        void* stream);
int cddmsl_avgpool2_bwd_q8(const void* dy, const void* mask, const void* add, void* dx, int N, int H, int W, int C, void* y8,
                           const float* q8, float* amax8, void* stream);
int cddmsl_maxpool3s2_fwd(const void* x, void* y, int N, int H, int W, int C, int dtype, void* stream);
int cddmsl_upsample_zero2(const void* t, const void* mask, const void* add, void* dx, int N, int H, int W, int C, int dtype,
                          void* stream);
int cddmsl_meanpool_fwd(const void* x, float* y, long K, int P, int C, int dtype, void* stream);
int cddmsl_meanpool_bwd(const float* dy, void* dx, long K, int P, int C, int dtype, void* stream);
int cddmsl_relu_bwd(const void* g, const void* y, void* dx, long numel, int g_f32, int dtype, void* stream);
int cddmsl_colsum(const void* x, float* out, long rows, int cols, int period, int dtype, void* stream);
int cddmsl_sgd_clip_step(float** params, const float** grads, float** moms, const long* sizes, int count, float* norm_ws,
                         float lr, float momentum, float wd, float clip, int first_step, void* stream);

int cddmsl_instance_boxes(const void* maps, int B, int H, int W, int dtype, int* records, int max_records, int* counts, void* ws,
                          size_t* ws_bytes, void* stream);

#ifdef __cplusplus
}
#endif
#endif
```

Measured before the change: 167.0.

## Fuse 2x2 average pooling into stem conv and last layer1 bottleneck producers

Adds a pooled variant of the small 3x3 conv kernel so the last stem conv writes the 2x2-averaged output directly, skipping the full-resolution activation and the separate avgpool kernel. It also adds a POOL mode to the fused bottleneck64 kernel that tiles 2x16 spatial patches and emits a 2x2-pooled copy of the block output alongside the full output, stored on the tensor for a downstream consumer. The goal is to remove separate pooling launches and their extra memory round trips. The cost is more complex tile indexing, an extra LDS read pass, and partially filled tiles at odd widths.

```diff
diff --git a/cddmsl_amd/csrc/bottleneck64.hip b/cddmsl_amd/csrc/bottleneck64.hip
--- a/cddmsl_amd/csrc/bottleneck64.hip
+++ b/cddmsl_amd/csrc/bottleneck64.hip
@@ -12,13 +12,17 @@
   const char* residual;
   char* out;
   char* o1n;
+  char* pooled;
+  int nxt, nyp, ntp;
+  FastDiv dXT, dYP;
   const float *s2, *b2, *s3, *b3, *sd, *bd, *s1n, *b1n;
   int H, W, M;
   FastDiv dW, dH;
 };
 
-template <bool DOWN, bool NEXT>
+template <bool DOWN, bool NEXT, bool POOL = false>
 __global__ __launch_bounds__(512) void k_bottleneck64(BottleneckArgs p) {
+  static_assert(!POOL || (!DOWN && !NEXT), "the pooled output is the last block's");
   using T = __bf16;
   constexpr int KS2 = 36, WAVES = 8;
   const int lane = threadIdx.x & 63, r = lane & 31, hh = lane >> 5, wv = threadIdx.x >> 6;
@@ -44,12 +48,14 @@
     sc1[nt] = NEXT ? p.s1n[nt * 32 + r] : 1.f; bi1[nt] = NEXT ? p.b1n[nt * 32 + r] : 0.f;
   }
   const int wave = blockIdx.x * WAVES + wv, nwaves = gridDim.x * WAVES;
-  const int ntiles = (p.M + 31) >> 5;
+  const int ntiles = POOL ? p.ntp : (p.M + 31) >> 5;
   const __amdgpu_buffer_rsrc_t rx = __builtin_amdgcn_make_buffer_rsrc((void*)(p.o1 - (long)(p.W + 1) * 128), 0, 0x7fffffff, 0x00020000);
   const __amdgpu_buffer_rsrc_t rx0 = __builtin_amdgcn_make_buffer_rsrc((void*)p.x0, 0, DOWN ? p.M * 128 : 0, 0x00020000);
   const __amdgpu_buffer_rsrc_t rres = __builtin_amdgcn_make_buffer_rsrc((void*)p.residual, 0, DOWN ? 0 : p.M * 512, 0x00020000);
   const __amdgpu_buffer_rsrc_t rout = __builtin_amdgcn_make_buffer_rsrc((void*)p.out, 0, p.M * 512, 0x00020000);
   const __amdgpu_buffer_rsrc_t ro1n = __builtin_amdgcn_make_buffer_rsrc((void*)p.o1n, 0, NEXT ? p.M * 128 : 0, 0x00020000);
+  const int hp = p.H >> 1, wp = p.W >> 1;
+  const __amdgpu_buffer_rsrc_t rpool = __builtin_amdgcn_make_buffer_rsrc((void*)p.pooled, 0, POOL ? (p.M / (p.H * p.W)) * hp * wp * 512 : 0, 0x00020000);
   const float relu_floor = 0.f;
   char* const sb = (char*)slots + wv * 4096;
   char* wbase[8];
@@ -61,6 +67,7 @@
   char* const mbase0 = sb + mrow * 128 + ((((lane & 7) ^ (lane >> 4))) << 4);
   char* const mbase1 = sb + mrow * 128 + ((((lane & 7) ^ (lane >> 4) ^ 4)) << 4);
   auto maddr = [&](int i) -> char* { return ((i & 1) ? mbase1 : mbase0) + i * 1024; };
+  const char* const pbase = sb + (lane >> 3) * 256 + ((((lane & 7) ^ (lane >> 3))) << 4);
   auto put = [&](const f32x16 (&acc)[2], const float (&sc)[2], const float (&bi)[2]) {
 #pragma unroll
     for (int nt = 0; nt < 2; ++nt)
@@ -76,11 +83,29 @@
     for (int ks = 0; ks < 4; ++ks) fa[ks] = *(const u32x4*)(fbase + (((2 * ks) ^ fsw) << 4));
   };
   for (int tile = wave; tile < ntiles; tile += nwaves) {
-    const int m = tile * 32 + r;
-    const bool vm = m < p.M;
-    const unsigned mm = vm ? m : 0;
-    const unsigned tq = fdiv(mm, p.dW), ox = mm - tq * p.W;
-    const unsigned img = fdiv(tq, p.dH), oy = tq - img * p.H;
+    bool vm;
+    unsigned img, oy, ox;
+    unsigned ty0 = 0, tx0 = 0, tb0, tb1, tbp = 0, pool_ok = 0;
+    if (POOL) {
+      const unsigned tu = (unsigned)__builtin_amdgcn_readfirstlane(tile);
+      const unsigned tq = fdiv(tu, p.dXT), xt = tu - tq * p.nxt;
+      img = fdiv(tq, p.dYP);
+      const unsigned yp = tq - img * p.nyp;
+      ty0 = 2 * yp; tx0 = 16 * xt;
+      oy = ty0 + (r >> 4); ox = tx0 + (r & 15);
+      vm = oy < (unsigned)p.H && ox < (unsigned)p.W;
+      tb0 = ((img * p.H + ty0) * p.W + tx0) * 512u; tb1 = tb0 + p.W * 512u;
+      tbp = ((img * hp + yp) * wp + 8 * xt) * 512u;
+      pool_ok = yp < (unsigned)hp ? 1u : 0u;
+    } else {
+      const int m = tile * 32 + r;
+      vm = m < p.M;
+      const unsigned mm = vm ? m : 0;
+      const unsigned tq = fdiv(mm, p.dW);
+      ox = mm - tq * p.W;
+      img = fdiv(tq, p.dH); oy = tq - img * p.H;
+      tb0 = tb1 = tile * 16384u;
+    }
     const int iy0 = (int)oy - 1, ix0 = (int)ox - 1;
     const unsigned lbase = (unsigned)((((int)img * p.H + iy0 + 1) * p.W + ix0 + 1) * 128) + hh * 16;
     unsigned bad = vm ? 0u : 0x1ffu;
@@ -96,9 +121,15 @@
       const unsigned v = lbase | (__builtin_amdgcn_ubfe(bad, (unsigned)t0, 1u) << 31);
       a[ks] = __builtin_amdgcn_raw_buffer_load_b128(rx, v, ((t0 / 3) * p.W + (t0 % 3)) * 128 + c0 * 16, 0);
     }
-    const unsigned rowbad[4] = {tile * 32 + mrow < p.M ? 0u : 0x80000000u, tile * 32 + 8 + mrow < p.M ? 0u : 0x80000000u,
-                                tile * 32 + 16 + mrow < p.M ? 0u : 0x80000000u, tile * 32 + 24 + mrow < p.M ? 0u : 0x80000000u};
+    unsigned rowbad[4];
+#pragma unroll
+    for (int i = 0; i < 4; ++i) {
+      const bool ok = POOL ? (ty0 + (i >> 1) < (unsigned)p.H && tx0 + 8 * (i & 1) + mrow < (unsigned)p.W) : (tile * 32 + 8 * i + mrow < p.M);
+      rowbad[i] = ok ? 0u : 0x80000000u;
+    }
     const unsigned vq = (unsigned)(mrow * 512 + (lane & 7) * 16);
+    auto pvo = [&](int i) -> unsigned { return (vq + (POOL ? (i & 1) : i) * 4096) | rowbad[i]; };
+    auto pso = [&](int i) -> unsigned { return (POOL && i >= 2) ? tb1 : tb0; };
     u32x4 xa[4], rr[4];
     if (DOWN) {
 #pragma unroll
@@ -106,7 +137,7 @@
         xa[ks] = __builtin_amdgcn_raw_buffer_load_b128(rx0, (unsigned)(r * 128 + hh * 16) | (vm ? 0u : 0x80000000u), tile * 4096 + ks * 32, 0);
     } else {
 #pragma unroll
-      for (int i = 0; i < 4; ++i) rr[i] = __builtin_amdgcn_raw_buffer_load_b128(rres, (vq + i * 4096) | rowbad[i], tile * 16384, 0);
+      for (int i = 0; i < 4; ++i) rr[i] = __builtin_amdgcn_raw_buffer_load_b128(rres, pvo(i), pso(i), 0);
     }
     f32x16 acc2[2];
 #pragma unroll
@@ -152,7 +183,7 @@
         for (int i = 0; i < 4; ++i) *(u32x4*)maddr(i) = rr[i];
         if (q < 3) {
 #pragma unroll
-          for (int i = 0; i < 4; ++i) rr[i] = __builtin_amdgcn_raw_buffer_load_b128(rres, (vq + i * 4096) | rowbad[i], tile * 16384 + (q + 1) * 128, 0);
+          for (int i = 0; i < 4; ++i) rr[i] = __builtin_amdgcn_raw_buffer_load_b128(rres, pvo(i), pso(i) + (q + 1) * 128, 0);
         }
       }
 #pragma unroll
@@ -192,7 +223,14 @@
 #pragma unroll
       for (int i = 0; i < 4; ++i) {
         const u32x4 o = *(const u32x4*)maddr(i);
-        __builtin_amdgcn_raw_buffer_store_b128(o, rout, (vq + i * 4096) | rowbad[i], tile * 16384 + q * 128, CDDMSL_STORE_AUX);
+        __builtin_amdgcn_raw_buffer_store_b128(o, rout, pvo(i), pso(i) + q * 128, CDDMSL_STORE_AUX);
+        asm volatile("s_nop 4" ::: "memory");
+        asm volatile("" :: "v"(o));
+      }
+      if (POOL) {
+        const u32x4 o = avg4<T>(*(const u32x4*)pbase, *(const u32x4*)(pbase + 128), *(const u32x4*)(pbase + 2048), *(const u32x4*)(pbase + 2048 + 128));
+        const unsigned pbad = (pool_ok && (tx0 >> 1) + (lane >> 3) < (unsigned)wp) ? 0u : 0x80000000u;
+        __builtin_amdgcn_raw_buffer_store_b128(o, rpool, (unsigned)((lane >> 3) * 512 + (lane & 7) * 16) | pbad, tbp + q * 128, 0);
         asm volatile("s_nop 4" ::: "memory");
         asm volatile("" :: "v"(o));
       }
@@ -228,29 +266,48 @@
   return (long)Nimg * H * W + W + 64 < (1L << 31) / 512 ? 1 : 0;
 }
 
-extern "C" int cddmsl_bottleneck64_fwd(const void* o1, const void* w2, const float* s2, const float* b2, const void* w3,
-                                       const float* s3, const float* b3, const void* residual, const void* x0, const void* wd,
-                                       const float* sd, const float* bd, const void* w1n, const float* s1n, const float* b1n,
-                                       void* out, void* o1n, int Nimg, int H, int W, int dtype, void* stream) {
+static int bottleneck64_run(const void* o1, const void* w2, const float* s2, const float* b2, const void* w3, const float* s3, const float* b3,
+                            const void* residual, const void* x0, const void* wd, const float* sd, const float* bd, const void* w1n,
+                            const float* s1n, const float* b1n, void* out, void* o1n, void* pooled, int Nimg, int H, int W, int dtype,
+                            void* stream) {
   if (!cddmsl_bottleneck64_ok(Nimg, H, W, dtype)) return CDDMSL_ERR_ARG;
   if (!o1 || !w2 || !s2 || !b2 || !w3 || !s3 || !b3 || !out) return CDDMSL_ERR_ARG;
   const bool down = wd != nullptr, next = w1n != nullptr;
   if (down ? (!x0 || !sd || !bd || residual) : (!residual || x0 || sd || bd)) return CDDMSL_ERR_ARG;
   if (next ? (!s1n || !b1n || !o1n) : (s1n || b1n || o1n)) return CDDMSL_ERR_ARG;
+  if (pooled && (down || next || H < 2 || W < 2)) return CDDMSL_ERR_ARG;
   BottleneckArgs a;
   a.o1 = (const char*)o1; a.w2 = (const char*)w2; a.w3 = (const char*)w3; a.wd = (const char*)wd; a.w1n = (const char*)w1n;
-  a.x0 = (const char*)x0; a.residual = (const char*)residual; a.out = (char*)out; a.o1n = (char*)o1n;
+  a.x0 = (const char*)x0; a.residual = (const char*)residual; a.out = (char*)out; a.o1n = (char*)o1n; a.pooled = (char*)pooled;
   a.s2 = s2; a.b2 = b2; a.s3 = s3; a.b3 = b3; a.sd = sd; a.bd = bd; a.s1n = s1n; a.b1n = b1n;
   a.H = H; a.W = W; a.M = Nimg * H * W;
   a.dW = make_fastdiv((unsigned)W); a.dH = make_fastdiv((unsigned)H);
+  a.nxt = (W + 15) / 16; a.nyp = (H + 1) / 2; a.ntp = Nimg * a.nyp * a.nxt;
+  a.dXT = make_fastdiv((unsigned)a.nxt); a.dYP = make_fastdiv((unsigned)a.nyp);
   if (record_kernel(13)) return CDDMSL_OK;
-  const int ncu = persistent_blocks_raw(), ntiles = (a.M + 31) / 32;
+  const int ncu = persistent_blocks_raw(), ntiles = pooled ? a.ntp : (a.M + 31) / 32;
   const int want = (ntiles + 7) / 8, cap = ncu > 0 ? ncu : 256;
   const unsigned nb = (unsigned)(want < cap ? want : cap);
   const hipStream_t st = (hipStream_t)stream;
-  if (down && next) hipLaunchKernelGGL((k_bottleneck64<true, true>), dim3(nb), dim3(512), 0, st, a);
+  if (pooled) hipLaunchKernelGGL((k_bottleneck64<false, false, true>), dim3(nb), dim3(512), 0, st, a);
+  else if (down && next) hipLaunchKernelGGL((k_bottleneck64<true, true>), dim3(nb), dim3(512), 0, st, a);
   else if (down) hipLaunchKernelGGL((k_bottleneck64<true, false>), dim3(nb), dim3(512), 0, st, a);
   else if (next) hipLaunchKernelGGL((k_bottleneck64<false, true>), dim3(nb), dim3(512), 0, st, a);
   else hipLaunchKernelGGL((k_bottleneck64<false, false>), dim3(nb), dim3(512), 0, st, a);
   return launch_status();
 }
+
+extern "C" int cddmsl_bottleneck64_fwd(const void* o1, const void* w2, const float* s2, const float* b2, const void* w3,
+                                       const float* s3, const float* b3, const void* residual, const void* x0, const void* wd,
+                                       const float* sd, const float* bd, const void* w1n, const float* s1n, const float* b1n,
+                                       void* out, void* o1n, int Nimg, int H, int W, int dtype, void* stream) {
+  return bottleneck64_run(o1, w2, s2, b2, w3, s3, b3, residual, x0, wd, sd, bd, w1n, s1n, b1n, out, o1n, nullptr, Nimg, H, W, dtype, stream);
+}
+
+extern "C" int cddmsl_bottleneck64_pool_fwd(const void* o1, const void* w2, const float* s2, const float* b2, const void* w3,
+                                            const float* s3, const float* b3, const void* residual, void* out, void* pooled,
+                                            int Nimg, int H, int W, int dtype, void* stream) {
+  if (!pooled) return CDDMSL_ERR_ARG;
+  return bottleneck64_run(o1, w2, s2, b2, w3, s3, b3, residual, nullptr, nullptr, nullptr, nullptr, nullptr, nullptr, nullptr, out, nullptr,
+                          pooled, Nimg, H, W, dtype, stream);
+}
diff --git a/cddmsl_amd/csrc/conv_fwd.hip b/cddmsl_amd/csrc/conv_fwd.hip
--- a/cddmsl_amd/csrc/conv_fwd.hip
+++ b/cddmsl_amd/csrc/conv_fwd.hip
@@ -479,8 +479,9 @@
   }
 }
 
-template <typename T, int CPP, int NT, int NTAP = 9>
+template <typename T, int CPP, int NT, int NTAP = 9, bool POOL = false>
 __global__ __launch_bounds__(256) void k_conv3x3_small(ConvArgs p) {
+  static_assert(!POOL || (sizeof(T) == 2 && CPP > 1 && NT == 2 && NTAP == 9), "pooled output: the bf16 3x3, 64-channel instantiations with LDS weights");
   constexpr int KC = NTAP * CPP, KS = (KC + 1) / 2;
   constexpr int PAD = NTAP == 9 ? 1 : 0;
   constexpr int ES = Mma<T>::ES;
@@ -507,7 +508,7 @@
 #pragma unroll
   for (int nt = 0; nt < NT; ++nt) { sc[nt] = p.scale ? p.scale[nt * 32 + r] : 1.f; bi[nt] = p.bias ? p.bias[nt * 32 + r] : 0.f; }
   const int wave = (blockIdx.x * blockDim.x + threadIdx.x) >> 6, nwaves = (gridDim.x * blockDim.x) >> 6;
-  const int ntiles = (p.M + 31) >> 5;
+  const int ntiles = POOL ? (p.M + 7) >> 3 : (p.M + 31) >> 5;
   const __amdgpu_buffer_rsrc_t rx = __builtin_amdgcn_make_buffer_rsrc((void*)(p.x - (long)(p.Wi + 1) * (CPP * 16)), 0, 0x7fffffff, 0x00020000);
   const long ybytes = (long)p.M * p.ldy * ES, mbytes = (long)p.M * p.ldm * ES;
   const __amdgpu_buffer_rsrc_t ry = __builtin_amdgcn_make_buffer_rsrc((void*)p.y, 0, (int)(ybytes > 0x7fffffffL ? 0x7fffffffL : ybytes), 0x00020000);
@@ -516,11 +517,11 @@
   __shared__ __attribute__((aligned(16))) u32x4 ost[ES == 2 ? 4 * 32 * NT * 4 : 1];
   const bool ost_ok = !p.relu_mask && p.ldy == NT * 32 && (long)p.M * NT * 64 < 0x7fffffffL;
   for (int tile = wave; tile < ntiles; tile += nwaves) {
-    const int m = tile * 32 + r;
+    const int m = POOL ? tile * 8 + (r >> 2) : tile * 32 + r;
     const bool vm = m < p.M;
     const unsigned mm = vm ? m : 0;
-    const unsigned tq = fdiv(mm, p.dWo), ox = mm - tq * p.Wo;
-    const unsigned img = fdiv(tq, p.dHo), oy = tq - img * p.Ho;
+    const unsigned tq = fdiv(mm, p.dWo), ox = POOL ? 2 * (mm - tq * p.Wo) + (r & 1) : mm - tq * p.Wo;
+    const unsigned img = fdiv(tq, p.dHo), oy = POOL ? 2 * (tq - img * p.Ho) + ((r >> 1) & 1) : tq - img * p.Ho;
     const int iy0 = (int)oy * p.stride - PAD, ix0 = (int)ox * p.stride - PAD;
     const unsigned lbase = (unsigned)((((int)img * p.Hi + iy0 + 1) * p.Wi + ix0 + 1) * (CPP * 16)) + (CPP > 1 ? hh * 16 : 0);
     unsigned bad = vm ? 0u : 0x1ffu;
@@ -563,7 +564,7 @@
         if (WLDS) Mma<T>::step(acc[nt], a[ks], wl[(nt * KS + ks) * 64 + wlane]);
         else Mma<T>::step(acc[nt], a[ks], bw[WLDS ? 0 : nt][WLDS ? 0 : ks]);
       }
-    if (ES == 2 && ost_ok) {
+    if (ES == 2 && (POOL || ost_ok)) {
       char* ob = (char*)ost + (threadIdx.x >> 6) * (32 * NT * 64);
 #pragma unroll
       for (int nt = 0; nt < NT; ++nt)
@@ -574,6 +575,19 @@
           asm("v_max_f32 %0, %1, %2" : "=v"(v) : "v"(v), "s"(relu_floor));
           *(unsigned short*)(ob + row * (NT * 64) + (nt * 32 + r) * 2) = f2bf(v);
         }
+      if (POOL) {
+        asm volatile("" ::: "memory");
+#pragma unroll
+        for (int i = 0; i < NT / 2; ++i) {
+          const int pc = i * 64 + lane, g = pc / (NT * 4), c = pc % (NT * 4);
+          const char* src = ob + (4 * g) * (NT * 64) + c * 16;
+          const u32x4 o = avg4<T>(*(const u32x4*)src, *(const u32x4*)(src + NT * 64), *(const u32x4*)(src + 2 * NT * 64), *(const u32x4*)(src + 3 * NT * 64));
+          const unsigned vo = (unsigned)(pc * 16) | (tile * 8 + g < p.M ? 0u : 0x80000000u);
+          __builtin_amdgcn_raw_buffer_store_b128(o, ry, vo, tile * (8 * NT * 64), 0);
+        }
+        asm volatile("" ::: "memory");
+        continue;
+      }
 #pragma unroll
       for (int i = 0; i < 2 * NT; ++i) {
         const u32x4 o = *(const u32x4*)(ob + (i * 64 + lane) * 16);
@@ -610,11 +624,15 @@
   else if (a.Cout == 32) hipLaunchKernelGGL((k_conv3x3_small<T, 4, 1>), dim3(nb), dim3(256), 0, st, a);
   else hipLaunchKernelGGL((k_conv3x3_small<T, 4, 2>), dim3(nb), dim3(256), 0, st, a);
 }
+template <typename T> void launch_small_pool(const ConvArgs& a, unsigned nb, hipStream_t st) {
+  if constexpr (sizeof(T) == 2) hipLaunchKernelGGL((k_conv3x3_small<T, 4, 2, 9, true>), dim3(nb), dim3(256), 0, st, a);
+}
 
 template <typename T> void launch_tile128(const ConvArgs& a, const Plan& p, hipStream_t st) {
   const dim3 grid(p.gx, p.gy);
   switch (p.kernel) {
     case 8: launch_small<T>(a, p.gx, st); break;
+    case 14: launch_small_pool<T>(a, p.gx, st); break;
     case 2: hipLaunchKernelGGL(k_conv_fwd_reg<T>, grid, dim3(256), 0, st, a); break;
     default: hipLaunchKernelGGL(k_conv_fwd<T>, grid, dim3(256), 0, st, a); break;
   }
diff --git a/cddmsl_amd/csrc/gemm_common.h b/cddmsl_amd/csrc/gemm_common.h
--- a/cddmsl_amd/csrc/gemm_common.h
+++ b/cddmsl_amd/csrc/gemm_common.h
@@ -53,6 +53,7 @@
   unsigned* amax8 = nullptr;
   float* partial = nullptr;
   int tile0 = 0, ksplits = 1, kper = 0, tile_limit = 0;
+  int pool_out = 0;
   int nt_out = 1;
 #ifdef CDDMSL_TILE_STAMPS
   unsigned long long* tstamps = nullptr;
diff --git a/cddmsl_amd/csrc/gemm_conv.hip b/cddmsl_amd/csrc/gemm_conv.hip
--- a/cddmsl_amd/csrc/gemm_conv.hip
+++ b/cddmsl_amd/csrc/gemm_conv.hip
@@ -95,6 +95,11 @@
   const long tiles128 = (long)((a.Cout + BN - 1) / BN) * ((a.M + BM - 1) / BM);
   if (tiles128 > 0x7fffffffL) return {};
   const bool packed = batch == 1 && a.xrs == a.cpp && a.wrs == a.Kc;
+  if (a.pool_out) {
+    const bool ok = op == OP_BF16 && !a.pool && a.KH == 3 && a.KW == 3 && a.pad == 1 && a.stride == 1 && a.cpp == 4 && a.Cout == 64 && a.ldy == 64 &&
+                    !a.residual && !a.relu_mask && !a.out_f32 && !a.y8 && packed && ((long)a.Nimg * a.Hi + 2) * a.Wi * 128 < (1L << 31);
+    return ok ? Plan{14, 256u * 2, 1} : Plan{};
+  }
   if (!a.pool && a.KH == 3 && a.KW == 3 && a.pad == 1 && (a.cpp == 1 || a.cpp == 4 || (a.cpp == 8 && a.Cout == 64)) &&
       (a.Cout == 32 || a.Cout == 64) && !a.residual && !a.out_f32 && packed) {
     return {8, a.cpp > 1 ? 256u * 2 : 256u * 8, 1};
@@ -193,6 +198,23 @@
                       relu, out_f32, nullptr, nullptr, nullptr, stream);
 }
 
+extern "C" int cddmsl_conv_pool2_fwd(const void* x, const void* w, void* y, const float* scale, const float* bias, const void* residual,
+                                     const void* relu_mask, int Nimg, int Hi, int Wi, int Cin, int Cout, int KH, int KW, int stride,
+                                     int pad, int ldy, int relu, int dtype, void* stream) {
+  if (dtype != 0 || residual || relu_mask) return CDDMSL_ERR_ARG;
+  ConvArgs a;
+  const int st = fill_conv(a, OP_BF16, x, w, y, scale, bias, nullptr, nullptr, Nimg, Hi, Wi, Cin, Cout, KH, KW, stride, pad, 0, ldy, ldy, ldy,
+                           relu, 0, nullptr, nullptr, nullptr);
+  if (st != CDDMSL_OK) return st;
+  if (a.Ho < 2 || a.Wo < 2) return CDDMSL_ERR_ARG;
+  a.pool_out = 1;
+  a.Ho /= 2; a.Wo /= 2; a.M = Nimg * a.Ho * a.Wo;
+  a.dWo = make_fastdiv((unsigned)a.Wo); a.dHo = make_fastdiv((unsigned)a.Ho);
+  const Plan p = plan_fwd(a, OP_BF16, 1);
+  if (p.kernel == 0 || a.M == 0) return p.kernel == 0 ? CDDMSL_ERR_ARG : CDDMSL_OK;
+  return run_fwd(a, OP_BF16, p, stream);
+}
+
 extern "C" int cddmsl_conv_fwd_q8(const void* x, const void* w, void* y, const float* scale, const float* bias,
                                   const void* residual, const void* relu_mask, int Nimg, int Hi, int Wi, int Cin,
                                   int Cout, int KH, int KW, int stride, int pad, int relu, void* y8, const float* q8, float* amax8,
diff --git a/cddmsl_amd/hip.py b/cddmsl_amd/hip.py
--- a/cddmsl_amd/hip.py
+++ b/cddmsl_amd/hip.py
@@ -21,6 +21,8 @@
         L.cddmsl_conv_fwd.argtypes = [vp] * 7 + [ci] * 16 + [vp]
         L.cddmsl_bottleneck64_ok.argtypes = [ci] * 4
         L.cddmsl_bottleneck64_fwd.argtypes = [vp] * 17 + [ci] * 4 + [vp]
+        L.cddmsl_bottleneck64_pool_fwd.argtypes = [vp] * 10 + [ci] * 4 + [vp]
+        L.cddmsl_conv_pool2_fwd.argtypes = [vp] * 7 + [ci] * 12 + [vp]
         L.cddmsl_conv_wgrad.argtypes = [vp] * 4 + [ci] * 12 + [vp]
         L.cddmsl_set_workspace.argtypes = [vp, c_long]
         L.cddmsl_weight_prep.argtypes = [vp] * 4 + [ci] * 5 + [vp]
@@ -166,7 +168,7 @@
 
 PROFILE = _Profiler()
 _CONV_KERNEL = {10: "k_conv_fwd256_fp8", 11: "k_conv_fwd2", 1: "k_conv_fwd", 2: "k_conv_fwd_reg", 3: "k_conv_fwd256", 4: "k_conv_wgrad", 5: "k_conv_wgrad_dma", 6: "k_wgrad256", 7: "k_gemm_tn_stream", 8: "k_conv3x3_small", 9: "k_gemm_tn_small", 12: "k_wgrad256_fp8",
-                13: "k_bottleneck64"}
+                13: "k_bottleneck64", 14: "k_conv3x3_small_pool"}
 
 
 def _timed(name):
@@ -260,6 +262,34 @@
     return y
 
 
+def pool_in_producer():
+    return os.environ.get("CDDMSL_POOL_IN_PRODUCER", "1") != "0"
+
+
+def conv_pool2_ok(x, w, stride=1, pad=1):
+    if not (x.is_cuda and x.dtype == torch.bfloat16 and w.dtype == torch.bfloat16 and x.dim() == 4 and x.is_contiguous() and w.is_contiguous()):
+        return False
+    N, H, W, Cin = x.shape
+    return (tuple(w.shape) == (64, 3, 3, 32) and Cin == 32 and stride == 1 and pad == 1 and N > 0 and H >= 2 and W >= 2
+            and (N * H + 2) * W * 128 < 2 ** 31)
+
+
+def conv_pool2_fwd(x, w, scale, bias, relu=True):
+    require_cuda(x, w, scale, bias)
+    assert conv_pool2_ok(x, w), (x.shape, w.shape, x.dtype)
+    N, H, W, Cin = x.shape
+    for v in (scale, bias):
+        assert v is None or (v.dtype == torch.float32 and v.numel() == 64 and v.is_contiguous())
+    y = torch.empty((N, H // 2, W // 2, 64), device=x.device, dtype=x.dtype)
+    e0 = PROFILE.begin(name="k_conv3x3_small_pool") if PROFILE.on else None
+    check(_L().cddmsl_conv_pool2_fwd(ptr(x), ptr(w), ptr(y), ptr(scale), ptr(bias), None, None, N, H, W, Cin, 64, 3, 3, 1, 1, 64, int(relu), 0,
+                                     stream_ptr()), "cddmsl_conv_pool2_fwd")
+    Mc = N * (H // 2) * (W // 2) * 4
+    PROFILE.end(e0, "k_conv3x3_small_pool", 2.0 * Mc * 64 * 9 * Cin, (Mc, 64, 9 * Cin, 3, 0, 1),
+                nbytes=float(N * min(H, 2 * (H // 2) + 1) * min(W, 2 * (W // 2) + 1) * Cin * 2 + w.numel() * 2 + y.numel() * 2))
+    return y
+
+
 def bottleneck64_ok(o1, w2, w3, wd=None, w1n=None):
     if not (o1.is_cuda and o1.dtype == torch.bfloat16 and o1.dim() == 4 and o1.is_contiguous() and o1.shape[3] == 64):
         return False
@@ -270,10 +300,11 @@
     return N > 0 and bool(_L().cddmsl_bottleneck64_ok(N, H, W, 0))
 
 
-def bottleneck64_fwd(o1, w2, bn2, w3, bn3, residual=None, x0=None, wd=None, bnd=None, w1n=None, bn1n=None):
+def bottleneck64_fwd(o1, w2, bn2, w3, bn3, residual=None, x0=None, wd=None, bnd=None, w1n=None, bn1n=None, with_pooled=False):
     require_cuda(o1, w2, w3, residual, x0, wd, w1n)
     assert bottleneck64_ok(o1, w2, w3, wd, w1n) and (residual is None) != (wd is None)
     N, H, W, _ = o1.shape
+    assert not with_pooled or (wd is None and w1n is None and H >= 2 and W >= 2)
     for t, c in ((residual, 256), (x0 if wd is not None else None, 64)):
         assert t is None or (t.dtype == torch.bfloat16 and t.is_contiguous() and tuple(t.shape) == (N, H, W, c))
     for bn, c in ((bn2, 64), (bn3, 256), (bnd, 256), (bn1n, 64)):
@@ -283,15 +314,21 @@
     o1n = torch.empty((N, H, W, 64), device=o1.device, dtype=o1.dtype) if w1n is not None else None
     sd, bd = bnd if bnd is not None else (None, None)
     s1n, b1n = bn1n if bn1n is not None else (None, None)
+    pooled = torch.empty((N, H // 2, W // 2, 256), device=o1.device, dtype=o1.dtype) if with_pooled else None
     e0 = PROFILE.begin(name="k_bottleneck64") if PROFILE.on else None
-    check(_L().cddmsl_bottleneck64_fwd(ptr(o1), ptr(w2), ptr(bn2[0]), ptr(bn2[1]), ptr(w3), ptr(bn3[0]), ptr(bn3[1]), ptr(residual),
-                                       ptr(x0 if wd is not None else None), ptr(wd), ptr(sd), ptr(bd), ptr(w1n), ptr(s1n), ptr(b1n),
-                                       ptr(out), ptr(o1n), N, H, W, 0, stream_ptr()), "cddmsl_bottleneck64_fwd")
+    if with_pooled:
+        check(_L().cddmsl_bottleneck64_pool_fwd(ptr(o1), ptr(w2), ptr(bn2[0]), ptr(bn2[1]), ptr(w3), ptr(bn3[0]), ptr(bn3[1]), ptr(residual),
+                                                ptr(out), ptr(pooled), N, H, W, 0, stream_ptr()), "cddmsl_bottleneck64_pool_fwd")
+    else:
+        check(_L().cddmsl_bottleneck64_fwd(ptr(o1), ptr(w2), ptr(bn2[0]), ptr(bn2[1]), ptr(w3), ptr(bn3[0]), ptr(bn3[1]), ptr(residual),
+                                           ptr(x0 if wd is not None else None), ptr(wd), ptr(sd), ptr(bd), ptr(w1n), ptr(s1n), ptr(b1n),
+                                           ptr(out), ptr(o1n), N, H, W, 0, stream_ptr()), "cddmsl_bottleneck64_fwd")
     M = N * H * W
     kn = 576 * 64 + 64 * 256 + (64 * 256 if wd is not None else 0) + (256 * 64 if w1n is not None else 0)
-    PROFILE.end(e0, "k_bottleneck64", 2.0 * M * kn, (M, 256, 576, 3, int(wd is not None), int(w1n is not None)),
-                nbytes=float(2 * M * (64 + (64 if wd is not None else 256) + 256 + (64 if w1n is not None else 0)) + 2 * kn))
-    return out, o1n
+    PROFILE.end(e0, "k_bottleneck64", 2.0 * M * kn, (M, 256, 576, 3, int(wd is not None), 2 if with_pooled else int(w1n is not None)),
+                nbytes=float(2 * M * (64 + (64 if wd is not None else 256) + 256 + (64 if w1n is not None else 0)) + 2 * kn
+                             + (pooled.numel() * 2 if with_pooled else 0)))
+    return (out, o1n, pooled) if with_pooled else (out, o1n)
 
 
 def conv_emit8_ok(M, Cout, KH, KW, Cin_chunks_ok=True):
diff --git a/cddmsl_amd/layers.py b/cddmsl_amd/layers.py
--- a/cddmsl_amd/layers.py
+++ b/cddmsl_amd/layers.py
@@ -585,6 +585,10 @@
         kw = dict(x0=cur, wd=wf(bp.pw[3]), bnd=bp.bn[3]) if bp.pw[3] is not None else dict(residual=cur)
         if nxt is not None:
             kw.update(w1n=wf(nxt.pw[0]), bn1n=nxt.bn[0])
+        elif bp.pw[3] is None and cur.shape[1] >= 2 and cur.shape[2] >= 2 and hip.pool_in_producer():
+            cur, _, pooled = hip.bottleneck64_fwd(o1, wf(bp.pw[1]), bp.bn[1], wf(bp.pw[2]), bp.bn[2], with_pooled=True, **kw)
+            cur._pooled2 = pooled
+            return cur
         cur, o1 = hip.bottleneck64_fwd(o1, wf(bp.pw[1]), bp.bn[1], wf(bp.pw[2]), bp.bn[2], **kw)
     return cur
 
diff --git a/cddmsl_amd/modeling/backbone.py b/cddmsl_amd/modeling/backbone.py
--- a/cddmsl_amd/modeling/backbone.py
+++ b/cddmsl_amd/modeling/backbone.py
@@ -184,6 +184,8 @@
         (s1, b1), (s2, b2), (s3, b3) = self.bn1.affine(), self.bn2.affine(), self.bn3.affine()
         x = hip.conv_fwd(x, w1, s1, b1, relu=True, stride=2, pad=1)
         x = hip.conv_fwd(x, w2, s2, b2, relu=True, pad=1)
+        if hip.pool_in_producer() and hip.conv_pool2_ok(x, w3):
+            return hip.conv_pool2_fwd(x, w3, s3, b3, relu=True)
         x = hip.conv_fwd(x, w3, s3, b3, relu=True, pad=1)
         return hip.avgpool2_fwd(x)
 
diff --git a/include/cddmsl_hip.h b/include/cddmsl_hip.h
--- a/include/cddmsl_hip.h
+++ b/include/cddmsl_hip.h
@@ -11,11 +11,17 @@
 int cddmsl_conv_fwd(const void* x, const void* w, void* y, const float* scale, const float* bias, const void* residual,
                     const void* relu_mask, int Nimg, int Hi, int Wi, int Cin, int Cout, int KH, int KW, int stride, int pad,
                     int pool, int ldy, int ldr, int ldm, int relu, int out_f32, int dtype, void* stream);
+int cddmsl_conv_pool2_fwd(const void* x, const void* w, void* y, const float* scale, const float* bias, const void* residual,
+                          const void* relu_mask, int Nimg, int Hi, int Wi, int Cin, int Cout, int KH, int KW, int stride, int pad,
+                          int ldy, int relu, int dtype, void* stream);
 int cddmsl_bottleneck64_ok(int Nimg, int H, int W, int dtype);
 int cddmsl_bottleneck64_fwd(const void* o1, const void* w2, const float* s2, const float* b2, const void* w3, const float* s3,
                             const float* b3, const void* residual, const void* x0, const void* wd, const float* sd,
                             const float* bd, const void* w1n, const float* s1n, const float* b1n, void* out, void* o1n,
                             int Nimg, int H, int W, int dtype, void* stream);
+int cddmsl_bottleneck64_pool_fwd(const void* o1, const void* w2, const float* s2, const float* b2, const void* w3, const float* s3,
+                                 const float* b3, const void* residual, void* out, void* pooled, int Nimg, int H, int W, int dtype,
+                                 void* stream);
 int cddmsl_set_workspace(void* ptr, long bytes);
 int cddmsl_conv_wgrad(const void* x, const void* dy, float* dw, const float* scale, int Nimg, int Hi, int Wi, int Cin,
                       int Cout, int KH, int KW, int stride, int pad, int pool, int ldd, int dtype, void* stream);
```

Result: no change. 166.9 (-0.1%).
